# Jiahao-Ma/VFA

Hardware: AMD Instinct MI355X
Metric: voxels aggregated/sec (7 views->BEV grid) (higher is better)
Workload: dtype f32; 1 GPU; multiviewc_200x200x1; cameras_per_rank=7, cameras_total=7, channels=256, rccl_ranks=1, parallelism=single GPU

## Files before the change

include/vfa_hip.h:

```cpp
#ifndef VFA_HIP_H
#define VFA_HIP_H

#include <stddef.h>
#include <stdint.h>

#ifdef __cplusplus
extern "C" {
#endif

#define VFA_ABI_VERSION 9

#define VFA_CONV_MULTIVIEWC 0
#define VFA_CONV_MULTIVIEWX 1
#define VFA_CONV_WILDTRACK 2

#define VFA_VOX_REFERENCE 0
#define VFA_VOX_LAYER_MAJOR 1

#define VFA_VOX_KERNEL_DIRECT 0x100
#define VFA_VOX_KERNEL_TAP_CACHE 0x200

#define VFA_ERR_BAD_ARGUMENT 10001
#define VFA_ERR_UNSUPPORTED 10002

int vfa_abi_version(void);

#define VFA_FLAG_TERMS_MASK 0xf
#define VFA_FLAG_RESERVED_CUS(n) (((n) & 0xff) << 8)
#define VFA_FLAG_DEBUG(mask) (((mask) & 0xfff) << 16)
#define VFA_FLAG_DUMP_VOX (1 << 30)
#define VFA_FLAG_ROWS_ONLY (1 << 28)
#define VFA_FLAG_SKIP_ROWS (1 << 29)
#define VFA_BWD_ACCUMULATE 1

int vfa_integral_image_f32(const float *feature, float *integral, int n_views, int C, int Hf, int Wf,
                           void *stream);

int vfa_affine_relu_integral_image_f32(const float *x, const float *scale, const float *shift, float *integral, int n_views, int C,
                                       int Hf, int Wf, void *stream);

size_t vfa_feature_stats_count(int n_views, int C, int Hf);
int vfa_integral_images_f32(const float *const *features, const float *const *scales, const float *const *shifts,
                            float *const *integrals, unsigned *const *absmax, int n_views, int C, int n_maps, const int *feat_hw,
                            void *stream);
int vfa_integral_absmax_f32(const float *integral, unsigned *absmax, int n_views, int C, int Hf, int Wf, void *stream);

int vfa_integral_images_hwc_f32(const float *const *features_hwc, const float *const *scales, const float *const *shifts,
                                float *const *integrals, unsigned *const *absmax, int n_views, int C, int n_maps, const int *feat_hw,
                                void *stream);

size_t vfa_lateral_conv_workspace_bytes(int n_views, int Hf, int Wf);
int vfa_lateral_conv_f32(const float *feat, const float *weight, const float *bias, const float *gamma, const float *beta, float eps,
                         float *out_hwc, float *scale, float *shift, void *workspace, size_t workspace_bytes, int n_views, int K,
                         int Hf, int Wf, void *stream);
int vfa_lateral_convs_f32(int n_maps, const float *const *feats, const float *const *weights, const float *const *biases,
                          const float *const *gammas, const float *const *betas, const float *eps, float *const *outs_hwc,
                          float *const *scales, float *const *shifts, void *const *workspaces, const size_t *workspace_bytes, int n_views,
                          const int *Ks, const int *feat_hw, void *stream);

int vfa_lateral_convs_train_f32(int n_maps, const float *const *feats, const float *const *weights, const float *const *biases,
                                const float *const *gammas, const float *const *betas, const float *eps, float *const *outs_hwc,
                                float *const *scales, float *const *shifts, double *const *means, double *const *rstds,
                                void *const *workspaces, const size_t *workspace_bytes, int n_views, const int *Ks, const int *feat_hw,
                                void *stream);
size_t vfa_lateral_backward_workspace_bytes(int n_views, int K, int Hf, int Wf);
int vfa_lateral_scan_backward_f32(int n_maps, const float *const *grad_integrals, const float *const *ys_hwc, const float *const *scales,
                                  const float *const *shifts, const double *const *means, const double *const *rstds,
                                  const float *const *gammas, float *const *dzs_hwc, float *const *grad_biases, float *const *grad_gammas,
                                  float *const *grad_betas, void *const *workspaces, const size_t *workspace_bytes, int n_views,
                                  const int *Ks, const int *feat_hw, void *stream);
int vfa_lateral_conv_backward_f32(int n_maps, const float *const *dzs_hwc, const float *const *ys_hwc, const double *const *means,
                                  const float *const *feats, const float *const *weights, float *const *grad_feats,
                                  float *const *grad_weights, void *const *workspaces, const size_t *workspace_bytes, int n_views,
                                  const int *Ks, const int *feat_hw, void *stream);

int vfa_box_params_f32(const float *calibs, const float *grid, const float *z_layers, const float *corner_off,
                       int n_views, int n_cells, int nl, int conv_kind, float img_w, float img_h, int Hf, int Wf,
                       float cmin, float cmax, float *box, float *area, uint8_t *visible, void *stream);

int vfa_gather_f32(const float *integral, const float *box, const float *area, const uint8_t *visible, float *vox,
                   int n_views, int C, int Hf, int Wf, int nl, int n_cells, int cell_begin, int cell_count,
                   int vox_layout, void *stream);

int vfa_project_gather_f32(const float *integral, const float *calibs, const float *grid, const float *z_layers,
                           const float *corner_off, float *vox, int n_views, int C, int Hf, int Wf, int nl,
                           int n_cells, int cell_begin, int cell_count, int conv_kind, float img_w, float img_h,
                           float cmin, float cmax, int vox_layout, void *stream);

int vfa_project_collapse_f32(const float *integral, const float *calibs, const float *grid, const float *z_layers,
                             const float *corner_off, const float *weight_t, float *lin, int n_views, int C, int Hf, int Wf,
                             int nl, int n_cells, int c_out, int conv_kind, float img_w, float img_h, float cmin, float cmax,
                             void *stream);

size_t vfa_gather_workspace_bytes(int n_views, int nl, int cell_count);
int vfa_project_gather_ws_f32(const float *integral, const float *calibs, const float *grid, const float *z_layers,
                              const float *corner_off, float *vox, void *workspace, size_t workspace_bytes, int n_views,
                              int C, int Hf, int Wf, int nl, int n_cells, int cell_begin, int cell_count, int conv_kind,
                              float img_w, float img_h, float cmin, float cmax, int vox_layout, void *stream);

int vfa_project_gather_backward_f32(const float *grad_vox, const float *calibs, const float *grid, const float *z_layers,
                                    const float *corner_off, float *grad_integral, int n_views, int C, int Hf, int Wf,
                                    int nl, int n_cells, int cell_begin, int cell_count, int conv_kind, float img_w,
                                    float img_h, float cmin, float cmax, int flags, void *stream);
int vfa_project_gather_backward_grid_f32(const float *grad_vox, const float *calibs, const float *grid, const float *z_layers,
                                    const float *corner_off, float *grad_integral, int n_views, int C, int Hf, int Wf,
                                    int nl, int n_cells, int cell_begin, int cell_count, int grid_w, int conv_kind, float img_w,
                                    float img_h, float cmin, float cmax, int flags, void *stream);

size_t vfa_gather_backward_det_workspace_bytes(int n_views, int nl, int cell_count, int C, int Hf, int Wf);
int vfa_project_gather_backward_det_f32(const float *grad_vox, const float *calibs, const float *grid, const float *z_layers,
                                        const float *corner_off, float *grad_integral, int n_views, int C, int Hf, int Wf, int nl,
                                        int n_cells, int cell_begin, int cell_count, int grid_w, int conv_kind, float img_w,
                                        float img_h, float cmin, float cmax, int flags, void *workspace, size_t workspace_bytes,
                                        void *stream);

size_t vfa_gather_backward_geometry_workspace_bytes(int n_views, int cell_count);
int vfa_project_gather_backward_geometry_f32(const float *grad_vox, const float *integral, const float *calibs, const float *grid,
                                             const float *z_layers, const float *corner_off, float *grad_calibs, float *grad_grid,
                                             int n_views, int C, int Hf, int Wf, int nl, int n_cells, int cell_begin, int cell_count,
                                             int conv_kind, float img_w, float img_h, float cmin, float cmax, int flags, void *workspace,
                                             size_t workspace_bytes, void *stream);

int vfa_column_sum_f32(const float *x, float *out, long long rows, int N, int accumulate, void *stream);

int vfa_integral_image_backward_f32(float *grad_integral, float *grad_feature, int n_views, int C, int Hf, int Wf,
                                    void *stream);

int vfa_relu_mask_backward_f32(const float *grad, const float *lin, const float *bias, float *grad_lin, float *grad_bias,
                               int n_views, size_t M, int N, void *stream);

int vfa_bias_relu_accumulate_f32(const float *lin, const float *bias, float *out, int n_views, size_t M, int N,
                                 int accumulate, void *stream);

int vfa_scale_view_sum_f32(const float *lin8, const float *lin16, const float *lin32, const float *bias8,
                           const float *bias16, const float *bias32, float *ortho, int n_views, size_t M, int N,
                           int accumulate, void *stream);

int vfa_scale_view_max_f32(const float *lin8, const float *lin16, const float *lin32, const float *bias8, const float *bias16,
                           const float *bias32, float *ortho, uint8_t *argmax, int n_views, size_t M, int N, void *stream);

int vfa_scale_view_max_backward_f32(const float *grad, const float *lin8, const float *lin16, const float *lin32, const float *bias8,
                                    const float *bias16, const float *bias32, const uint8_t *argmax, float *grad_lin8,
                                    float *grad_lin16, float *grad_lin32, float *grad_bias8, float *grad_bias16, float *grad_bias32,
                                    int n_views, size_t M, int N, void *stream);

int vfa_collapse_relu_sum_f32(const float *vox, const float *weight, const float *bias, float *out, int n_views, size_t M,
                              int K, int N, int accumulate, int flags, void *stream);

size_t vfa_collapse_gemm_workspace_bytes(int K, int N);
int vfa_collapse_gemm_f32(const float *vox, const float *weight, float *lin, void *workspace, size_t workspace_bytes, size_t M,
                          int K, int N, int flags, void *stream);

int vfa_collapse_gemm_relu_backward_f32(const float *vox, const float *weight, const float *bias, const float *grad_out,
                                        float *grad_lin, float *grad_bias, void *workspace, size_t workspace_bytes, int n_views,
                                        size_t cells, int K, int N, int flags, void *stream);
int vfa_collapse_gemm_relu_backward_f16_f32(const float *vox, const float *weight, const float *bias, const float *grad_out,
                                            float *grad_lin, float *grad_bias, void *workspace, size_t workspace_bytes, int n_views,
                                            size_t cells, int K, int N, const unsigned *feat_absmax, int absmax_count,
                                            const unsigned char *row_shift, const unsigned char *tile_any, int flags, void *stream);
size_t vfa_sliver_shifts_scratch_bytes(int L, int W);
int vfa_sliver_shifts_u8(const float *calibs, const float *grid, const float *z_layers, int n_layers, const float *corner_off, int n_views,
                         int L, int W, int conv_kind, float img_w, float img_h, float cmin, float cmax, int Hf, int Wf, int per_item,
                         unsigned char *shift, void *scratch, size_t scratch_bytes, void *stream);

size_t vfa_frame_workspace_bytes(int n_views, int L, int W, int n_scales);
int vfa_frame_workspace_layout(int n_views, int L, int W, int n_scales, size_t *offsets, int *tiles);
int vfa_frame_records_f32(const float *calibs, const float *grid, const float *z_layers, const float *corner_off, int n_views, int L,
                          int W, int conv_kind, float img_w, float img_h, float cmin, float cmax, int n_scales,
                          const int *feat_hw, const float *const *weights, int flags, void *workspace, size_t workspace_bytes,
                          void *stream);
int vfa_frame_boxes_f32(const float *calibs, const float *grid, const float *z_layers, const float *corner_off, int n_views, int L,
                        int W, int conv_kind, float img_w, float img_h, float cmin, float cmax, int n_scales,
                        const int *feat_hw, void *workspace, size_t workspace_bytes, void *stream);
int vfa_frame_cuts_f32(int n_views, int L, int W, int n_scales, const float *const *weights, int flags, void *workspace,
                       size_t workspace_bytes, void *stream);
int vfa_pool_windows_f32(const float *integral, const void *workspace, size_t workspace_bytes, float *vox, int n_views, int L, int W,
                         int n_scales, int scale, int Hf, int Wf, void *stream);
int vfa_pool_collapse_relu_sum_f32(const float *const *integrals, const unsigned *const *feat_absmax, const float *const *biases,
                                   const void *workspace, size_t workspace_bytes, float *out, int n_views, int L, int W, int n_scales,
                                   const int *feat_hw, int accumulate, int flags, void *stream);

size_t vfa_pipe_workspace_bytes(int n_views, int L, int W, int n_layers, int n_scales);
int vfa_pipe_workspace_layout(int n_views, int L, int W, int n_layers, int n_scales, size_t *offsets, int *tiles);
int vfa_pipe_boxes_f32(const float *calibs, const float *grid, const float *z_layers, int n_layers, const float *corner_off, int n_views,
                       int L, int W, int conv_kind, float img_w, float img_h, float cmin, float cmax, int n_scales, const int *feat_hw,
                       int flags, void *workspace, size_t workspace_bytes, void *stream);
int vfa_pipe_cuts_f32(int n_views, int L, int W, int n_layers, int n_scales, const float *const *weights, int flags, void *workspace,
                      size_t workspace_bytes, void *stream);
int vfa_pipe_records_f32(const float *calibs, const float *grid, const float *z_layers, int n_layers, const float *corner_off,
                         int n_views, int L, int W, int conv_kind, float img_w, float img_h, float cmin, float cmax, int n_scales,
                         const int *feat_hw, const float *const *weights, int flags, void *workspace, size_t workspace_bytes, void *stream);
int vfa_pipe_collapse_relu_sum_f32(const float *const *integrals, const unsigned *const *feat_absmax, const float *const *biases,
                                   void *workspace, size_t workspace_bytes, float *out, int n_views, int L, int W, int n_layers,
                                   int n_scales, const int *feat_hw, int accumulate, int flags, void *stream);
int vfa_pipe_balance_f32(int n_views, int L, int W, int n_layers, int n_scales, int reserved_cus, int mode, void *workspace,
                         size_t workspace_bytes, void *stream);

size_t vfa_pipe_batch_workspace_bytes(int n_frames, int n_views, int L, int W, int n_layers, int n_scales);
int vfa_pipe_batch_workspace_layout(int n_frames, int n_views, int L, int W, int n_layers, int n_scales, size_t *offsets, int *tiles);
int vfa_pipe_batch_records_f32(const float *calibs, const float *grid, const float *z_layers, int n_layers, const float *corner_off,
                               int n_views, int L, int W, int conv_kind, float img_w, float img_h, float cmin, float cmax, int n_scales,
                               const int *feat_hw, const float *const *weights, int n_frames, int flags, void *workspace,
                               size_t workspace_bytes, void *stream);
int vfa_pipe_batch_collapse_relu_sum_f32(const float *const *integrals, const unsigned *const *feat_absmax, const float *const *biases,
                                         void *workspace, size_t workspace_bytes, float *out, int n_frames, int n_views, int L, int W,
                                         int n_layers, int n_scales, const int *feat_hw, int accumulate, int flags, void *stream);
int vfa_pipe_batch_balance_f32(int n_frames, int n_views, int L, int W, int n_layers, int n_scales, int reserved_cus, int mode,
                               void *workspace, size_t workspace_bytes, void *stream);

size_t vfa_grad_weight_workspace_bytes(long long rows, int K);
int vfa_grad_weight_f32(const float *g_lin, const float *vox, float *g_w, long long rows, int K, int accumulate, void *workspace,
                        size_t workspace_bytes, void *stream);
size_t vfa_grad_input_workspace_bytes(int K);
int vfa_grad_input_f32(const float *g_lin, const float *w, float *g_vox, long long rows, int K, void *workspace, size_t workspace_bytes,
                       void *stream);

int vfa_sort_vertices_f32(const float *vertices, const uint8_t *mask, const int *num_valid, int *idx, int b, int n, int m, void *stream);
int vfa_bev_nms_f32(const float *heatmap, float *conf, int L, int W, void *stream);
int vfa_bev_nms_batch_f32(const float *heatmap, float *conf, int B, int L, int W, void *stream);

int vfa_iou3d_f32(const float *box1, const float *box2, float *iou3d, float *iou_bev, long long count, void *stream);
int vfa_iou3d_frames_f32(const float *det, const int *det_begin, const float *gt, const int *gt_begin, int n_frames, int n_det, int n_gt,
                         const long long *pair_begin, long long n_pairs, float *iou, int *best_idx, float *best_iou, void *stream);

#define VFA_CLEAR_MOD_MAX_SIDE 512
#define VFA_CLEAR_MOD_TOO_LARGE 1
#define VFA_CLEAR_MOD_BAD_OFFSETS 2
#define VFA_CLEAR_MOD_SOLVER_FLAG 3
int vfa_clear_mod_frames_f64(const double *det_xy, const int *det_begin, const double *gt_xy, const int *gt_begin, int n_frames, int n_det,
                             int n_gt, double td, const long long *pair_begin, long long n_pairs, double *dist, int *gt_match,
                             double *gt_dist, long long *frame_counts, double *frame_cost, int *frame_status, void *stream);

#define VFA_BEV_DECODE_MAX_TOPK 1024
size_t vfa_bev_decode_workspace_bytes(int B, int L, int W, int topk);
int vfa_bev_decode_f32(const float *heatmap, const float *loc_offset, const long long *loc_stride, const float *dim_offset,
                       const long long *dim_stride, const float *rotation, const long long *rot_stride, int B, int L, int W, int n_rot,
                       int topk, float cls_thresh, float grid0, float grid1, float world0, float world1, const float *dimension_mean,
                       int yx_first, void *workspace, size_t workspace_bytes, int *count, float *conf, float *location, int *cell,
                       float *dimension, float *rotation_out, void *stream);

#ifdef __cplusplus
}
#endif
#endif
```

vfa_amd/_lib.py:

```python
import ctypes
import os

_HERE = os.path.dirname(os.path.abspath(__file__))
LIB_PATH = os.environ.get("VFA_AMD_LIB") or os.path.join(_HERE, "csrc", "libvfa_hip.so")
ABI_VERSION = 9

CONV_KIND = {"MultiviewC": 0, "MultiviewX": 1, "Wildtrack": 2}
VOX_REFERENCE, VOX_LAYER_MAJOR = 0, 1
VOX_KERNEL_DIRECT, VOX_KERNEL_TAP_CACHE = 0x100, 0x200
BWD_ACCUMULATE = 1


FLAG_ROWS_ONLY, FLAG_SKIP_ROWS = 1 << 28, 1 << 29
FLAG_DUMP_VOX = 1 << 30


def collapse_flags(terms=0, reserved_cus=0):
    return (int(terms) & 0xf) | ((int(reserved_cus) & 0xff) << 8)


_c_int, _c_float, _c_size_t, _vp, _c_longlong = ctypes.c_int, ctypes.c_float, ctypes.c_size_t, ctypes.c_void_p, ctypes.c_longlong
_c_double = ctypes.c_double

SIGNATURES = {
    "vfa_abi_version": [],
    "vfa_integral_image_f32": [_vp, _vp, _c_int, _c_int, _c_int, _c_int, _vp],
    "vfa_affine_relu_integral_image_f32": [_vp, _vp, _vp, _vp, _c_int, _c_int, _c_int, _c_int, _vp],
    "vfa_box_params_f32": [_vp, _vp, _vp, _vp, _c_int, _c_int, _c_int, _c_int, _c_float, _c_float, _c_int, _c_int,
                           _c_float, _c_float, _vp, _vp, _vp, _vp],
    "vfa_gather_f32": [_vp, _vp, _vp, _vp, _vp, _c_int, _c_int, _c_int, _c_int, _c_int, _c_int, _c_int, _c_int, _c_int,
                       _vp],
    "vfa_project_gather_f32": [_vp, _vp, _vp, _vp, _vp, _vp, _c_int, _c_int, _c_int, _c_int, _c_int, _c_int, _c_int,
                               _c_int, _c_int, _c_float, _c_float, _c_float, _c_float, _c_int, _vp],
    "vfa_project_collapse_f32": [_vp, _vp, _vp, _vp, _vp, _vp, _vp, _c_int, _c_int, _c_int, _c_int, _c_int, _c_int, _c_int,
                                 _c_int, _c_float, _c_float, _c_float, _c_float, _vp],
    "vfa_gather_workspace_bytes": [_c_int, _c_int, _c_int],
    "vfa_project_gather_ws_f32": [_vp, _vp, _vp, _vp, _vp, _vp, _vp, _c_size_t, _c_int, _c_int, _c_int, _c_int, _c_int,
                                  _c_int, _c_int, _c_int, _c_int, _c_float, _c_float, _c_float, _c_float, _c_int, _vp],
    "vfa_project_gather_backward_f32": [_vp, _vp, _vp, _vp, _vp, _vp, _c_int, _c_int, _c_int, _c_int, _c_int, _c_int,
                                        _c_int, _c_int, _c_int, _c_float, _c_float, _c_float, _c_float, _c_int, _vp],
    "vfa_project_gather_backward_grid_f32": [_vp, _vp, _vp, _vp, _vp, _vp, _c_int, _c_int, _c_int, _c_int, _c_int, _c_int,
                                             _c_int, _c_int, _c_int, _c_int, _c_float, _c_float, _c_float, _c_float, _c_int, _vp],
    "vfa_gather_backward_det_workspace_bytes": [_c_int, _c_int, _c_int, _c_int, _c_int, _c_int],
    "vfa_project_gather_backward_det_f32": [_vp, _vp, _vp, _vp, _vp, _vp, _c_int, _c_int, _c_int, _c_int, _c_int, _c_int,
                                            _c_int, _c_int, _c_int, _c_int, _c_float, _c_float, _c_float, _c_float, _c_int, _vp,
                                            _c_size_t, _vp],
    "vfa_gather_backward_geometry_workspace_bytes": [_c_int, _c_int],
    "vfa_project_gather_backward_geometry_f32": [_vp, _vp, _vp, _vp, _vp, _vp, _vp, _vp, _c_int, _c_int, _c_int, _c_int, _c_int, _c_int,
                                                 _c_int, _c_int, _c_int, _c_float, _c_float, _c_float, _c_float, _c_int, _vp, _c_size_t,
                                                 _vp],
    "vfa_column_sum_f32": [_vp, _vp, _c_longlong, _c_int, _c_int, _vp],
    "vfa_integral_image_backward_f32": [_vp, _vp, _c_int, _c_int, _c_int, _c_int, _vp],
    "vfa_relu_mask_backward_f32": [_vp, _vp, _vp, _vp, _vp, _c_int, _c_size_t, _c_int, _vp],
    "vfa_bias_relu_accumulate_f32": [_vp, _vp, _vp, _c_int, _c_size_t, _c_int, _c_int, _vp],
    "vfa_scale_view_sum_f32": [_vp, _vp, _vp, _vp, _vp, _vp, _vp, _c_int, _c_size_t, _c_int, _c_int, _vp],
    "vfa_scale_view_max_f32": [_vp, _vp, _vp, _vp, _vp, _vp, _vp, _vp, _c_int, _c_size_t, _c_int, _vp],
    "vfa_scale_view_max_backward_f32": [_vp, _vp, _vp, _vp, _vp, _vp, _vp, _vp, _vp, _vp, _vp, _vp, _vp, _vp, _c_int, _c_size_t, _c_int,
                                        _vp],
    "vfa_collapse_gemm_workspace_bytes": [_c_int, _c_int],
    "vfa_collapse_gemm_f32": [_vp, _vp, _vp, _vp, _c_size_t, _c_size_t, _c_int, _c_int, _c_int, _vp],
    "vfa_collapse_gemm_relu_backward_f32": [_vp, _vp, _vp, _vp, _vp, _vp, _vp, _c_size_t, _c_int, _c_size_t, _c_int, _c_int, _c_int, _vp],
    "vfa_collapse_gemm_relu_backward_f16_f32": [_vp, _vp, _vp, _vp, _vp, _vp, _vp, _c_size_t, _c_int, _c_size_t, _c_int, _c_int, _vp, _c_int, _vp,
                                                _vp, _c_int, _vp],
    "vfa_sliver_shifts_scratch_bytes": [_c_int, _c_int],
    "vfa_sliver_shifts_u8": [_vp, _vp, _vp, _c_int, _vp, _c_int, _c_int, _c_int, _c_int, _c_float, _c_float, _c_float, _c_float, _c_int, _c_int,
                             _c_int, _vp, _vp, _c_size_t, _vp],
    "vfa_collapse_relu_sum_f32": [_vp, _vp, _vp, _vp, _c_int, _c_size_t, _c_int, _c_int, _c_int, _c_int, _vp],
    "vfa_feature_stats_count": [_c_int, _c_int, _c_int],
    "vfa_integral_images_f32": [_vp, _vp, _vp, _vp, _vp, _c_int, _c_int, _c_int, _vp, _vp],
    "vfa_integral_images_hwc_f32": [_vp, _vp, _vp, _vp, _vp, _c_int, _c_int, _c_int, _vp, _vp],
    "vfa_integral_absmax_f32": [_vp, _vp, _c_int, _c_int, _c_int, _c_int, _vp],
    "vfa_lateral_conv_workspace_bytes": [_c_int, _c_int, _c_int],
    "vfa_lateral_conv_f32": [_vp, _vp, _vp, _vp, _vp, _c_float, _vp, _vp, _vp, _vp, _c_size_t, _c_int, _c_int, _c_int, _c_int, _vp],
    "vfa_grad_weight_workspace_bytes": [_c_longlong, _c_int],
    "vfa_grad_weight_f32": [_vp, _vp, _vp, _c_longlong, _c_int, _c_int, _vp, _c_size_t, _vp],
    "vfa_grad_input_workspace_bytes": [_c_int],
    "vfa_grad_input_f32": [_vp, _vp, _vp, _c_longlong, _c_int, _vp, _c_size_t, _vp],
    "vfa_lateral_convs_f32": [_c_int, _vp, _vp, _vp, _vp, _vp, _vp, _vp, _vp, _vp, _vp, _vp, _c_int, _vp, _vp, _vp],
    "vfa_lateral_convs_train_f32": [_c_int, _vp, _vp, _vp, _vp, _vp, _vp, _vp, _vp, _vp, _vp, _vp, _vp, _vp, _c_int, _vp, _vp, _vp],
    "vfa_lateral_backward_workspace_bytes": [_c_int, _c_int, _c_int, _c_int],
    "vfa_lateral_scan_backward_f32": [_c_int, _vp, _vp, _vp, _vp, _vp, _vp, _vp, _vp, _vp, _vp, _vp, _vp, _vp, _c_int, _vp, _vp, _vp],
    "vfa_lateral_conv_backward_f32": [_c_int, _vp, _vp, _vp, _vp, _vp, _vp, _vp, _vp, _vp, _c_int, _vp, _vp, _vp],
    "vfa_sort_vertices_f32": [_vp, _vp, _vp, _vp, _c_int, _c_int, _c_int, _vp],
    "vfa_bev_nms_f32": [_vp, _vp, _c_int, _c_int, _vp],
    "vfa_frame_workspace_bytes": [_c_int, _c_int, _c_int, _c_int],
    "vfa_frame_workspace_layout": [_c_int, _c_int, _c_int, _c_int, _vp, _vp],
    "vfa_frame_records_f32": [_vp, _vp, _vp, _vp, _c_int, _c_int, _c_int, _c_int, _c_float, _c_float, _c_float, _c_float,
                              _c_int, _vp, _vp, _c_int, _vp, _c_size_t, _vp],
    "vfa_frame_boxes_f32": [_vp, _vp, _vp, _vp, _c_int, _c_int, _c_int, _c_int, _c_float, _c_float, _c_float, _c_float,
                            _c_int, _vp, _vp, _c_size_t, _vp],
    "vfa_frame_cuts_f32": [_c_int, _c_int, _c_int, _c_int, _vp, _c_int, _vp, _c_size_t, _vp],
    "vfa_pool_windows_f32": [_vp, _vp, _c_size_t, _vp, _c_int, _c_int, _c_int, _c_int, _c_int, _c_int, _c_int, _vp],
    "vfa_pool_collapse_relu_sum_f32": [_vp, _vp, _vp, _vp, _c_size_t, _vp, _c_int, _c_int, _c_int, _c_int, _vp, _c_int, _c_int,
                                       _vp],
    "vfa_pipe_workspace_bytes": [_c_int, _c_int, _c_int, _c_int, _c_int],
    "vfa_pipe_workspace_layout": [_c_int, _c_int, _c_int, _c_int, _c_int, _vp, _vp],
    "vfa_pipe_boxes_f32": [_vp, _vp, _vp, _c_int, _vp, _c_int, _c_int, _c_int, _c_int, _c_float, _c_float, _c_float, _c_float,
                           _c_int, _vp, _c_int, _vp, _c_size_t, _vp],
    "vfa_pipe_cuts_f32": [_c_int, _c_int, _c_int, _c_int, _c_int, _vp, _c_int, _vp, _c_size_t, _vp],
    "vfa_pipe_records_f32": [_vp, _vp, _vp, _c_int, _vp, _c_int, _c_int, _c_int, _c_int, _c_float, _c_float, _c_float, _c_float,
                             _c_int, _vp, _vp, _c_int, _vp, _c_size_t, _vp],
    "vfa_pipe_collapse_relu_sum_f32": [_vp, _vp, _vp, _vp, _c_size_t, _vp, _c_int, _c_int, _c_int, _c_int, _c_int, _vp, _c_int, _c_int,
                                       _vp],
    "vfa_pipe_balance_f32": [_c_int, _c_int, _c_int, _c_int, _c_int, _c_int, _c_int, _vp, _c_size_t, _vp],
    "vfa_pipe_batch_workspace_bytes": [_c_int, _c_int, _c_int, _c_int, _c_int, _c_int],
    "vfa_pipe_batch_workspace_layout": [_c_int, _c_int, _c_int, _c_int, _c_int, _c_int, _vp, _vp],
    "vfa_pipe_batch_records_f32": [_vp, _vp, _vp, _c_int, _vp, _c_int, _c_int, _c_int, _c_int, _c_float, _c_float, _c_float, _c_float,
                                   _c_int, _vp, _vp, _c_int, _c_int, _vp, _c_size_t, _vp],
    "vfa_pipe_batch_collapse_relu_sum_f32": [_vp, _vp, _vp, _vp, _c_size_t, _vp, _c_int, _c_int, _c_int, _c_int, _c_int, _c_int, _vp,
                                             _c_int, _c_int, _vp],
    "vfa_pipe_batch_balance_f32": [_c_int, _c_int, _c_int, _c_int, _c_int, _c_int, _c_int, _c_int, _vp, _c_size_t, _vp],
    "vfa_bev_nms_batch_f32": [_vp, _vp, _c_int, _c_int, _c_int, _vp],
    "vfa_iou3d_f32": [_vp, _vp, _vp, _vp, _c_longlong, _vp],
    "vfa_iou3d_frames_f32": [_vp, _vp, _vp, _vp, _c_int, _c_int, _c_int, _vp, _c_longlong, _vp, _vp, _vp, _vp],
    "vfa_clear_mod_frames_f64": [_vp, _vp, _vp, _vp, _c_int, _c_int, _c_int, _c_double, _vp, _c_longlong, _vp, _vp, _vp, _vp, _vp, _vp, _vp],
    "vfa_bev_decode_workspace_bytes": [_c_int, _c_int, _c_int, _c_int],
    "vfa_bev_decode_f32": [_vp, _vp, _vp, _vp, _vp, _vp, _vp, _c_int, _c_int, _c_int, _c_int, _c_int, _c_float, _c_float, _c_float,
                           _c_float, _c_float, _vp, _c_int, _vp, _c_size_t, _vp, _vp, _vp, _vp, _vp, _vp, _vp],
}

_lib = None


class VFAHipError(RuntimeError):
    pass


def lib():
    global _lib
    if _lib is None:
        if not os.path.exists(LIB_PATH):
            raise VFAHipError(
                f"{LIB_PATH} is missing: build it with `python -m vfa_amd.build` (hipcc --offload-arch=gfx950). "
                "vfa_amd has no CPU or PyTorch fallback.")
        handle = ctypes.CDLL(LIB_PATH)
        for name, argtypes in SIGNATURES.items():
            fn = getattr(handle, name)
            fn.argtypes = argtypes
            fn.restype = ctypes.c_size_t if name.endswith(("_bytes", "_count")) else ctypes.c_int
        got = handle.vfa_abi_version()
        if got != ABI_VERSION:
            raise VFAHipError(f"libvfa_hip.so has ABI version {got}, the Python side expects {ABI_VERSION}; rebuild")
        _lib = handle
    return _lib


def call(name, *args):
    status = getattr(lib(), name)(*args)
    if status != 0:
        raise VFAHipError(f"{name} failed with status {status}"
                          + (" (bad argument)" if status == 10001 else " (hipError_t)"))


def ptr(t):
    return None if t is None else ctypes.c_void_p(t.data_ptr())


def ptr_array(tensors):
    return (ctypes.c_void_p * len(tensors))(*[None if t is None else t.data_ptr() for t in tensors])


def int_array(values):
    return (ctypes.c_int * len(values))(*[int(v) for v in values])


def current_device_index():
    import torch
    return torch._C._cuda_getDevice()


def current_stream_handle():
    import torch
    try:
        return ctypes.c_void_p(torch._C._cuda_getCurrentRawStream(torch._C._cuda_getDevice()))
    except AttributeError:
        return ctypes.c_void_p(torch.cuda.current_stream().cuda_stream)


def current_stream(dev):
    import torch
    return torch.cuda.current_stream(dev.index if dev.index is not None else current_device_index())


def require_device(*tensors):
    for t in tensors:
        if t is not None and not t.is_cuda:
            raise VFAHipError("vfa_amd runs on an AMD GPU (MI355X, gfx950) only; got a CPU tensor and there is no "
                              "CPU fallback")
```

vfa_amd/csrc/vfa_fused.hip:

```cpp
#include <hip/hip_runtime.h>
#include <stdint.h>
#include <type_traits>

#include "vfa_geom.h"
#include "vfa_split.h"
#include "vfa_tile.h"

#ifndef VFA_TICKET_ORDER
#define VFA_TICKET_ORDER __ATOMIC_RELAXED
#endif

namespace {
using namespace vfa_dev;

constexpr int kRecBytes = 96;
constexpr int kMaxSlots = 123;
constexpr unsigned kItemCost = 704, kRowItemCost = 522;
constexpr int kRecSlots = 3;
constexpr int kThreads = 512;
constexpr int kRowBytes = 2 * kC;
constexpr int kPlane = kTileBoxes * kRowBytes;
constexpr int kSteps = kC / 16;

constexpr int kCont = 1 << 8;
constexpr int kTileRows = 4;
constexpr int kTileShiftAt = 8;

typedef int i32x8 __attribute__((ext_vector_type(8)));

struct RecordArgs {
    BoxGeom g;
    int n_views, L, W, tiles_w, n_tiles, n_scales;
    ScaleDims dims[kMaxScales];
    unsigned *live[kMaxScales];
    unsigned *direct[kMaxScales];
    unsigned *overflow[kMaxScales];
    unsigned *row_counter;
    unsigned rows_cap;
    unsigned *row_list;
    unsigned char *hdrs[kMaxScales];
    unsigned char *recs[kMaxScales];
    unsigned short *item_w;
    int views_pad;
};

__global__ __launch_bounds__(kWave) void frame_records_kernel(RecordArgs a)
{
    __shared__ uint4 stage[2][kTileBoxes * 6];
    const TileLane ln = tile_lane(a.n_views, a.n_tiles, a.tiles_w, a.L, a.W);
    const int lane = threadIdx.x, half = ln.half, b = ln.b, view = ln.view, tile = ln.tile;
    const bool pair_ok = ln.pair_ok, valid = ln.valid;

    float l, t, r, bt;
    cube_box(a.g, a.g.calibs + (size_t)view * 12, ln.cell, 0, l, t, r, bt);
#pragma unroll 1
    for (int s = 0; s < a.n_scales; ++s) {
        const int Hf = a.dims[s].Hf, Wf = a.dims[s].Wf;
        const float area = box_area(l, t, r, bt, Hf, Wf);
        const bool vis = valid && box_visible(area, Hf, Wf);
        const float masked = valid ? area * 0.0f : 0.0f;
        const bool live_box = vis || (valid && masked != masked);
        const BoxTaps tp = box_taps(l, t, r, bt, Hf, Wf);
        const int dx = tp.xr.i0 - tp.xl.i0, dy = tp.yb.i0 - tp.yt.i0;
        const int dxc = dx == 0 ? 0 : (dx == 1 ? 1 : 2), dyc = dy == 0 ? 0 : (dy == 1 ? 1 : 2);
        const TileWindow tw = tile_window(tp, vis, live_box, area, Hf, Wf, half);
        const Window &win = tw.w;
        const bool any_live = tw.any_live;
        const int shift = tw.shift, n_slots = win.n_slots;
        const bool direct = n_slots > kMaxSlots;
        unsigned rows[4], cols[4];
        tap_parts(win, tp, direct, rows, cols);
        const int tag = (vis ? 1 : 0) | (dxc << 1) | (dyc << 3);
        const unsigned kx = (unsigned)(tp.xs[0] + 1) | ((unsigned)(tp.xs[2] + 1) << 16), ky = (unsigned)(tp.ys[0] + 1) | ((unsigned)(tp.ys[2] + 1) << 16);
        const int tag_p = __shfl_up(tag, 1);
        const unsigned kx_p = __shfl_up(kx, 1), ky_p = __shfl_up(ky, 1);
        const bool cont = vis && (b & 3) != 0 && tag_p == tag && kx_p == kx && ky_p == ky;

        float w[16];
        {
            float q[4];
            bilinear_weights(q, tp.xl, tp.yt); w[0] = q[0]; w[1] = q[1]; w[2] = q[2]; w[3] = q[3];
            bilinear_weights(q, tp.xr, tp.yb); w[4] = q[0]; w[5] = q[1]; w[6] = q[2]; w[7] = q[3];
            bilinear_weights(q, tp.xr, tp.yt); w[8] = q[0]; w[9] = q[1]; w[10] = q[2]; w[11] = q[3];
            bilinear_weights(q, tp.xl, tp.yb); w[12] = q[0]; w[13] = q[1]; w[14] = q[2]; w[15] = q[3];
        }
        if (pair_ok) {
            uint4 *st = stage[half] + b * 6;
            st[0] = make_uint4(__float_as_uint(w[0]), __float_as_uint(w[1]), __float_as_uint(w[2]), __float_as_uint(w[3]));
            st[1] = make_uint4(__float_as_uint(w[4]), __float_as_uint(w[5]), __float_as_uint(w[6]), __float_as_uint(w[7]));
            st[2] = make_uint4(__float_as_uint(w[8]), __float_as_uint(w[9]), __float_as_uint(w[10]), __float_as_uint(w[11]));
            st[3] = make_uint4(__float_as_uint(w[12]), __float_as_uint(w[13]), __float_as_uint(w[14]), __float_as_uint(w[15]));
            const float rcp = 1.0f / area;
            st[4] = make_uint4(__float_as_uint(rcp), (unsigned)tag | (cont ? (unsigned)kCont : 0u), rows[0] | (rows[1] << 16),
                               rows[2] | (rows[3] << 16));
            st[5] = make_uint4(cols[0] | (cols[1] << 16), cols[2] | (cols[3] << 16), __float_as_uint(masked), __float_as_uint(area));
        }
        __syncthreads();
        if (pair_ok) {
            uint4 *rec = reinterpret_cast<uint4 *>(a.recs[s] + ((size_t)view * a.n_tiles + tile) * kTileBoxes * kRecBytes);
#pragma unroll
            for (int k = 0; k < 6; ++k) rec[k * 32 + b] = stage[half][k * 32 + b];
            if (b == 0) {
                uint4 *hdr = reinterpret_cast<uint4 *>(a.hdrs[s] + ((size_t)view * a.n_tiles + tile) * kHdrBytes);
                unsigned hflags = (any_live ? kTileLive : 0) | (direct ? kTileDirect : 0) | ((unsigned)shift << kTileShiftAt), word2 = (unsigned)win.cwid;
                if (any_live) atomicOr(a.live[s] + tile, 1u << view);
                if (any_live && direct) {
                    atomicOr(a.direct[s] + tile, 1u << view);
                    const unsigned slot = atomicAdd(a.row_counter, 1u);
                    if (slot < a.rows_cap) {
                        hflags |= kTileRows; word2 = slot;
                        a.row_list[slot] = ((unsigned)s << 30) | ((unsigned)view << 25) | (unsigned)tile;
                    }
                    else atomicOr(a.overflow[s] + tile, 1u << view);
                }
                const bool main_item = any_live && !(direct && !(hflags & kTileRows));
                a.item_w[((size_t)tile * kMaxScales + s) * a.views_pad + view] =
                    (unsigned short)(!main_item ? 0u : (direct ? kRowItemCost : kItemCost + (unsigned)n_slots));
                hdr[0] = tile_header0(hflags, win, word2);
                hdr[1] = tile_header1(win);
            }
        }
        __syncthreads();
        if (blockIdx.x == 0 && lane < 6)
            reinterpret_cast<uint4 *>(a.recs[s] + (size_t)a.n_views * a.n_tiles * kTileBoxes * kRecBytes)[lane] = make_uint4(0u, 0u, 0u, 0u);
    }
}

struct ShiftArgs {
    BoxGeom g;
    int n_views, L, W, tiles_w, n_tiles, nl, Hf, Wf, per_item;
    unsigned char *out;
    unsigned *tile_max;
};
__global__ __launch_bounds__(kWave) void sliver_shift_kernel(ShiftArgs a)
{
    const TileLane ln = tile_lane(a.n_views, a.n_tiles, a.tiles_w, a.L, a.W);
    const float *P = a.g.calibs + (size_t)ln.view * 12;
    int shift = 0;
    for (int layer = 0; layer < a.nl; ++layer) {
        float l, t, r, bt;
        cube_box(a.g, P, ln.cell, layer, l, t, r, bt);
        const float area = box_area(l, t, r, bt, a.Hf, a.Wf);
        if (ln.valid && box_visible(area, a.Hf, a.Wf)) shift = max(shift, sliver_shift(area, a.Hf, a.Wf));
    }
#pragma unroll
    for (int m = 1; m < 32; m <<= 1) shift = max(shift, __shfl_xor(shift, m, 32));
    if (a.per_item) {
        if (ln.valid) a.out[(size_t)ln.view * a.L * a.W + ln.cell] = (unsigned char)shift;
    } else if (ln.pair_ok && ln.b == 0 && shift > 0) {
        atomicMax(a.tile_max + ln.tile, (unsigned)shift);
    }
}
__global__ __launch_bounds__(256) void sliver_expand_kernel(const unsigned *tile_max, unsigned char *out, int L, int W, int tiles_w)
{
    const int cell = blockIdx.x * 256 + threadIdx.x;
    if (cell >= L * W) return;
    const int cl = cell / W, cw = cell - cl * W;
    out[cell] = (unsigned char)tile_max[(cl / kTileL) * tiles_w + cw / kTileW];
}

constexpr int kWmaxParts = 32;
struct SplitArgs { const float *w[kMaxScales]; uint4 *out[kMaxScales]; unsigned *wmax; int *wexp; int f16; };
constexpr int kSplitBlocks = 8 * kSteps * 64 / 1024;
__device__ __forceinline__ void split_block(const SplitArgs &sa, int b, unsigned long long *part)
{
    const int scale = b / kSplitBlocks, j = b - scale * kSplitBlocks, tid = threadIdx.x;
    const float *__restrict__ w = sa.w[scale];
    uint4 *__restrict__ out = sa.out[scale];
    int ew = 0;
    if (sa.f16) {
        unsigned m = 0u;
        for (int i = tid; i < kC * kC; i += 1024) m = max(m, __float_as_uint(w[i]) & 0x7fffffffu);
        m = wave_max_u32(m);
        if ((tid & 63) == 0) part[tid >> 6] = m;
        __syncthreads();
        unsigned mm = 0u;
        for (int i = 0; i < 16; ++i) mm = max(mm, (unsigned)part[i]);
        ew = split_exponent(mm, kExpW);
    }
    const int idx = j * 1024 + tid;
    const int lane = idx & 63, st = (idx >> 6) & 15, wave = idx >> 10;
    const float *src = w + (size_t)(wave * 32 + (lane & 31)) * kC + 16 * st + 8 * (lane >> 5);
    if (idx == 0 && scale == 0) sa.wexp[kMaxScales] = sa.f16 ? 2 : 3;
    uint4 uh, ul;
    if (sa.f16) {
        fp16_saturate_mode(true);
        if (idx == 0) sa.wexp[scale] = ew;
        const float sc = pow2f(ew);
        uint2 h0, l0, h1, l1;
        split_f16x4(src[0] * sc, src[1] * sc, src[2] * sc, src[3] * sc, h0, l0);
        split_f16x4(src[4] * sc, src[5] * sc, src[6] * sc, src[7] * sc, h1, l1);
        uh = make_uint4(h0.x, h0.y, h1.x, h1.y);
        ul = make_uint4(l0.x, l0.y, l1.x, l1.y);
    } else {
        union { __bf16 b[8]; uint4 u; } hi, lo;
#pragma unroll
        for (int k = 0; k < 8; ++k) {
            const float x = src[k];
            hi.b[k] = (__bf16)x;
            lo.b[k] = (__bf16)(x - (float)hi.b[k]);
        }
        uh = hi.u; ul = lo.u;
    }
    out[((size_t)(wave * kSteps + st) * 2 + 0) * 64 + lane] = uh;
    out[((size_t)(wave * kSteps + st) * 2 + 1) * 64 + lane] = ul;
}

struct ChunkArgs {
    const unsigned *live[kMaxScales], *overflow[kMaxScales];
    const unsigned short *item_w;
    int n_scales, n_tiles, n_views, views_pad;
    int *chunk_start, *chunk_rank;
    SplitArgs split;
    int n_split_blocks;
};
template <int G> struct TileItemsT { unsigned m[kMaxScales]; uint4 q[kMaxScales][G]; };
template <int G>
__global__ __launch_bounds__(1024) void tile_chunks_kernel(ChunkArgs a)
{
    using TileItems = TileItemsT<G>;
    constexpr bool kCache = G == 1;
    __shared__ unsigned long long part[1024];
    if (blockIdx.x > 0) {
        split_block(a.split, (int)blockIdx.x - 1, part);
        return;
    }
    const int tid = threadIdx.x, n_tiles = a.n_tiles;
    const unsigned view_mask = a.n_views >= 32 ? 0xffffffffu : ((1u << a.n_views) - 1u);
    const int per = (n_tiles + 1023) / 1024, t0 = min(n_tiles, tid * per), t1 = min(n_tiles, t0 + per);
    constexpr unsigned kScale = 294, kTile = 330, kEmpty = 32;
    struct RawTile { unsigned lv[kMaxScales], ov[kMaxScales]; uint4 q[kMaxScales][G]; };
    auto load_raw = [&](int t) {
        RawTile rt;
#pragma unroll
        for (int s = 0; s < kMaxScales; ++s) {
            const bool on = s < a.n_scales;
            const unsigned *lp = on ? a.live[s] : a.live[0], *op = on ? a.overflow[s] : a.overflow[0];
            rt.lv[s] = lp[t]; rt.ov[s] = op[t];
#pragma unroll
            for (int g = 0; g < G; ++g) {
                const int gg = g * 8 < a.n_views ? g : 0;
                rt.q[s][g] = *reinterpret_cast<const uint4 *>(a.item_w + ((size_t)t * kMaxScales + (on ? s : 0)) * a.views_pad + 8 * gg);
            }
        }
        return rt;
    };
    auto finish_tile = [&](const RawTile &rt) {
        TileItems ti;
#pragma unroll
        for (int s = 0; s < kMaxScales; ++s) {
            const bool on = s < a.n_scales;
            ti.m[s] = on ? rt.lv[s] & ~rt.ov[s] & view_mask : 0u;
#pragma unroll
            for (int g = 0; g < G; ++g) ti.q[s][g] = (!on || g * 8 >= a.n_views) ? make_uint4(0u, 0u, 0u, 0u) : rt.q[s][g];
        }
        return ti;
    };
    auto load_tile = [&](int t) { return finish_tile(load_raw(t)); };
    auto walk = [&](const TileItems &ti, auto &&visit) -> unsigned {
        unsigned w = 0;
        int k = 0;
#pragma unroll
        for (int s = 0; s < kMaxScales; ++s) {
            bool first = true;
#pragma unroll
            for (int g = 0; g < G; ++g) {
                unsigned mg = (ti.m[s] >> (8 * g)) & 0xffu;
                const uint4 q = ti.q[s][g];
                const unsigned long long lo = (unsigned long long)q.x | ((unsigned long long)q.y << 32), hi = (unsigned long long)q.z | ((unsigned long long)q.w << 32);
                while (mg) {
                    const int v = __builtin_ctz(mg);
                    mg &= mg - 1u;
                    unsigned wi = (unsigned)(((v < 4 ? lo : hi) >> (16 * (v & 3))) & 0xffffull);
                    if (first) wi += kScale;
                    if (k == 0) wi += kTile;
                    first = false;
                    visit(k, w, w + wi);
                    w += wi;
                    ++k;
                }
            }
        }
        return k == 0 ? kEmpty : w;
    };
    TileItems c0 = {}, c1 = {};
    if (kCache && n_tiles > 0) {
        const RawTile r0 = load_raw(min(t0, n_tiles - 1)), r1 = load_raw(min(t0 + 1, n_tiles - 1));
        __builtin_amdgcn_sched_barrier(0);
        c0 = finish_tile(r0);
        c1 = finish_tile(r1);
    }
    auto tile_of = [&](int t) { return (kCache && t == t0) ? c0 : (kCache && t == t0 + 1) ? c1 : load_tile(t); };
    unsigned long long local = 0;
    for (int t = t0; t < t1; ++t) local += walk(tile_of(t), [](int, unsigned, unsigned) {});
    part[tid] = local;
    for (int c = tid; c <= kChunks; c += 1024) { a.chunk_start[c] = n_tiles; a.chunk_rank[c] = 0; }
    __syncthreads();
    for (int d = 1; d < 1024; d <<= 1) {
        const unsigned long long v = tid >= d ? part[tid - d] : 0ull;
        __syncthreads();
        part[tid] += v;
        __syncthreads();
    }
    const unsigned long long total = part[1023];
    unsigned long long before = part[tid] - local;
    auto pos_of = [&](long long cc) { return (total * (unsigned long long)cc + kChunks - 1) / kChunks; };
    for (int t = t0; t < t1; ++t) {
        const unsigned long long tb = before;
        long long c = tb > 0 ? (long long)((tb - 1) * kChunks / total) : 0;
        while (c < kChunks && pos_of(c) < tb) ++c;
        const TileItems ti = tile_of(t);
        int n_items = 0;
        walk(ti, [&](int kk, unsigned, unsigned) { n_items = kk + 1; });
        const unsigned w = walk(ti, [&](int kk, unsigned w0, unsigned w1) {
            while (c < kChunks) {
                const unsigned long long pc = pos_of(c);
                if (pc >= tb + w1) break;
                const int k = ((unsigned)(pc - tb) - w0) * 2 < (w1 - w0) ? kk : kk + 1;
                if (k >= n_items) { a.chunk_start[c] = t + 1 < n_tiles ? t + 1 : n_tiles; a.chunk_rank[c] = 0; }
                else { a.chunk_start[c] = t; a.chunk_rank[c] = k; }
                ++c;
            }
        });
        if (n_items == 0)
            for (; c < kChunks && pos_of(c) < tb + w; ++c) { a.chunk_start[c] = t; a.chunk_rank[c] = 0; }
        before += w;
    }
}

struct FusedScale {
    const float *integral;
    const float *bias;
    const uint4 *wfrag;
    const unsigned *live, *direct, *overflow;
    const unsigned char *hdrs, *recs;
    int Hf, Wf;
    const unsigned *amax;
    int amax_n;
};
struct FusedArgs {
    FusedScale sc[kMaxScales];
    int n_scales, n_views, L, W, tiles_w, n_tiles;
    float *out;
    const int *chunk_start, *chunk_rank;
    float *partial;
    unsigned *tickets;
    const float *rows;
    const unsigned *row_counter;
    int rows_cap;
    int accumulate;
    const int *wexp;
    int debug;
    unsigned long long *diag;
};
constexpr int kDbgNoFills = 1, kDbgNoPool = 2, kDbgNoMfma = 4, kDbgOneW = 8, kDbgNoRecords = 16, kDbgNoExtra = 32, kDbgStamps = 128;
constexpr int kDbgDumpVox = 0x1000;

struct LRec { uint4 v[6]; };

template <bool F16>
__device__ __forceinline__ void store_quad_at(unsigned char *planes, int off, float4 v)
{
    uint2 hu, lu;
    if constexpr (F16) {
        split_f16x4(v.x, v.y, v.z, v.w, hu, lu);
    } else {
        const float x[4] = {v.x, v.y, v.z, v.w};
        union { __bf16 b[4]; uint2 u; } hi, lo;
#pragma unroll
        for (int j = 0; j < 4; ++j) {
            hi.b[j] = (__bf16)x[j];
            lo.b[j] = (__bf16)(x[j] - (float)hi.b[j]);
        }
        hu = hi.u; lu = lo.u;
    }
    *reinterpret_cast<uint2 *>(planes + off) = hu;
    *reinterpret_cast<uint2 *>(planes + kPlane + off) = lu;
}
template <bool F16>
__device__ __forceinline__ void store_quad(unsigned char *planes, int row, int c4, float4 v)
{
    store_quad_at<F16>(planes, row * kRowBytes + ((((c4 >> 1) ^ (row & 15)) << 4) | ((c4 & 1) << 3)), v);
}

struct Item { int tile, scale, view; unsigned rest; bool valid; int rank; };

template <int TERMS, bool DIAG, bool DIRECT>
__global__ __launch_bounds__(kThreads) void pool_collapse_kernel(FusedArgs a)
{
    __shared__ float4 s_taps[(kMaxSlots + kRecSlots) * 64];
    __shared__ __align__(16) unsigned char s_planes[2 * kPlane];
    __shared__ uint4 s_hdr[2][16];
    const int tid = threadIdx.x, wave = uniform_i(tid >> 6), lane = tid & 63, r = lane & 31, h = lane >> 5;
    constexpr bool F16 = TERMS == 2;

    if (DIRECT && uniform_i((int)*a.row_counter) <= a.rows_cap) return;
    const int nblk = gridDim.x;
    if (uniform_i(a.wexp[kMaxScales]) != (F16 ? 2 : 3)) {
        if (!DIRECT)
            for (size_t i = (size_t)blockIdx.x * kThreads + tid; i < (size_t)a.L * a.W * kC; i += (size_t)nblk * kThreads)
                a.out[i] = __uint_as_float(0x7fc00000u);
        return;
    }
    const int lb = (int)xcd_contiguous(blockIdx.x, (nblk + 7) / 8);
    if (lb >= nblk) return;
    const int t_step = DIRECT ? nblk : 1;
    auto range_of = [&](int wg, int &tb, int &kb, int &te, int &ke) {
        const int c0 = (int)((long long)kChunks * wg / nblk), c1 = (int)((long long)kChunks * (wg + 1) / nblk);
        tb = uniform_i(a.chunk_start[c0]); kb = uniform_i(a.chunk_rank[c0]);
        te = uniform_i(a.chunk_start[c1]); ke = uniform_i(a.chunk_rank[c1]);
    };
    int t_begin = lb, k_begin = 0, t_end = a.n_tiles, k_end = 0;
    if (!DIRECT) range_of(lb, t_begin, k_begin, t_end, k_end);
    if (t_begin > t_end || (t_begin == t_end && k_begin >= k_end)) return;
    const int t_lim = (!DIRECT && k_end > 0) ? t_end + 1 : t_end;
    __shared__ unsigned s_ticket;
    auto share_of = [&](int tile, int &first, int &last, int &parts) {
        first = lb; last = lb; parts = 1;
        for (int j = lb - 1; j >= 0; --j) {
            int tb, kb, te, ke;
            range_of(j, tb, kb, te, ke);
            if (te < tile || (te == tile && ke == 0)) break;
            if (tb > te || (tb == te && kb >= ke)) continue;
            first = j; ++parts;
        }
        for (int j = lb + 1; j < nblk; ++j) {
            int tb, kb, te, ke;
            range_of(j, tb, kb, te, ke);
            if (tb > tile) break;
            if (tb > te || (tb == te && kb >= ke)) continue;
            last = j; ++parts;
        }
    };
    int sh_b_first = lb, sh_b_last = lb, sh_b_parts = 1, sh_e_first = lb, sh_e_last = lb, sh_e_parts = 1;
    if (!DIRECT && k_begin > 0) share_of(t_begin, sh_b_first, sh_b_last, sh_b_parts);
    if (!DIRECT && k_end > 0) share_of(t_end, sh_e_first, sh_e_last, sh_e_parts);
    const unsigned view_mask = a.n_views >= 32 ? 0xffffffffu : ((1u << a.n_views) - 1u);

    float f_a[kMaxScales] = {1.0f, 1.0f, 1.0f}, f_a_inv[kMaxScales] = {1.0f, 1.0f, 1.0f}, f_fwd[kMaxScales] = {1.0f, 1.0f, 1.0f}, f_inv[kMaxScales] = {1.0f, 1.0f, 1.0f};
    if constexpr (F16) {
        __shared__ unsigned s_amax[kMaxScales];
        if (tid < kMaxScales) s_amax[tid] = 0u;
        __syncthreads();
#pragma unroll
        for (int s2 = 0; s2 < kMaxScales; ++s2) {
            if (s2 < a.n_scales) {
                unsigned m = 0u;
                for (int i = tid; i < a.sc[s2].amax_n; i += kThreads) m = max(m, a.sc[s2].amax[i]);
                m = wave_max_u32(m);
                if (lane == 0) atomicMax(&s_amax[s2], m);
            }
        }
        __syncthreads();
#pragma unroll
        for (int s2 = 0; s2 < kMaxScales; ++s2) {
            if (s2 < a.n_scales) {
                const int ea = split_exponent((unsigned)uniform_i((int)s_amax[s2]), kExpA), ew = uniform_i(a.wexp[s2]);
                f_a[s2] = pow2f(ea); f_a_inv[s2] = pow2f(-ea); f_fwd[s2] = pow2f(ea + ew); f_inv[s2] = pow2f(-(ea + ew));
            }
        }
    }
    auto pick = [&](const float (&t)[kMaxScales], int scale) { return scale == 0 ? t[0] : (scale == 1 ? t[1] : t[2]); };

    auto mask_at = [&](const unsigned *p, int tile) {
        return *reinterpret_cast<const __attribute__((address_space(4))) unsigned *>((size_t)(p + tile));
    };
    auto live_all = [&](int tile, int scale) { return mask_at(a.sc[scale].live, tile) & view_mask; };
    auto live_of = [&](int tile, int scale) {
        const unsigned dm = mask_at(a.sc[scale].overflow, tile) & view_mask;
        return DIRECT ? dm : (mask_at(a.sc[scale].live, tile) & view_mask & ~dm);
    };
    auto seek = [&](int tile, int scale, unsigned rest, int rank) {
        Item it;
        it.valid = false; it.tile = tile; it.scale = scale; it.view = 0; it.rest = 0; it.rank = rank;
        while (tile < t_lim) {
            if (rest) {
                if (!DIRECT && tile == t_end && rank >= k_end) return it;
                it.view = __builtin_ctz(rest);
                it.rest = rest & (rest - 1u);
                it.tile = tile; it.scale = scale; it.rank = rank; it.valid = true;
                return it;
            }
            if (++scale == a.n_scales) { scale = 0; tile += t_step; rank = 0; }
            if (tile < t_lim) rest = live_of(tile, scale);
        }
        return it;
    };

    auto bias_of = [&](int scale) { return a.sc[scale].bias ? a.sc[scale].bias[wave * 32 + r] : 0.0f; };
    float rbias[kMaxScales];
#pragma unroll
    for (int s2 = 0; s2 < kMaxScales; ++s2) rbias[s2] = s2 < a.n_scales ? relu_t(bias_of(s2)) : 0.0f;

    auto write_tile = [&](int tile, const f32x16 &sum, bool have_sum) {
        if (DIAG && (a.debug & kDbgDumpVox)) return;
        const int tl = tile / a.tiles_w, tw = tile - tl * a.tiles_w;
        float extra = 0.0f;
        if (!DIRECT && !(DIAG && (a.debug & kDbgNoExtra))) {
#pragma unroll
            for (int s = 0; s < kMaxScales; ++s)
                if (s < a.n_scales) extra += (float)(a.n_views - __popc(live_all(tile, s))) * rbias[s];
        }
        int h2 = h, r2 = r;
        asm volatile("" : "+v"(h2), "+v"(r2));
        float *ocol = a.out + wave * 32 + r2;
#pragma unroll
        for (int i = 0; i < 16; ++i) {
            const int row = (i & 3) + 8 * (i >> 2) + 4 * h2;
            const int cl = tl * kTileL + (row >> 3), cw = tw * kTileW + (row & 7);
            if (cl < a.L && cw < a.W) {
                float *o = ocol + (size_t)(cl * a.W + cw) * kC;
                float v = (have_sum ? sum[i] : 0.0f) + extra;
                if (DIRECT || a.accumulate) v += *o;
                *o = v;
            }
        }
    };

    auto header_of = [&](const Item &it, int buf) {
        if (wave == 0) {
            const unsigned char *p = a.sc[it.scale].hdrs + ((size_t)it.view * a.n_tiles + it.tile) * kHdrBytes + lane * 4;
            __builtin_amdgcn_global_load_lds((const __attribute__((address_space(1))) void *)p,
                                             (__attribute__((address_space(3))) void *)(&s_hdr[buf][0]), 4, 0, 0);
        }
    };
    auto header_get = [&](i32x8 &hd, int buf) {
        const uint4 h0 = s_hdr[buf][0], h1 = s_hdr[buf][1];
        hd[0] = uniform_i((int)h0.x); hd[1] = uniform_i((int)h0.y); hd[2] = uniform_i((int)h0.z); hd[3] = uniform_i((int)h0.w);
        hd[4] = uniform_i((int)h1.x); hd[5] = uniform_i((int)h1.y); hd[6] = uniform_i((int)h1.z); hd[7] = uniform_i((int)h1.w);
    };
    constexpr int kFillWaves = 4;
    int f_slot = 0, f_n = 0;
    unsigned f_off = 0;
    const char *f_img = nullptr;
    auto begin_fills = [&](const Item &it, const i32x8 &hd) {
        f_slot = wave;
        f_n = 0;
        if (wave >= kFillWaves) return;
        const FusedScale &sc = a.sc[it.scale];
        const int slot = wave + kFillWaves * (lane & 31);
        if (!DIRECT && (hd[0] & kTileRows)) {
            f_n = kTileBoxes;
            f_off = (unsigned)slot * kSlotBytes;
            f_img = reinterpret_cast<const char *>(a.rows) + (size_t)hd[2] * kTileBoxes * kSlotBytes;
            return;
        }
        f_n = (DIRECT || (hd[0] & kTileDirect)) ? 0 : hd[1];
        const int cw = hd[2], inv = hd[3], x0 = hd[4], t0 = hd[5], top = hd[6], b0 = hd[7], wp = sc.Wf + 2;
        const int wr = (slot * inv) >> 16, wc = slot - wr * cw;
        const int y = wr < top ? t0 + wr : b0 + (wr - top), x = x0 + wc;
        f_off = (unsigned)((y + 1) * wp + (x + 1)) * kSlotBytes;
        f_img = reinterpret_cast<const char *>(sc.integral) + (size_t)it.view * (sc.Hf + 2) * wp * kSlotBytes;
    };
    auto fill_at = [&](int j) {
        const char *src = f_img + (size_t)(unsigned)__builtin_amdgcn_readlane((int)f_off, j) + lane * 16;
        __builtin_amdgcn_global_load_lds((const __attribute__((address_space(1))) void *)src,
                                         (__attribute__((address_space(3))) void *)(s_taps + f_slot * 64), 16, 0, 0);
        f_slot += kFillWaves;
    };
    auto one_fill = [&](int j) {
        if (f_slot < f_n) fill_at(j);
    };
    auto rest_fills = [&]() {
        while (f_slot < f_n) fill_at((f_slot - wave) / kFillWaves);
    };

    const int grp = lane >> 4, cq = lane & 15;
    LRec rec;
    auto load_record = [&](const Item &it, int it_flags, int it_slot) {
        if constexpr (DIRECT) {
            const uint4 *p = reinterpret_cast<const uint4 *>(a.sc[it.scale].recs + (((size_t)it.view * a.n_tiles + it.tile) * kTileBoxes + 4 * wave + grp) * kRecBytes);
#pragma unroll
            for (int k = 0; k < 6; ++k) rec.v[k] = p[k];
        } else if (!(it_flags & kTileRows) && wave >= 1 && wave <= kRecSlots) {
            const int k = wave - 1;
            const unsigned char *p = a.sc[it.scale].recs + ((size_t)it.view * a.n_tiles + it.tile) * kTileBoxes * kRecBytes + k * 1024 + lane * 16;
            __builtin_amdgcn_global_load_lds((const __attribute__((address_space(1))) void *)p,
                                             (__attribute__((address_space(3))) void *)(s_taps + (kMaxSlots + k) * 64), 16, 0, 0);
        }
    };
    auto dump_vox = [&](int tile, int row, int c4, float4 v) {
        const int tl = tile / a.tiles_w, tw = tile - tl * a.tiles_w;
        const int cl = tl * kTileL + (row >> 3), cw = tw * kTileW + (row & 7);
        if (cl < a.L && cw < a.W) *reinterpret_cast<float4 *>(a.out + (size_t)(cl * a.W + cw) * kC + 4 * c4) = v;
    };
    auto pool = [&](const Item &it, int it_flags, int it_word1, float s_a, float s_a_inv) {
        if (!DIRECT && (it_flags & kTileRows)) {
#pragma unroll
            for (int q = 0; q < 4; ++q) {
                float4 v = s_taps[(4 * wave + grp) * 64 + q * 16 + cq];
                if (DIAG && (a.debug & kDbgDumpVox)) dump_vox(it.tile, 4 * wave + grp, q * 16 + cq, v);
                if constexpr (F16) v = mul4(v, s_a);
                store_quad<F16>(s_planes, 4 * wave + grp, q * 16 + cq, v);
            }
            return;
        }
        const FusedScale &sc = a.sc[it.scale];
        const unsigned Wp = (unsigned)sc.Wf + 2u;
        const char *img = reinterpret_cast<const char *>(sc.integral) + (size_t)it.view * (sc.Hf + 2) * Wp * kSlotBytes;
        if constexpr (!DIRECT) {
            const uint4 *rp = reinterpret_cast<const uint4 *>(s_taps + kMaxSlots * 64) + (4 * wave + grp) * (kRecBytes / 16);
#pragma unroll
            for (int k = 0; k < 6; ++k) rec.v[k] = rp[k];
        }
        const float wt[16] = {__uint_as_float(rec.v[0].x), __uint_as_float(rec.v[0].y), __uint_as_float(rec.v[0].z), __uint_as_float(rec.v[0].w),
                              __uint_as_float(rec.v[1].x), __uint_as_float(rec.v[1].y), __uint_as_float(rec.v[1].z), __uint_as_float(rec.v[1].w),
                              __uint_as_float(rec.v[2].x), __uint_as_float(rec.v[2].y), __uint_as_float(rec.v[2].z), __uint_as_float(rec.v[2].w),
                              __uint_as_float(rec.v[3].x), __uint_as_float(rec.v[3].y), __uint_as_float(rec.v[3].z), __uint_as_float(rec.v[3].w)};
        const float rcp = __uint_as_float(rec.v[4].x), masked = __uint_as_float(rec.v[5].z), area = __uint_as_float(rec.v[5].w);
        const bool vis = (rec.v[4].y & (unsigned)kVis) != 0u;
        unsigned rw[4] = {rec.v[4].z & 0xffffu, rec.v[4].z >> 16, rec.v[4].w & 0xffffu, rec.v[4].w >> 16};
        unsigned cl[4] = {rec.v[5].x & 0xffffu, rec.v[5].x >> 16, rec.v[5].y & 0xffffu, rec.v[5].y >> 16};
#pragma unroll
        for (int k = 0; k < 4; ++k) {
            rw[k] = (vis ? (DIRECT ? rw[k] * Wp : rw[k]) : 0u) * 64u + (unsigned)cq;
            cl[k] = (vis ? cl[k] : 0u) * 64u;
        }
        const int row = 4 * wave + grp;
        auto pair = [&](int q, int ra, int ca, int rb2, int cb, const float *wa, const float *wb, float4 &sa, float4 &sb) {
            float4 t[2][4];
#pragma unroll
            for (int k = 0; k < 4; ++k) {
                const unsigned oa = rw[ra + (k >> 1)] + cl[ca + (k & 1)] + (unsigned)(q * 16);
                const unsigned ob = rw[rb2 + (k >> 1)] + cl[cb + (k & 1)] + (unsigned)(q * 16);
                if constexpr (DIRECT) {
                    t[0][k] = *reinterpret_cast<const float4 *>(img + (size_t)oa * 16);
                    t[1][k] = *reinterpret_cast<const float4 *>(img + (size_t)ob * 16);
                } else {
                    t[0][k] = s_taps[oa];
                    t[1][k] = s_taps[ob];
                }
            }
            sa = sample4(t[0][0], t[0][1], t[0][2], t[0][3], wa[0], wa[1], wa[2], wa[3]);
            sb = sample4(t[1][0], t[1][1], t[1][2], t[1][3], wb[0], wb[1], wb[2], wb[3]);
        };
        const float rs = (vis ? rcp : masked) * s_a, as = area * s_a_inv;
        const int plane0 = row * kRowBytes + (((((cq >> 1) ^ (row & 15)) << 4)) | ((cq & 1) << 3));
        auto finish = [&](int q, float4 lt, float4 rb, float4 rt, float4 lb) {
            float4 v = make_float4(lt.x + rb.x, lt.y + rb.y, lt.z + rb.z, lt.w + rb.w);
            v = make_float4(v.x - rt.x, v.y - rt.y, v.z - rt.z, v.w - rt.w);
            v = make_float4(v.x - lb.x, v.y - lb.y, v.z - lb.z, v.w - lb.w);
            v = make_float4(box_quotient_scaled(v.x, as, rs), box_quotient_scaled(v.y, as, rs), box_quotient_scaled(v.z, as, rs),
                            box_quotient_scaled(v.w, as, rs));
            if (DIAG && (a.debug & kDbgDumpVox))
                dump_vox(it.tile, row, q * 16 + cq, make_float4(v.x * s_a_inv, v.y * s_a_inv, v.z * s_a_inv, v.w * s_a_inv));
            store_quad_at<F16>(s_planes, plane0 ^ (q << 7), v);
        };
        if constexpr (DIRECT) {
#pragma unroll 1
            for (int q = 0; q < 4; ++q) {
                float4 lt, rb, rt, lb;
                pair(q, 0, 0, 2, 2, wt + 0, wt + 4, lt, rb);
                __builtin_amdgcn_sched_barrier(0);
                pair(q, 0, 2, 2, 0, wt + 8, wt + 12, rt, lb);
                finish(q, lt, rb, rt, lb);
            }
        } else {
            unsigned tb[4][4];
#pragma unroll
            for (int i = 0; i < 4; ++i)
#pragma unroll
                for (int j = 0; j < 4; ++j) tb[i][j] = rw[i] + cl[j];
#pragma unroll
            for (int q = 0; q < 4; ++q) {
                float4 lt, rb, rt, lb;
                {
                    const float4 t0 = s_taps[tb[0][0] + q * 16], t1 = s_taps[tb[0][1] + q * 16], t2 = s_taps[tb[1][0] + q * 16], t3 = s_taps[tb[1][1] + q * 16];
                    const float4 u0 = s_taps[tb[2][2] + q * 16], u1 = s_taps[tb[2][3] + q * 16], u2 = s_taps[tb[3][2] + q * 16], u3 = s_taps[tb[3][3] + q * 16];
                    lt = sample4(t0, t1, t2, t3, wt[0], wt[1], wt[2], wt[3]);
                    rb = sample4(u0, u1, u2, u3, wt[4], wt[5], wt[6], wt[7]);
                }
                __builtin_amdgcn_sched_barrier(0);
                {
                    const float4 t0 = s_taps[tb[0][2] + q * 16], t1 = s_taps[tb[0][3] + q * 16], t2 = s_taps[tb[1][2] + q * 16], t3 = s_taps[tb[1][3] + q * 16];
                    const float4 u0 = s_taps[tb[2][0] + q * 16], u1 = s_taps[tb[2][1] + q * 16], u2 = s_taps[tb[3][0] + q * 16], u3 = s_taps[tb[3][1] + q * 16];
                    rt = sample4(t0, t1, t2, t3, wt[8], wt[9], wt[10], wt[11]);
                    lb = sample4(u0, u1, u2, u3, wt[12], wt[13], wt[14], wt[15]);
                }
                __builtin_amdgcn_sched_barrier(0);
                finish(q, lt, rb, rt, lb);
            }
        }
    };

    Frag w[kSteps];
    auto load_weights = [&](int scale) {
        const uint4 *src = a.sc[scale].wfrag + (size_t)wave * kSteps * 2 * 64 + lane;
#pragma unroll
        for (int s = 0; s < kSteps; ++s) {
            const uint4 uh = src[(s * 2 + 0) * 64], ul = src[(s * 2 + 1) * 64];
            w[s].hi = *reinterpret_cast<const bf16x8 *>(&uh);
            w[s].lo = *reinterpret_cast<const bf16x8 *>(&ul);
        }
    };

    const int key = r & 15;
    const int frag_base = r * kRowBytes + ((h ^ (key & 1)) << 4);

    Item cur;
    if (DIRECT || k_begin == 0) {
        cur = seek(t_begin, 0, live_of(t_begin, 0), 0);
    } else {
        int sc0 = 0, left = k_begin;
        unsigned rest0 = live_of(t_begin, 0);
        while (left > 0 && (rest0 || sc0 + 1 < a.n_scales)) {
            if (rest0) { rest0 &= rest0 - 1u; --left; }
            else rest0 = live_of(t_begin, ++sc0);
        }
        cur = seek(t_begin, sc0, rest0, k_begin);
    }
    {
        f32x16 none = {};
        if (!DIRECT)
            for (int t2 = t_begin; t2 < (cur.valid ? cur.tile : t_end); ++t2) write_tile(t2, none, false);
    }
    if (!cur.valid) return;
    const int dbg = DIAG ? a.debug : 0;
    unsigned long long stamp[8] = {0, 0, 0, 0, 0, 0, 0, 0}, t_prev = 0;
    auto tick = [&](int k) {
        if (DIAG && (dbg & kDbgStamps)) {
            const unsigned long long now = __builtin_amdgcn_s_memtime();
            stamp[k] += now - t_prev;
            t_prev = now;
        }
    };
    i32x8 nh;
    int hbuf = 0;
    header_of(cur, 1);
    __builtin_amdgcn_s_waitcnt(0x0f70);
    __syncthreads();
    header_get(nh, 1);
    int cur_flags = nh[0], cur_word1 = nh[2], nxt_flags = 0, nxt_word1 = 0;
    load_record(cur, cur_flags, cur_word1);
    if (!(dbg & kDbgNoFills)) {
        begin_fills(cur, nh);
        rest_fills();
    }
    Item nxt = seek(cur.tile, cur.scale, cur.rest, cur.rank + 1);
    if (nxt.valid) header_of(nxt, hbuf);
    int w_scale = -1;
    float bc = 0.0f, sa_cur = 1.0f, sa_inv_cur = 1.0f, inv_cur = 1.0f;
    f32x16 sum;
#pragma unroll
    for (int i = 0; i < 16; ++i) sum[i] = 0.0f;
    int pend_tile = -1, pend_next = 0;
    auto flush = [&]() {
        if (pend_tile < 0) return;
        if (!DIRECT) {
            const bool at_begin = pend_tile == t_begin && k_begin > 0, at_end = pend_tile == t_end && k_end > 0;
            if (!(at_begin || at_end)) {
                write_tile(pend_tile, sum, true);
            } else {
                const int which = at_begin ? 0 : 1;
                float *pp = a.partial + (((size_t)lb * 2 + which) * 8 + wave) * 16 * 64 + lane;
#pragma unroll
                for (int i = 0; i < 16; ++i) __hip_atomic_store(pp + i * 64, sum[i], __ATOMIC_RELAXED, __HIP_MEMORY_SCOPE_AGENT);
                asm volatile("s_waitcnt vmcnt(0)" ::: "memory");
                __syncthreads();
                if (tid == 0) s_ticket = __hip_atomic_fetch_add(a.tickets + pend_tile, 1u, VFA_TICKET_ORDER, __HIP_MEMORY_SCOPE_AGENT);
                __syncthreads();
                const int first = at_begin ? sh_b_first : sh_e_first, last = at_begin ? sh_b_last : sh_e_last;
                const int parts = at_begin ? sh_b_parts : sh_e_parts;
                if (uniform_i((int)s_ticket) == parts - 1) {
                    if (tid == 0) __hip_atomic_store(a.tickets + pend_tile, 0u, __ATOMIC_RELAXED, __HIP_MEMORY_SCOPE_AGENT);
                    f32x16 tot;
#pragma unroll
                    for (int i = 0; i < 16; ++i) tot[i] = 0.0f;
                    for (int j = first; j <= last; ++j) {
                        if (j == lb) {
#pragma unroll
                            for (int i = 0; i < 16; ++i) tot[i] += sum[i];
                            continue;
                        }
                        int tb, kb, te, ke;
                        range_of(j, tb, kb, te, ke);
                        if (tb > te || (tb == te && kb >= ke)) continue;
                        const int wj = (pend_tile == tb && kb > 0) ? 0 : 1;
                        const float *qq = a.partial + (((size_t)j * 2 + wj) * 8 + wave) * 16 * 64 + lane;
#pragma unroll
                        for (int i = 0; i < 16; ++i) tot[i] += __hip_atomic_load(qq + i * 64, __ATOMIC_RELAXED, __HIP_MEMORY_SCOPE_AGENT);
                    }
                    write_tile(pend_tile, tot, true);
                }
            }
        } else {
            write_tile(pend_tile, sum, true);
        }
#pragma unroll
        for (int i = 0; i < 16; ++i) sum[i] = 0.0f;
        if (!DIRECT)
            for (int t2 = pend_tile + 1; t2 < pend_next; ++t2) write_tile(t2, sum, false);
        pend_tile = -1;
    };
    if (DIAG) t_prev = __builtin_amdgcn_s_memtime();

    while (cur.valid) {
        Item nn;
        nn.valid = false;
        if (nxt.valid) nn = seek(nxt.tile, nxt.scale, nxt.rest, nxt.rank + 1);
        tick(0);
        __builtin_amdgcn_s_waitcnt(0x0f70);
        tick(1);
        __syncthreads();
        if (nxt.valid) header_get(nh, hbuf);
        tick(2);
        flush();
        if (cur.scale != w_scale && !((dbg & kDbgOneW) && w_scale >= 0)) {
            load_weights(cur.scale);
            bc = bias_of(cur.scale);
            if constexpr (F16) { bc *= pick(f_fwd, cur.scale); sa_cur = pick(f_a, cur.scale); sa_inv_cur = pick(f_a_inv, cur.scale); inv_cur = pick(f_inv, cur.scale); }
            w_scale = cur.scale;
        }
        const int shift = F16 ? (cur_flags >> kTileShiftAt) & 0xff : 0;
        const float up = pow2f(shift), down = pow2f(-shift);
        if constexpr (F16) fp16_saturate_mode(true);
        if (!(dbg & kDbgNoPool)) pool(cur, cur_flags, cur_word1, sa_cur * down, sa_inv_cur * up);
        if constexpr (F16) fp16_saturate_mode(false);
        tick(3);
        __builtin_amdgcn_s_waitcnt(0x0f70);
        __syncthreads();
        tick(4);
        f_n = 0;
        if (nxt.valid) {
            nxt_flags = nh[0]; nxt_word1 = nh[2];
            if (!(dbg & kDbgNoFills)) begin_fills(nxt, nh);
            if (!(dbg & kDbgNoRecords)) load_record(nxt, nxt_flags, nxt_word1);
        }
        hbuf ^= 1;
        if (nn.valid) header_of(nn, hbuf);
        tick(5);

        f32x16 acc;
#pragma unroll
        for (int i = 0; i < 16; ++i) acc[i] = bc * down;
        if (!(dbg & kDbgNoMfma)) {
            int key2 = key, fb = frag_base;
            asm volatile("" : "+v"(key2), "+v"(fb));
            const unsigned pa = (unsigned)(size_t)(__attribute__((address_space(3))) unsigned char *)s_planes + (unsigned)fb;
            auto frags = [&](int k, bf16x8 &hh, bf16x8 &ll) {
                const unsigned addr = pa + (unsigned)((k ^ (key2 >> 1)) << 5);
                asm volatile("ds_read_b128 %0, %2\n\tds_read_b128 %1, %2 offset:%3" : "=&v"(hh), "=&v"(ll) : "v"(addr), "n"(kPlane) : "memory");
            };
            bf16x8 fh[3], fl[3];
            frags(0, fh[0], fl[0]);
            frags(1, fh[1], fl[1]);
#pragma unroll
            for (int k = 0; k < kSteps; ++k) {
                one_fill(k);
                if (k + 2 < kSteps) {
                    frags(k + 2, fh[(k + 2) % 3], fl[(k + 2) % 3]);
                    asm volatile("s_waitcnt lgkmcnt(4)" : "+v"(fh[k % 3]), "+v"(fl[k % 3]));
                } else if (k + 1 < kSteps) {
                    asm volatile("s_waitcnt lgkmcnt(2)" : "+v"(fh[k % 3]), "+v"(fl[k % 3]));
                } else {
                    asm volatile("s_waitcnt lgkmcnt(0)" : "+v"(fh[k % 3]), "+v"(fl[k % 3]));
                }
                __builtin_amdgcn_sched_barrier(0);
                if constexpr (F16) {
                    const f16x8 ah = __builtin_bit_cast(f16x8, fh[k % 3]), al = __builtin_bit_cast(f16x8, fl[k % 3]);
                    const f16x8 wh = __builtin_bit_cast(f16x8, w[k].hi), wl = __builtin_bit_cast(f16x8, w[k].lo);
                    acc = __builtin_amdgcn_mfma_f32_32x32x16_f16(ah, wl, acc, 0, 0, 0);
                    acc = __builtin_amdgcn_mfma_f32_32x32x16_f16(ah, wh, acc, 0, 0, 0);
                    acc = __builtin_amdgcn_mfma_f32_32x32x16_f16(al, wh, acc, 0, 0, 0);
                } else {
                    acc = __builtin_amdgcn_mfma_f32_32x32x16_bf16(fh[k % 3], w[k].lo, acc, 0, 0, 0);
                    acc = __builtin_amdgcn_mfma_f32_32x32x16_bf16(fh[k % 3], w[k].hi, acc, 0, 0, 0);
                    acc = __builtin_amdgcn_mfma_f32_32x32x16_bf16(fl[k % 3], w[k].hi, acc, 0, 0, 0);
                    if (TERMS >= 4) acc = __builtin_amdgcn_mfma_f32_32x32x16_bf16(fl[k % 3], w[k].lo, acc, 0, 0, 0);
                }
                __builtin_amdgcn_sched_barrier(0);
            }
        }
        rest_fills();
#pragma unroll
        for (int i = 0; i < 16; ++i) {
            if constexpr (F16) sum[i] = fmaf(relu_t(acc[i]), inv_cur * up, sum[i]);
            else sum[i] = sum[i] + relu_t(acc[i]);
        }
        tick(6);

        if (!nxt.valid || nxt.tile != cur.tile) {
            pend_tile = cur.tile;
            pend_next = nxt.valid ? nxt.tile : t_end;
        }
        if (DIAG) stamp[7] += 1;
        cur = nxt;
        cur_flags = nxt_flags; cur_word1 = nxt_word1;
        nxt = nn;
    }
    flush();
    if (DIAG && (dbg & kDbgStamps) && a.diag && tid == ((dbg >> 8) & 7) * 64)
        for (int k = 0; k < 8; ++k) a.diag[(size_t)blockIdx.x * 8 + k] = stamp[k];
}

struct PoolArgs {
    const float *integral;
    const unsigned char *hdrs, *recs;
    const unsigned *direct;
    float *vox;
    int n_views, L, W, tiles_w, n_tiles, Hf, Wf;
    long long per_xcd;
};

__global__ __launch_bounds__(512, 2) void pool_windows_kernel(PoolArgs a)
{
    __shared__ float4 s_win0[(kMaxSlots + 3) / 4 * 4 * 16], s_win1[(kMaxSlots + 3) / 4 * 4 * 16];
    __shared__ __align__(16) unsigned char s_rec0[kTileBoxes * kRecBytes], s_rec1[kTileBoxes * kRecBytes];
    const int tid = threadIdx.x, wave = uniform_i(tid >> 6), lane = tid & 63, grp = lane >> 4, cq = lane & 15;
    const long long n_units = (long long)a.n_views * a.n_tiles * 4;
    const int nblk = gridDim.x;
    const int lb = (int)xcd_contiguous(blockIdx.x, (nblk + 7) / 8);
    if (lb >= nblk) return;
    const long long u_begin = n_units * lb / nblk, u_end = n_units * (lb + 1) / nblk;
    if (u_begin >= u_end) return;
    const int Wp = a.Wf + 2;
    const size_t img_stride = (size_t)(a.Hf + 2) * Wp * kSlotBytes;

    auto header_of = [&](long long u, i32x8 &hd) {
        const unsigned char *p = a.hdrs + (size_t)(u >> 2) * kHdrBytes;
        hd = *reinterpret_cast<const __attribute__((address_space(4))) i32x8 *>((size_t)p);
    };
    auto header_wait = [&](i32x8 &) {};
    struct Pos { int item, q, view, tl, tw; };
    auto pos_of = [&](long long u) {
        Pos p;
        p.item = (int)(u >> 2); p.q = (int)(u & 3);
        p.view = p.item / a.n_tiles;
        const int tile = p.item - p.view * a.n_tiles;
        p.tl = tile / a.tiles_w; p.tw = tile - p.tl * a.tiles_w;
        return p;
    };
    auto advance = [&](Pos &p) {
        if (++p.q == 4) {
            p.q = 0; ++p.item;
            if (++p.tw == a.tiles_w) {
                p.tw = 0;
                if (++p.tl * a.tiles_w >= a.n_tiles) { p.tl = 0; ++p.view; }
            }
        }
    };
    auto fetch = [&](auto buf_tag, const Pos &ps, const i32x8 &hd) {
        constexpr int B = decltype(buf_tag)::value;
        const int item = ps.item, q = ps.q, view = ps.view;
        const int flags = hd[0], n_slots = hd[1], cwid = hd[2], inv = hd[3], x0 = hd[4], t0 = hd[5], top_rows = hd[6], b0 = hd[7];
        if (wave < 3) {
            const unsigned char *src = a.recs + (size_t)item * kTileBoxes * kRecBytes + wave * 1024 + lane * 16;
            __builtin_amdgcn_global_load_lds((const __attribute__((address_space(1))) void *)src,
                                             (__attribute__((address_space(3))) void *)((B ? s_rec1 : s_rec0) + wave * 1024), 16, 0, 0);
        }
        if ((flags & kTileLive) && !(flags & kTileDirect)) {
            const char *img = reinterpret_cast<const char *>(a.integral) + view * img_stride + q * 256 + cq * 16;
            for (int s = 4 * wave; s < n_slots; s += 32) {
                const int sl = min(s + grp, n_slots - 1);
                const int wr = (sl * inv) >> 16, wc = sl - wr * cwid;
                const int y = wr < top_rows ? t0 + wr : b0 + (wr - top_rows), x = x0 + wc;
                const char *src = img + ((size_t)(y + 1) * Wp + (x + 1)) * kSlotBytes;
                __builtin_amdgcn_global_load_lds((const __attribute__((address_space(1))) void *)src,
                                                 (__attribute__((address_space(3))) void *)((B ? s_win1 : s_win0) + s * 16), 16, 0, 0);
            }
        }
    };
    float4 keep = make_float4(0.f, 0.f, 0.f, 0.f);
    float *keep_at = nullptr;
    auto flush = [&]() {
        if (keep_at) {
            typedef float nt4 __attribute__((ext_vector_type(4)));
            const nt4 x = {keep.x, keep.y, keep.z, keep.w};
            __builtin_nontemporal_store(x, reinterpret_cast<nt4 *>(keep_at));
        }
    };
    auto pool = [&](auto buf_tag, const Pos &ps, int flags) {
        constexpr int B = decltype(buf_tag)::value;
        const int q = ps.q, view = ps.view, tl = ps.tl, tw = ps.tw;
        if (flags & kTileDirect) {
            keep_at = nullptr;
            return;
        }
        const int b = 4 * wave + grp;
        const int cl = tl * kTileL + (b >> 3), cw = tw * kTileW + (b & 7);
        uint4 r[6];
        {
            const unsigned ra = (unsigned)(size_t)(__attribute__((address_space(3))) unsigned char *)(B ? s_rec1 : s_rec0) + (unsigned)(b * kRecBytes);
            asm volatile("ds_read_b128 %0, %6\n\tds_read_b128 %1, %6 offset:16\n\tds_read_b128 %2, %6 offset:32\n\t"
                         "ds_read_b128 %3, %6 offset:48\n\tds_read_b128 %4, %6 offset:64\n\tds_read_b128 %5, %6 offset:80\n\t"
                         "s_waitcnt lgkmcnt(0)"
                         : "=&v"(r[0]), "=&v"(r[1]), "=&v"(r[2]), "=&v"(r[3]), "=&v"(r[4]), "=&v"(r[5]) : "v"(ra) : "memory");
        }
        const float wt[16] = {__uint_as_float(r[0].x), __uint_as_float(r[0].y), __uint_as_float(r[0].z), __uint_as_float(r[0].w),
                              __uint_as_float(r[1].x), __uint_as_float(r[1].y), __uint_as_float(r[1].z), __uint_as_float(r[1].w),
                              __uint_as_float(r[2].x), __uint_as_float(r[2].y), __uint_as_float(r[2].z), __uint_as_float(r[2].w),
                              __uint_as_float(r[3].x), __uint_as_float(r[3].y), __uint_as_float(r[3].z), __uint_as_float(r[3].w)};
        const float rcp = __uint_as_float(r[4].x), masked = __uint_as_float(r[5].z), area = __uint_as_float(r[5].w);
        const bool vis = (r[4].y & (unsigned)kVis) != 0u;
        unsigned rws[4] = {r[4].z & 0xffffu, r[4].z >> 16, r[4].w & 0xffffu, r[4].w >> 16};
        unsigned cls[4] = {r[5].x & 0xffffu, r[5].x >> 16, r[5].y & 0xffffu, r[5].y >> 16};
#pragma unroll
        for (int k = 0; k < 4; ++k) {
            rws[k] = vis ? rws[k] : 0u;
            cls[k] = vis ? cls[k] : 0u;
        }
        typedef float nf4 __attribute__((ext_vector_type(4)));
        nf4 t[4][4];
        {
            const unsigned wa = (unsigned)(size_t)(__attribute__((address_space(3))) float4 *)(B ? s_win1 : s_win0) + (unsigned)(cq * 16);
            unsigned ad[4][4];
#pragma unroll
            for (int i = 0; i < 4; ++i)
#pragma unroll
                for (int j = 0; j < 4; ++j) ad[i][j] = wa + (rws[i] + cls[j]) * 256u;
#pragma unroll
            for (int i = 0; i < 4; i += 2)
                asm volatile("ds_read_b128 %0, %8\n\tds_read_b128 %1, %9\n\tds_read_b128 %2, %10\n\tds_read_b128 %3, %11\n\t"
                             "ds_read_b128 %4, %12\n\tds_read_b128 %5, %13\n\tds_read_b128 %6, %14\n\tds_read_b128 %7, %15"
                             : "=&v"(t[i][0]), "=&v"(t[i][1]), "=&v"(t[i][2]), "=&v"(t[i][3]), "=&v"(t[i + 1][0]), "=&v"(t[i + 1][1]),
                               "=&v"(t[i + 1][2]), "=&v"(t[i + 1][3])
                             : "v"(ad[i][0]), "v"(ad[i][1]), "v"(ad[i][2]), "v"(ad[i][3]), "v"(ad[i + 1][0]), "v"(ad[i + 1][1]),
                               "v"(ad[i + 1][2]), "v"(ad[i + 1][3])
                             : "memory");
            asm volatile("s_waitcnt lgkmcnt(0)"
                         : "+v"(t[0][0]), "+v"(t[0][1]), "+v"(t[0][2]), "+v"(t[0][3]), "+v"(t[1][0]), "+v"(t[1][1]), "+v"(t[1][2]), "+v"(t[1][3]),
                           "+v"(t[2][0]), "+v"(t[2][1]), "+v"(t[2][2]), "+v"(t[2][3]), "+v"(t[3][0]), "+v"(t[3][1]), "+v"(t[3][2]), "+v"(t[3][3])
                         :: "memory");
        }
        auto f4 = [](const nf4 &v) { return make_float4(v.x, v.y, v.z, v.w); };
        const float4 lt = sample4(f4(t[0][0]), f4(t[0][1]), f4(t[1][0]), f4(t[1][1]), wt[0], wt[1], wt[2], wt[3]);
        const float4 rb = sample4(f4(t[2][2]), f4(t[2][3]), f4(t[3][2]), f4(t[3][3]), wt[4], wt[5], wt[6], wt[7]);
        const float4 rt = sample4(f4(t[0][2]), f4(t[0][3]), f4(t[1][2]), f4(t[1][3]), wt[8], wt[9], wt[10], wt[11]);
        const float4 lb2 = sample4(f4(t[2][0]), f4(t[2][1]), f4(t[3][0]), f4(t[3][1]), wt[12], wt[13], wt[14], wt[15]);
        float4 res = make_float4(box_mean(lt.x, rb.x, rt.x, lb2.x, area, rcp), box_mean(lt.y, rb.y, rt.y, lb2.y, area, rcp),
                                 box_mean(lt.z, rb.z, rt.z, lb2.z, area, rcp), box_mean(lt.w, rb.w, rt.w, lb2.w, area, rcp));
        if (!vis) res = make_float4(masked, masked, masked, masked);
        const bool inside = cl < a.L && cw < a.W;
        keep = res;
        keep_at = inside ? a.vox + ((size_t)view * a.L * a.W + (size_t)cl * a.W + cw) * kC + q * 64 + cq * 4 : nullptr;
    };

    i32x8 hc, hn;
    header_of(u_begin, hc);
    header_wait(hc);
    Pos pc = pos_of(u_begin), pn = pc;
    fetch(std::integral_constant<int, 0>{}, pc, hc);
    advance(pn);
    if (u_begin + 1 < u_end) header_of(u_begin + 1, hn);
    for (long long u = u_begin; u < u_end; u += 2) {
        asm volatile("s_waitcnt vmcnt(0)" ::: "memory");
        __builtin_amdgcn_s_barrier();
        asm volatile("" ::: "memory");
        flush();
        if (u + 1 < u_end) {
            header_wait(hn);
            fetch(std::integral_constant<int, 1>{}, pn, hn);
        }
        pool(std::integral_constant<int, 0>{}, pc, hc[0]);
        if (u + 1 >= u_end) break;
        hc = hn;
        pc = pn;
        advance(pn);
        if (u + 2 < u_end) header_of(u + 2, hn);
        asm volatile("s_waitcnt vmcnt(0)" ::: "memory");
        __builtin_amdgcn_s_barrier();
        asm volatile("" ::: "memory");
        flush();
        if (u + 2 < u_end) {
            header_wait(hn);
            fetch(std::integral_constant<int, 0>{}, pn, hn);
        }
        pool(std::integral_constant<int, 1>{}, pc, hc[0]);
        hc = hn;
        pc = pn;
        advance(pn);
        if (u + 3 < u_end) header_of(u + 3, hn);
    }
    flush();
}

__global__ __launch_bounds__(512) void pool_direct_kernel(PoolArgs a)
{
    const int tid = threadIdx.x, wave = uniform_i(tid >> 6), lane = tid & 63, grp = lane >> 4, cq = lane & 15;
    const int tile = blockIdx.x >> 2, q = blockIdx.x & 3;
    unsigned mask = (unsigned)uniform_i((int)a.direct[tile]);
    if (a.n_views < 32) mask &= (1u << a.n_views) - 1u;
    const int tl = tile / a.tiles_w, tw = tile - tl * a.tiles_w;
    const int b = 4 * wave + grp;
    const int cl = tl * kTileL + (b >> 3), cw = tw * kTileW + (b & 7);
    const int Wp = a.Wf + 2;
    while (mask) {
        const int view = __builtin_ctz(mask);
        mask &= mask - 1u;
        const int item = view * a.n_tiles + tile;
        const uint4 *rp = reinterpret_cast<const uint4 *>(a.recs + ((size_t)item * kTileBoxes + b) * kRecBytes);
        uint4 r[6];
#pragma unroll
        for (int k = 0; k < 6; ++k) r[k] = rp[k];
        const float wt[16] = {__uint_as_float(r[0].x), __uint_as_float(r[0].y), __uint_as_float(r[0].z), __uint_as_float(r[0].w),
                              __uint_as_float(r[1].x), __uint_as_float(r[1].y), __uint_as_float(r[1].z), __uint_as_float(r[1].w),
                              __uint_as_float(r[2].x), __uint_as_float(r[2].y), __uint_as_float(r[2].z), __uint_as_float(r[2].w),
                              __uint_as_float(r[3].x), __uint_as_float(r[3].y), __uint_as_float(r[3].z), __uint_as_float(r[3].w)};
        const float rcp = __uint_as_float(r[4].x), masked = __uint_as_float(r[5].z), area = __uint_as_float(r[5].w);
        const bool vis = (r[4].y & (unsigned)kVis) != 0u;
        const unsigned rws[4] = {vis ? r[4].z & 0xffffu : 0u, vis ? r[4].z >> 16 : 0u, vis ? r[4].w & 0xffffu : 0u, vis ? r[4].w >> 16 : 0u};
        const unsigned cls[4] = {vis ? r[5].x & 0xffffu : 0u, vis ? r[5].x >> 16 : 0u, vis ? r[5].y & 0xffffu : 0u, vis ? r[5].y >> 16 : 0u};
        const char *img = reinterpret_cast<const char *>(a.integral) + (size_t)view * (a.Hf + 2) * Wp * kSlotBytes + q * 256 + cq * 16;
        float4 t[4][4];
#pragma unroll
        for (int i = 0; i < 4; ++i)
#pragma unroll
            for (int j = 0; j < 4; ++j) t[i][j] = *reinterpret_cast<const float4 *>(img + (size_t)(rws[i] * Wp + cls[j]) * kSlotBytes);
        __builtin_amdgcn_sched_barrier(0);
        const float4 lt = sample4(t[0][0], t[0][1], t[1][0], t[1][1], wt[0], wt[1], wt[2], wt[3]);
        const float4 rb = sample4(t[2][2], t[2][3], t[3][2], t[3][3], wt[4], wt[5], wt[6], wt[7]);
        const float4 rt = sample4(t[0][2], t[0][3], t[1][2], t[1][3], wt[8], wt[9], wt[10], wt[11]);
        const float4 lb2 = sample4(t[2][0], t[2][1], t[3][0], t[3][1], wt[12], wt[13], wt[14], wt[15]);
        float4 res = make_float4(box_mean(lt.x, rb.x, rt.x, lb2.x, area, rcp), box_mean(lt.y, rb.y, rt.y, lb2.y, area, rcp),
                                 box_mean(lt.z, rb.z, rt.z, lb2.z, area, rcp), box_mean(lt.w, rb.w, rt.w, lb2.w, area, rcp));
        if (!vis) res = make_float4(masked, masked, masked, masked);
        if (cl < a.L && cw < a.W) {
            typedef float nt4 __attribute__((ext_vector_type(4)));
            const nt4 x = {res.x, res.y, res.z, res.w};
            __builtin_nontemporal_store(x, reinterpret_cast<nt4 *>(a.vox + ((size_t)view * a.L * a.W + (size_t)cl * a.W + cw) * kC + q * 64 + cq * 4));
        }
    }
}

struct RowsArgs {
    const float *integral[kMaxScales];
    const unsigned char *recs[kMaxScales];
    int Hf[kMaxScales], Wf[kMaxScales];
    const unsigned *row_list;
    const unsigned *row_counter;
    float *rows;
    int n_tiles, rows_cap;
};
__global__ __launch_bounds__(512) void pool_rows_kernel(RowsArgs a)
{
    const int tid = threadIdx.x, wave = uniform_i(tid >> 6), lane = tid & 63, grp = lane >> 4, cq = lane & 15;
    const int count = min(uniform_i((int)*a.row_counter), a.rows_cap);
    const int b = 4 * wave + grp;
    for (int u = blockIdx.x; u < 4 * count; u += gridDim.x) {
        const int slot = u >> 2, q = u & 3;
        const unsigned e = (unsigned)uniform_i((int)a.row_list[slot]);
        const int s = (int)(e >> 30), view = (int)((e >> 25) & 31u), tile = (int)(e & 0x1ffffffu);
        const int Wp = a.Wf[s] + 2;
        const int item = view * a.n_tiles + tile;
        const uint4 *rp = reinterpret_cast<const uint4 *>(a.recs[s] + ((size_t)item * kTileBoxes + b) * kRecBytes);
        uint4 r[6];
#pragma unroll
        for (int k = 0; k < 6; ++k) r[k] = rp[k];
        const float wt[16] = {__uint_as_float(r[0].x), __uint_as_float(r[0].y), __uint_as_float(r[0].z), __uint_as_float(r[0].w),
                              __uint_as_float(r[1].x), __uint_as_float(r[1].y), __uint_as_float(r[1].z), __uint_as_float(r[1].w),
                              __uint_as_float(r[2].x), __uint_as_float(r[2].y), __uint_as_float(r[2].z), __uint_as_float(r[2].w),
                              __uint_as_float(r[3].x), __uint_as_float(r[3].y), __uint_as_float(r[3].z), __uint_as_float(r[3].w)};
        const float rcp = __uint_as_float(r[4].x), masked = __uint_as_float(r[5].z), area = __uint_as_float(r[5].w);
        const bool vis = (r[4].y & (unsigned)kVis) != 0u;
        const unsigned rws[4] = {vis ? r[4].z & 0xffffu : 0u, vis ? r[4].z >> 16 : 0u, vis ? r[4].w & 0xffffu : 0u, vis ? r[4].w >> 16 : 0u};
        const unsigned cls[4] = {vis ? r[5].x & 0xffffu : 0u, vis ? r[5].x >> 16 : 0u, vis ? r[5].y & 0xffffu : 0u, vis ? r[5].y >> 16 : 0u};
        const char *img = reinterpret_cast<const char *>(a.integral[s]) + (size_t)view * (a.Hf[s] + 2) * Wp * kSlotBytes + q * 256 + cq * 16;
        float4 t[4][4];
#pragma unroll
        for (int i = 0; i < 4; ++i)
#pragma unroll
            for (int j = 0; j < 4; ++j) t[i][j] = *reinterpret_cast<const float4 *>(img + (size_t)(rws[i] * Wp + cls[j]) * kSlotBytes);
        __builtin_amdgcn_sched_barrier(0);
        const float4 lt = sample4(t[0][0], t[0][1], t[1][0], t[1][1], wt[0], wt[1], wt[2], wt[3]);
        const float4 rb = sample4(t[2][2], t[2][3], t[3][2], t[3][3], wt[4], wt[5], wt[6], wt[7]);
        const float4 rt = sample4(t[0][2], t[0][3], t[1][2], t[1][3], wt[8], wt[9], wt[10], wt[11]);
        const float4 lb2 = sample4(t[2][0], t[2][1], t[3][0], t[3][1], wt[12], wt[13], wt[14], wt[15]);
        float4 res = make_float4(box_mean(lt.x, rb.x, rt.x, lb2.x, area, rcp), box_mean(lt.y, rb.y, rt.y, lb2.y, area, rcp),
                                 box_mean(lt.z, rb.z, rt.z, lb2.z, area, rcp), box_mean(lt.w, rb.w, rt.w, lb2.w, area, rcp));
        if (!vis) res = make_float4(masked, masked, masked, masked);
        reinterpret_cast<float4 *>(a.rows)[((size_t)slot * kTileBoxes + b) * (kC / 4) + q * 16 + cq] = res;
    }
}


struct WorkspaceLayout {
    size_t live[kMaxScales], direct[kMaxScales], overflow[kMaxScales], counter, hdrs[kMaxScales], recs[kMaxScales], wfrag[kMaxScales],
        masks_bytes, chunks, ranks, diag, rows, row_list, partial, tickets, item_w, wmax, wexp, amax, total;
    int tiles_l, tiles_w, n_tiles, rows_cap, views_pad;
};
inline WorkspaceLayout layout_of(int n_views, int L, int W, int n_scales)
{
    WorkspaceLayout w;
    w.tiles_l = (L + kTileL - 1) / kTileL;
    w.tiles_w = (W + kTileW - 1) / kTileW;
    w.n_tiles = w.tiles_l * w.tiles_w;
    size_t off = 0;
    for (int s = 0; s < kMaxScales; ++s) {
        const bool on = s < n_scales;
        w.live[s] = off;  off = align_up(off + (on ? (size_t)w.n_tiles * 4 : 0), 256);
        w.direct[s] = off; off = align_up(off + (on ? (size_t)w.n_tiles * 4 : 0), 256);
        w.overflow[s] = off; off = align_up(off + (on ? (size_t)w.n_tiles * 4 : 0), 256);
    }
    w.counter = off; off += 256;
    w.tickets = off; off = align_up(off + (size_t)w.n_tiles * sizeof(unsigned), 256);
    w.masks_bytes = off;
    for (int s = 0; s < kMaxScales; ++s) {
        const bool on = s < n_scales;
        w.hdrs[s] = off;  off = align_up(off + (on ? (size_t)n_views * w.n_tiles * kHdrBytes : 0), 256);
        w.recs[s] = off;  off = align_up(off + (on ? ((size_t)n_views * w.n_tiles * kTileBoxes + 1) * kRecBytes : 0), 256);
        w.wfrag[s] = off; off = align_up(off + (on ? (size_t)8 * kSteps * 2 * 64 * 16 : 0), 256);
    }
    w.chunks = off;
    off = align_up(off + (kChunks + 1) * sizeof(int), 256);
    w.ranks = off;
    off = align_up(off + (kChunks + 1) * sizeof(int), 256);
    w.partial = off;
    off = align_up(off + (size_t)kMaxBlocks * 2 * 8 * 16 * 64 * sizeof(float), 256);
    w.diag = off;
    off = align_up(off + 512 * 8 * sizeof(unsigned long long), 256);
    const size_t items = (size_t)n_views * w.n_tiles * n_scales;
    size_t cap = items / 4 + 64;
    if (cap > 8192) cap = 8192;
    if (items * (size_t)(kTileBoxes * kC * sizeof(float)) <= ((size_t)1 << 30)) cap = items;
    if (cap > items) cap = items;
    w.rows_cap = (int)cap;
    w.row_list = off;
    off = align_up(off + cap * sizeof(unsigned), 256);
    w.wmax = off; off = align_up(off + (size_t)kMaxScales * kWmaxParts * sizeof(unsigned), 256);
    w.wexp = off; off = align_up(off + (kMaxScales + 1) * sizeof(int), 256);
    w.amax = off; off = align_up(off + (size_t)kMaxScales * kFallbackStats * sizeof(unsigned), 256);
    w.views_pad = (n_views + 7) / 8 * 8;
    w.item_w = off;
    off = align_up(off + (size_t)w.n_tiles * kMaxScales * w.views_pad * sizeof(unsigned short) + 16, 256);
    w.rows = off;
    off = align_up(off + cap * kTileBoxes * kC * sizeof(float), 256);
    w.total = off;
    return w;
}

inline int rows_cap_of(const WorkspaceLayout &lay, size_t bytes)
{
    if (bytes <= lay.rows) return 0;
    const size_t fit = (bytes - lay.rows) / ((size_t)kTileBoxes * kC * sizeof(float));
    return fit < (size_t)lay.rows_cap ? (int)fit : lay.rows_cap;
}

}

extern "C" {

size_t vfa_frame_workspace_bytes(int n_views, int L, int W, int n_scales)
{
    if (n_views < 0 || L < 0 || W < 0 || n_scales < 1 || n_scales > kMaxScales) return 0;
    return layout_of(n_views, L, W, n_scales).total;
}

int vfa_frame_workspace_layout(int n_views, int L, int W, int n_scales, size_t *offsets, int *tiles)
{
    if (n_views < 0 || L < 0 || W < 0 || n_scales < 1 || n_scales > kMaxScales || !offsets || !tiles) return VFA_ERR_BAD_ARGUMENT;
    const WorkspaceLayout lay = layout_of(n_views, L, W, n_scales);
    for (int k = 0; k < kMaxScales; ++k) {
        offsets[5 * k + 0] = lay.live[k];
        offsets[5 * k + 1] = lay.direct[k];
        offsets[5 * k + 2] = lay.hdrs[k];
        offsets[5 * k + 3] = lay.recs[k];
        offsets[5 * k + 4] = lay.wfrag[k];
    }
    offsets[15] = lay.diag;
    offsets[16] = lay.total;
    for (int k = 0; k < kMaxScales; ++k) offsets[17 + k] = lay.overflow[k];
    offsets[20] = lay.counter;
    offsets[21] = lay.rows;
    offsets[22] = (size_t)lay.rows_cap;
    offsets[23] = lay.chunks;
    offsets[24] = lay.ranks;
    tiles[0] = lay.tiles_l;
    tiles[1] = lay.tiles_w;
    tiles[2] = kMaxSlots;
    tiles[3] = kChunks;
    return 0;
}

int vfa_frame_boxes_f32(const float *calibs, const float *grid, const float *z_layers, const float *corner_off, int n_views, int L,
                        int W, int conv_kind, float img_w, float img_h, float cmin, float cmax, int n_scales,
                        const int *feat_hw, void *workspace, size_t workspace_bytes, void *stream)
{
    if (n_views < 0 || L < 0 || W < 0 || n_scales < 1 || n_scales > kMaxScales || conv_kind < 0 || conv_kind > 2 || !feat_hw)
        return VFA_ERR_BAD_ARGUMENT;
    if (n_views > 32) return VFA_ERR_UNSUPPORTED;
    const WorkspaceLayout lay = layout_of(n_views, L, W, n_scales);
    if (lay.n_tiles == 0 || n_views == 0) return 0;
    if ((long long)n_views * lay.n_tiles >= (1ll << 31) - 2 || lay.n_tiles >= (1 << 25)) return VFA_ERR_UNSUPPORTED;
    if (!workspace || workspace_bytes < lay.rows) return VFA_ERR_BAD_ARGUMENT;
    hipStream_t s = (hipStream_t)stream;
    unsigned char *ws = reinterpret_cast<unsigned char *>(workspace);
    RecordArgs a;
    a.g = BoxGeom{calibs, grid, z_layers, corner_off, conv_kind, img_w, img_h, cmin, cmax};
    a.n_views = n_views; a.L = L; a.W = W; a.tiles_w = lay.tiles_w; a.n_tiles = lay.n_tiles; a.n_scales = n_scales;
    for (int k = 0; k < kMaxScales; ++k) {
        a.dims[k].Hf = k < n_scales ? feat_hw[2 * k] : 1;
        a.dims[k].Wf = k < n_scales ? feat_hw[2 * k + 1] : 1;
        if (a.dims[k].Hf <= 0 || a.dims[k].Wf <= 0 || a.dims[k].Hf > 65533 || a.dims[k].Wf > 65533) return VFA_ERR_BAD_ARGUMENT;
        a.live[k] = reinterpret_cast<unsigned *>(ws + lay.live[k]);
        a.direct[k] = reinterpret_cast<unsigned *>(ws + lay.direct[k]);
        a.overflow[k] = reinterpret_cast<unsigned *>(ws + lay.overflow[k]);
        a.hdrs[k] = ws + lay.hdrs[k];
        a.recs[k] = ws + lay.recs[k];
    }
    a.row_counter = reinterpret_cast<unsigned *>(ws + lay.counter);
    a.rows_cap = (unsigned)rows_cap_of(lay, workspace_bytes);
    a.row_list = reinterpret_cast<unsigned *>(ws + lay.row_list);
    a.item_w = reinterpret_cast<unsigned short *>(ws + lay.item_w);
    a.views_pad = lay.views_pad;
    const hipError_t e = zero_fill(ws, lay.masks_bytes, s);
    if (e != hipSuccess) return (int)e;
    const long long pairs = (long long)n_views * lay.n_tiles;
    hipLaunchKernelGGL(frame_records_kernel, dim3((unsigned)((pairs + 1) / 2)), dim3(kWave), 0, s, a);
    return (int)hipGetLastError();
}

int vfa_frame_cuts_f32(int n_views, int L, int W, int n_scales, const float *const *weights, int flags, void *workspace,
                       size_t workspace_bytes, void *stream)
{
    const int terms = flags & VFA_FLAG_TERMS_MASK;
    if ((flags & ~VFA_FLAG_TERMS_MASK) || (terms != 0 && terms != 2 && terms != 3 && terms != 4)) return VFA_ERR_BAD_ARGUMENT;
    if (n_views < 0 || L < 0 || W < 0 || n_scales < 1 || n_scales > kMaxScales) return VFA_ERR_BAD_ARGUMENT;
    if (n_views > 32) return VFA_ERR_UNSUPPORTED;
    const WorkspaceLayout lay = layout_of(n_views, L, W, n_scales);
    if (lay.n_tiles == 0 || n_views == 0) return 0;
    if (!workspace || workspace_bytes < lay.rows) return VFA_ERR_BAD_ARGUMENT;
    hipStream_t s = (hipStream_t)stream;
    unsigned char *ws = reinterpret_cast<unsigned char *>(workspace);
    ChunkArgs ca;
    for (int k = 0; k < kMaxScales; ++k) {
        const int q = k < n_scales ? k : 0;
        ca.live[k] = reinterpret_cast<const unsigned *>(ws + lay.live[q]);
        ca.overflow[k] = reinterpret_cast<const unsigned *>(ws + lay.overflow[q]);
    }
    ca.n_scales = n_scales; ca.n_tiles = lay.n_tiles; ca.n_views = n_views; ca.views_pad = lay.views_pad;
    ca.item_w = reinterpret_cast<const unsigned short *>(ws + lay.item_w);
    ca.chunk_start = reinterpret_cast<int *>(ws + lay.chunks);
    ca.chunk_rank = reinterpret_cast<int *>(ws + lay.ranks);
    ca.split = SplitArgs{};
    ca.n_split_blocks = 0;
    if (weights) {
        SplitArgs &sa = ca.split;
        for (int k = 0; k < kMaxScales; ++k) {
            sa.w[k] = weights[k < n_scales ? k : 0];
            sa.out[k] = reinterpret_cast<uint4 *>(ws + lay.wfrag[k < n_scales ? k : 0]);
            if (!sa.w[k]) return VFA_ERR_BAD_ARGUMENT;
        }
        sa.wmax = reinterpret_cast<unsigned *>(ws + lay.wmax);
        sa.wexp = reinterpret_cast<int *>(ws + lay.wexp);
        sa.f16 = (terms == 0 || terms == 2) ? 1 : 0;
        ca.n_split_blocks = n_scales * kSplitBlocks;
    }
    if (n_views <= 8) hipLaunchKernelGGL(tile_chunks_kernel<1>, dim3(1 + ca.n_split_blocks), dim3(1024), 0, s, ca);
    else hipLaunchKernelGGL(tile_chunks_kernel<4>, dim3(1 + ca.n_split_blocks), dim3(1024), 0, s, ca);
    return (int)hipGetLastError();
}

int vfa_frame_records_f32(const float *calibs, const float *grid, const float *z_layers, const float *corner_off, int n_views, int L,
                          int W, int conv_kind, float img_w, float img_h, float cmin, float cmax, int n_scales,
                          const int *feat_hw, const float *const *weights, int flags, void *workspace, size_t workspace_bytes, void *stream)
{
    const int st = vfa_frame_boxes_f32(calibs, grid, z_layers, corner_off, n_views, L, W, conv_kind, img_w, img_h, cmin, cmax, n_scales, feat_hw,
                                       workspace, workspace_bytes, stream);
    if (st) return st;
    return vfa_frame_cuts_f32(n_views, L, W, n_scales, weights, flags, workspace, workspace_bytes, stream);
}

int vfa_pool_windows_f32(const float *integral, const void *workspace, size_t workspace_bytes, float *vox, int n_views, int L, int W,
                         int n_scales, int scale, int Hf, int Wf, void *stream)
{
    if (n_views < 0 || L < 0 || W < 0 || n_scales < 1 || n_scales > kMaxScales || scale < 0 || scale >= n_scales || Hf <= 0 || Wf <= 0)
        return VFA_ERR_BAD_ARGUMENT;
    if (n_views > 32) return VFA_ERR_UNSUPPORTED;
    const WorkspaceLayout lay = layout_of(n_views, L, W, n_scales);
    if (lay.n_tiles == 0 || n_views == 0) return 0;
    if (!workspace || workspace_bytes < lay.rows || !integral || !vox) return VFA_ERR_BAD_ARGUMENT;
    const unsigned char *ws = reinterpret_cast<const unsigned char *>(workspace);
    PoolArgs a;
    a.integral = integral; a.hdrs = ws + lay.hdrs[scale]; a.recs = ws + lay.recs[scale]; a.vox = vox;
    a.direct = reinterpret_cast<const unsigned *>(ws + lay.direct[scale]);
    a.n_views = n_views; a.L = L; a.W = W; a.tiles_w = lay.tiles_w; a.n_tiles = lay.n_tiles; a.Hf = Hf; a.Wf = Wf;
    const long long units = (long long)n_views * lay.n_tiles * 4;
    if (units >= (1ll << 31) - 8) return VFA_ERR_UNSUPPORTED;
    a.per_xcd = 0;
    int n_cu = 256;
    {
        int dev = 0, cus = 0;
        if (hipGetDevice(&dev) == hipSuccess && hipDeviceGetAttribute(&cus, hipDeviceAttributeMultiprocessorCount, dev) == hipSuccess &&
            cus > 0)
            n_cu = cus;
    }
    long long nblk = 2ll * n_cu;
    if (nblk > units) nblk = units;
    nblk = (nblk + 7) / 8 * 8;
    hipLaunchKernelGGL(pool_windows_kernel, dim3((unsigned)nblk), dim3(512), 0, (hipStream_t)stream, a);
    int st = (int)hipGetLastError();
    if (st) return st;
    if ((long long)lay.n_tiles * 4 >= (1ll << 31)) return VFA_ERR_UNSUPPORTED;
    hipLaunchKernelGGL(pool_direct_kernel, dim3((unsigned)(lay.n_tiles * 4)), dim3(512), 0, (hipStream_t)stream, a);
    return (int)hipGetLastError();
}

int vfa_pool_collapse_relu_sum_f32(const float *const *integrals, const unsigned *const *feat_absmax, const float *const *biases,
                                   const void *workspace, size_t workspace_bytes, float *out, int n_views, int L, int W, int n_scales,
                                   const int *feat_hw, int accumulate, int flags, void *stream)
{
    const int terms = flags & VFA_FLAG_TERMS_MASK, reserved_cus = (flags >> 8) & 0xff;
    const int debug = ((flags >> 16) & 0xfff) | ((flags & VFA_FLAG_DUMP_VOX) ? kDbgDumpVox : 0);
    if (debug && terms != 0 && terms != 2) return VFA_ERR_BAD_ARGUMENT;
    if (flags & ~(VFA_FLAG_TERMS_MASK | 0xfffff00 | VFA_FLAG_ROWS_ONLY | VFA_FLAG_SKIP_ROWS | VFA_FLAG_DUMP_VOX)) return VFA_ERR_BAD_ARGUMENT;
    if ((flags & VFA_FLAG_ROWS_ONLY) && (flags & VFA_FLAG_SKIP_ROWS)) return VFA_ERR_BAD_ARGUMENT;
    if (n_views < 0 || L < 0 || W < 0 || n_scales < 1 || n_scales > kMaxScales || !feat_hw || !integrals ||
        (terms != 0 && terms != 2 && terms != 3 && terms != 4))
        return VFA_ERR_BAD_ARGUMENT;
    const bool f16 = terms == 0 || terms == 2;
    if (n_views > 32) return VFA_ERR_UNSUPPORTED;
    const WorkspaceLayout lay = layout_of(n_views, L, W, n_scales);
    if (lay.n_tiles == 0) return 0;
    hipStream_t s = (hipStream_t)stream;
    if (n_views == 0) {
        if (!accumulate) return (int)zero_fill(out, (size_t)L * W * kC * sizeof(float), s);
        return 0;
    }
    if (!workspace || workspace_bytes < lay.rows) return VFA_ERR_BAD_ARGUMENT;
    const unsigned char *ws = reinterpret_cast<const unsigned char *>(workspace);
    const int rows_cap = rows_cap_of(lay, workspace_bytes);
    FusedArgs a;
    for (int k = 0; k < kMaxScales; ++k) {
        const int q = k < n_scales ? k : 0;
        a.sc[k].integral = integrals[q];
        a.sc[k].bias = biases ? biases[q] : nullptr;
        a.sc[k].wfrag = reinterpret_cast<const uint4 *>(ws + lay.wfrag[q]);
        a.sc[k].live = reinterpret_cast<const unsigned *>(ws + lay.live[q]);
        a.sc[k].direct = reinterpret_cast<const unsigned *>(ws + lay.direct[q]);
        a.sc[k].overflow = reinterpret_cast<const unsigned *>(ws + lay.overflow[q]);
        a.sc[k].hdrs = ws + lay.hdrs[q];
        a.sc[k].recs = ws + lay.recs[q];
        a.sc[k].Hf = feat_hw[2 * q];
        a.sc[k].Wf = feat_hw[2 * q + 1];
        if (!a.sc[k].integral) return VFA_ERR_BAD_ARGUMENT;
        a.sc[k].amax = nullptr; a.sc[k].amax_n = 0;
    }
    if (f16 && !(flags & VFA_FLAG_ROWS_ONLY)) {
        for (int k = 0; k < n_scales; ++k) {
            if (feat_absmax && feat_absmax[k]) {
                a.sc[k].amax = feat_absmax[k];
                a.sc[k].amax_n = (int)feature_stats_count(n_views, kC, a.sc[k].Hf);
            } else {
                unsigned *dst = reinterpret_cast<unsigned *>(const_cast<unsigned char *>(ws) + lay.amax) + (size_t)k * kFallbackStats;
                const int st = integral_absmax_folded(a.sc[k].integral, dst, n_views, kC, a.sc[k].Hf, a.sc[k].Wf, kFallbackStats, &a.sc[k].amax_n, stream);
                if (st) return st;
                a.sc[k].amax = dst;
            }
        }
    }
    a.wexp = reinterpret_cast<const int *>(ws + lay.wexp);
    a.n_scales = n_scales; a.n_views = n_views; a.L = L; a.W = W; a.tiles_w = lay.tiles_w; a.n_tiles = lay.n_tiles;
    a.out = out; a.accumulate = accumulate;
    a.chunk_start = reinterpret_cast<const int *>(ws + lay.chunks);
    a.chunk_rank = reinterpret_cast<const int *>(ws + lay.ranks);
    a.partial = reinterpret_cast<float *>(const_cast<unsigned char *>(ws) + lay.partial);
    a.tickets = reinterpret_cast<unsigned *>(const_cast<unsigned char *>(ws) + lay.tickets);
    a.debug = debug;
    a.diag = reinterpret_cast<unsigned long long *>(const_cast<unsigned char *>(ws) + lay.diag);
    if (debug & kDbgDumpVox) {
        if (n_views != 1 || n_scales != 1 || accumulate || !out) return VFA_ERR_BAD_ARGUMENT;
        const hipError_t e = hipMemsetAsync(out, 0, (size_t)L * W * kC * sizeof(float), s);
        if (e != hipSuccess) return (int)e;
    }
    int n_cu = 256;
    {
        int dev = 0, cus = 0;
        if (hipGetDevice(&dev) == hipSuccess && hipDeviceGetAttribute(&cus, hipDeviceAttributeMultiprocessorCount, dev) == hipSuccess &&
            cus > 0)
            n_cu = cus;
    }
    if (reserved_cus > 0 && n_cu - reserved_cus >= 8) n_cu -= reserved_cus;
    int nblk = lay.n_tiles < n_cu ? lay.n_tiles : n_cu;
    nblk = (nblk + 7) / 8 * 8;
    if (nblk > kMaxBlocks) nblk = kMaxBlocks;
    a.rows = reinterpret_cast<const float *>(ws + lay.rows);
    a.row_counter = reinterpret_cast<const unsigned *>(ws + lay.counter);
    a.rows_cap = rows_cap;
    if (!(debug & 64) && !(flags & VFA_FLAG_SKIP_ROWS)) {
        RowsArgs ra;
        for (int k = 0; k < kMaxScales; ++k) {
            ra.integral[k] = a.sc[k].integral; ra.recs[k] = a.sc[k].recs;
            ra.Hf[k] = a.sc[k].Hf; ra.Wf[k] = a.sc[k].Wf;
        }
        ra.row_list = reinterpret_cast<const unsigned *>(ws + lay.row_list);
        ra.row_counter = a.row_counter;
        ra.rows = reinterpret_cast<float *>(const_cast<unsigned char *>(ws) + lay.rows);
        ra.n_tiles = lay.n_tiles; ra.rows_cap = rows_cap;
        hipLaunchKernelGGL(pool_rows_kernel, dim3(4096), dim3(512), 0, s, ra);
        const int st0 = (int)hipGetLastError();
        if (st0 || (flags & VFA_FLAG_ROWS_ONLY)) return st0;
    }
    if (debug & 64) {
        hipLaunchKernelGGL((pool_collapse_kernel<2, false, true>), dim3(nblk), dim3(kThreads), 0, s, a);
        return (int)hipGetLastError();
    }
    if (debug)
        hipLaunchKernelGGL((pool_collapse_kernel<2, true, false>), dim3(nblk), dim3(kThreads), 0, s, a);
    else if (terms == 4)
        hipLaunchKernelGGL((pool_collapse_kernel<4, false, false>), dim3(nblk), dim3(kThreads), 0, s, a);
    else if (terms == 3)
        hipLaunchKernelGGL((pool_collapse_kernel<3, false, false>), dim3(nblk), dim3(kThreads), 0, s, a);
    else
        hipLaunchKernelGGL((pool_collapse_kernel<2, false, false>), dim3(nblk), dim3(kThreads), 0, s, a);
    int st = (int)hipGetLastError();
    if (st || debug) return st;
    if ((size_t)rows_cap >= (size_t)n_views * lay.n_tiles * n_scales) return st;
    if (terms == 4)
        hipLaunchKernelGGL((pool_collapse_kernel<4, false, true>), dim3(nblk), dim3(kThreads), 0, s, a);
    else if (terms == 3)
        hipLaunchKernelGGL((pool_collapse_kernel<3, false, true>), dim3(nblk), dim3(kThreads), 0, s, a);
    else
        hipLaunchKernelGGL((pool_collapse_kernel<2, false, true>), dim3(nblk), dim3(kThreads), 0, s, a);
    return (int)hipGetLastError();
}

size_t vfa_sliver_shifts_scratch_bytes(int L, int W)
{
    if (L <= 0 || W <= 0) return 0;
    return ((size_t)((L + kTileL - 1) / kTileL) * ((W + kTileW - 1) / kTileW) * sizeof(unsigned) + 15) / 16 * 16;
}

int vfa_sliver_shifts_u8(const float *calibs, const float *grid, const float *z_layers, int n_layers, const float *corner_off, int n_views,
                         int L, int W, int conv_kind, float img_w, float img_h, float cmin, float cmax, int Hf, int Wf, int per_item,
                         unsigned char *shift, void *scratch, size_t scratch_bytes, void *stream)
{
    if (n_views < 0 || L < 0 || W < 0 || n_layers < 1 || Hf <= 0 || Wf <= 0 || conv_kind < 0 || conv_kind > 2 || !shift) return VFA_ERR_BAD_ARGUMENT;
    if (per_item && n_layers != 1) return VFA_ERR_BAD_ARGUMENT;
    if (n_views == 0 || L == 0 || W == 0) return 0;
    hipStream_t s = (hipStream_t)stream;
    ShiftArgs a;
    a.g = BoxGeom{calibs, grid, z_layers, corner_off, conv_kind, img_w, img_h, cmin, cmax};
    a.n_views = n_views; a.L = L; a.W = W; a.tiles_w = (W + kTileW - 1) / kTileW; a.n_tiles = ((L + kTileL - 1) / kTileL) * a.tiles_w;
    a.nl = n_layers; a.Hf = Hf; a.Wf = Wf; a.per_item = per_item ? 1 : 0;
    a.out = shift; a.tile_max = reinterpret_cast<unsigned *>(scratch);
    if (!per_item) {
        if (!scratch || scratch_bytes < vfa_sliver_shifts_scratch_bytes(L, W)) return VFA_ERR_BAD_ARGUMENT;
        const hipError_t e = zero_fill(scratch, vfa_sliver_shifts_scratch_bytes(L, W), s);
        if (e != hipSuccess) return (int)e;
    }
    const long long pairs = (long long)n_views * a.n_tiles;
    hipLaunchKernelGGL(sliver_shift_kernel, dim3((unsigned)((pairs + 1) / 2)), dim3(kWave), 0, s, a);
    if (!per_item) hipLaunchKernelGGL(sliver_expand_kernel, dim3((unsigned)((L * W + 255) / 256)), dim3(256), 0, s, a.tile_max, shift, L, W, a.tiles_w);
    return (int)hipGetLastError();
}

}
```

vfa_amd/ops.py:

```python
import os
import ctypes

import torch

from . import _lib


def _f32c(t):
    return t.to(dtype=torch.float32).contiguous()


class KernelTimer:
    active = None

    def __init__(self, only=None, every=1):
        self.records = []
        self.only = None if only is None else frozenset(only)
        self.every = max(int(every), 1)
        self.seen = {}

    def __enter__(self):
        KernelTimer.active = self
        return self

# ... 397 lines not shown
        key = (dev.index, _lib.current_stream(dev).cuda_stream)
        ws = _det_ws.get(key)
        if ws is None or ws.numel() < need:
            ws = _det_ws[key] = None
            ws = _det_ws[key] = torch.empty(max(need, 256), dtype=torch.uint8, device=dev)
        _launch("vfa_project_gather_backward_det_f32", _lib.ptr(grad_vox), _lib.ptr(calibs), _lib.ptr(grid_flat),
                _lib.ptr(z_layers), _lib.ptr(corner_off), _lib.ptr(out), n, C, Hp - 2, Wp - 2, nl, n_cells, cell_begin,
                cell_count, grid_w, int(conv_kind), float(image_wh[0]), float(image_wh[1]), float(crange[0]), float(crange[1]),
                (_lib.BWD_ACCUMULATE if accumulate else 0) | _lib.collapse_flags(0, reserved_cus), _lib.ptr(ws), need,
                _lib.current_stream_handle(), tag=(n, C, Hp - 2, Wp - 2, nl, cell_count))
        return out
    _launch("vfa_project_gather_backward_grid_f32", _lib.ptr(grad_vox), _lib.ptr(calibs), _lib.ptr(grid_flat),
            _lib.ptr(z_layers), _lib.ptr(corner_off), _lib.ptr(out), n, C, Hp - 2, Wp - 2, nl, n_cells, cell_begin,
            cell_count, grid_w, int(conv_kind), float(image_wh[0]), float(image_wh[1]), float(crange[0]), float(crange[1]),
            (_lib.BWD_ACCUMULATE if accumulate else 0) | (_lib.VOX_KERNEL_DIRECT if kernel == "direct" else 0),
            _lib.current_stream_handle())
    return out


def project_gather_backward_geometry(grad_vox, integral, calibs, grid_flat, z_layers, corner_off, conv_kind, image_wh,
                                     crange=(-1, 0.95), cell_begin=0, cell_count=None, grad_calibs=None, grad_grid=None, want_calibs=True,
                                     want_grid=True, accumulate=False):
    if integral.dim() != 4:
        raise ValueError(f"integral must be (n, Hf+2, Wf+2, C), got {tuple(integral.shape)}")
    n, Hp, Wp, C = integral.shape
    if Hp < 3 or Wp < 3:
        raise ValueError(f"integral must be zero-bordered (n, Hf+2, Wf+2, C), got {tuple(integral.shape)}")
    if tuple(calibs.shape) != (n, 12):
        raise ValueError(f"calibs must be ({n}, 12), got {tuple(calibs.shape)}")
    if grid_flat.dim() != 2 or grid_flat.shape[1] != 3:
        raise ValueError(f"grid_flat must be (n_cells, 3), got {tuple(grid_flat.shape)}")
    n_cells, nl = grid_flat.shape[0], z_layers.numel()
    cell_count = n_cells - cell_begin if cell_count is None else cell_count
    if cell_begin < 0 or cell_count < 0 or cell_begin + cell_count > n_cells:
        raise ValueError(f"cell range [{cell_begin}, {cell_begin + cell_count}) outside the {n_cells} cells")
    if tuple(grad_vox.shape) != (n, cell_count, nl * C):
        raise ValueError(f"grad_vox must be ({n}, {cell_count}, {nl * C}), got {tuple(grad_vox.shape)}")
    for name, t, shape in (("grad_calibs", grad_calibs, (n, 12)), ("grad_grid", grad_grid, (cell_count, 3))):
        if t is not None and (tuple(t.shape) != shape or t.dtype != torch.float32 or not t.is_contiguous()):
            raise ValueError(f"{name} must be a contiguous fp32 {shape}, got {tuple(t.shape)} {t.dtype}")
    _lib.require_device(grad_vox, integral, calibs, grid_flat, z_layers, corner_off, grad_calibs, grad_grid)
    dev = grad_vox.device
    if accumulate and ((grad_calibs is None and want_calibs) or (grad_grid is None and want_grid)):
        raise ValueError("accumulate=True adds into the outputs: pass every wanted one (grad_calibs / grad_grid), or want_*=False")
    if grad_calibs is None and want_calibs:
        grad_calibs = torch.empty((n, 12), dtype=torch.float32, device=dev)
    if grad_grid is None and want_grid:
        grad_grid = torch.empty((cell_count, 3), dtype=torch.float32, device=dev)
    if grad_calibs is None and grad_grid is None:
        return None, None
    acc = bool(accumulate)
    grad_vox, integral, calibs, grid_flat = _f32c(grad_vox), _f32c(integral), _f32c(calibs), _f32c(grid_flat)
    need = int(_lib.lib().vfa_gather_backward_geometry_workspace_bytes(n, cell_count)) if grad_calibs is not None else 0
    ws = torch.empty(max(need, 256), dtype=torch.uint8, device=dev) if need else None
    _launch("vfa_project_gather_backward_geometry_f32", _lib.ptr(grad_vox), _lib.ptr(integral), _lib.ptr(calibs),
            _lib.ptr(grid_flat), _lib.ptr(z_layers), _lib.ptr(corner_off), _lib.ptr(grad_calibs), _lib.ptr(grad_grid), n, C, Hp - 2,
            Wp - 2, nl, n_cells, cell_begin, cell_count, int(conv_kind), float(image_wh[0]), float(image_wh[1]), float(crange[0]),
            float(crange[1]), _lib.BWD_ACCUMULATE if acc else 0, _lib.ptr(ws), need, _lib.current_stream_handle(),
            tag=(n, C, Hp - 2, Wp - 2, nl, cell_count))
    return grad_calibs, grad_grid


def integral_image_backward(grad_integral):
    _lib.require_device(grad_integral)
    grad_integral = _f32c(grad_integral)
    n, Hp, Wp, C = grad_integral.shape
    grad_feature = torch.empty((n, C, Hp - 2, Wp - 2), dtype=torch.float32, device=grad_integral.device)
    _launch("vfa_integral_image_backward_f32", _lib.ptr(grad_integral), _lib.ptr(grad_feature), n, C, Hp - 2, Wp - 2,
            _lib.current_stream_handle())
    return grad_feature


def relu_mask_backward(grad, lin, bias, deterministic=None):
    _lib.require_device(grad, lin, bias)
    n, M, N = lin.shape
    grad = _f32c(grad)
    det = deterministic_mode(deterministic)
    if N % 4 != 0 or 1024 % N != 0:
        pre = lin if bias is None else lin + bias
        g = grad.unsqueeze(0) * (pre > 0)
        if bias is None:
            return g, None
        return g, (column_sum(g.reshape(n * M, N)) if det else g.sum(dim=(0, 1)))
    glin = torch.empty_like(lin)
    gbias = None if (bias is None or det) else torch.empty_like(bias)
    _launch("vfa_relu_mask_backward_f32", _lib.ptr(grad), _lib.ptr(lin), _lib.ptr(bias), _lib.ptr(glin), _lib.ptr(gbias),
            n, M, N, _lib.current_stream_handle())
    if det and bias is not None:
        gbias = column_sum(glin.view(n * M, N))
    return glin, gbias


COLUMN_SUM_WIDTH = 16384


def column_sum(x, out=None, accumulate=False):
    _lib.require_device(x, out)
    x = _f32c(x)
    rows, N = x.shape
    if out is None:
        out = torch.empty(N, dtype=torch.float32, device=x.device)
        accumulate = False
    assert tuple(out.shape) == (N,) and out.is_contiguous() and out.dtype == torch.float32
    B = COLUMN_SUM_WIDTH // N if N % 4 == 0 else 1
    if B >= 2 and rows >= 4 * B:
        head = rows // B * B
        part = torch.empty((B + rows - head, N), dtype=torch.float32, device=x.device)
        _launch("vfa_column_sum_f32", _lib.ptr(x), _lib.ptr(part), head // B, B * N, 0, _lib.current_stream_handle(), tag=(rows, N))
        part[B:] = x[head:]
        x, rows = part, part.shape[0]
    _launch("vfa_column_sum_f32", _lib.ptr(x), _lib.ptr(out), rows, N, 1 if accumulate else 0, _lib.current_stream_handle(),
            tag=(rows, N))
    return out


_grad_w_ws = {}


def grad_weight(g_lin, vox, out=None, accumulate=False):
    _lib.require_device(g_lin, vox, out)
    g_lin, vox = _f32c(g_lin), _f32c(vox)
    rows, K = vox.shape
    assert tuple(g_lin.shape) == (rows, 256) and K % 256 == 0
    dev = vox.device
    if out is None:
        out = torch.empty((256, K), dtype=torch.float32, device=dev)
        accumulate = False
    assert tuple(out.shape) == (256, K) and out.is_contiguous() and out.dtype == torch.float32
    need = _lib.lib().vfa_grad_weight_workspace_bytes(rows, K)
    key = (dev.index, _lib.current_stream(dev).cuda_stream)
    ws = _grad_w_ws.get(key)
    if ws is None or ws.numel() < need:
        ws = _grad_w_ws[key] = torch.empty(max(need, 8), dtype=torch.uint8, device=dev)
    _launch("vfa_grad_weight_f32", _lib.ptr(g_lin), _lib.ptr(vox), _lib.ptr(out), rows, K, 1 if accumulate else 0, _lib.ptr(ws),
            ws.numel(), _lib.current_stream_handle(), tag=(rows, K))
    return out


def grad_input(g_lin, w, out=None):
    _lib.require_device(g_lin, w, out)
    g_lin, w = _f32c(g_lin), _f32c(w)
    rows, K = g_lin.shape[0], w.shape[1]
    assert g_lin.shape[1] == 256 and w.shape[0] == 256 and K % 256 == 0
    dev = g_lin.device
    if out is None:
        out = torch.empty((rows, K), dtype=torch.float32, device=dev)
    assert tuple(out.shape) == (rows, K) and out.is_contiguous() and out.dtype == torch.float32
    need = _lib.lib().vfa_grad_input_workspace_bytes(K)
    key = (dev.index, _lib.current_stream(dev).cuda_stream, "x")
    ws = _grad_w_ws.get(key)
    if ws is None or ws.numel() < need:
        ws = _grad_w_ws[key] = torch.empty(max(need, 8), dtype=torch.uint8, device=dev)
    _launch("vfa_grad_input_f32", _lib.ptr(g_lin), _lib.ptr(w), _lib.ptr(out), rows, K, _lib.ptr(ws), ws.numel(),
            _lib.current_stream_handle(), tag=(rows, K))
    return out


def bias_relu_accumulate(lin, bias, out=None, accumulate=False):
    _lib.require_device(lin, bias, out)
    n, M, N = lin.shape
    if out is None:
        out = torch.empty((M, N), dtype=torch.float32, device=lin.device)
        accumulate = False
    _launch("vfa_bias_relu_accumulate_f32", _lib.ptr(lin), _lib.ptr(bias), _lib.ptr(out), n, M, N,
              1 if accumulate else 0, _lib.current_stream_handle())
    return out


def scale_view_sum(lin8, lin16, lin32, b8, b16, b32, out=None, accumulate=False):
    _lib.require_device(lin8, lin16, lin32, b8, b16, b32, out)
    n, M, N = lin8.shape
    if out is None:
        out = torch.empty((M, N), dtype=torch.float32, device=lin8.device)
        accumulate = False
    _launch("vfa_scale_view_sum_f32", _lib.ptr(lin8), _lib.ptr(lin16), _lib.ptr(lin32), _lib.ptr(b8), _lib.ptr(b16),
              _lib.ptr(b32), _lib.ptr(out), n, M, N, 1 if accumulate else 0, _lib.current_stream_handle())
    return out


MAX_VIEWS = 256


def scale_view_max(lin8, lin16, lin32, b8, b16, b32, out=None, want_argmax=True):
    _lib.require_device(lin8, lin16, lin32, b8, b16, b32, out)
    n, M, N = lin8.shape
    if tuple(lin16.shape) != (n, M, N) or tuple(lin32.shape) != (n, M, N):
        raise ValueError(f"scale_view_max: lin shapes differ: {tuple(lin8.shape)}, {tuple(lin16.shape)}, {tuple(lin32.shape)}")
    if n > MAX_VIEWS:
        raise ValueError(f"scale_view_max: {n} views, at most {MAX_VIEWS}")
    lin8, lin16, lin32 = _f32c(lin8), _f32c(lin16), _f32c(lin32)
    b8, b16, b32 = (None if b is None else _f32c(b) for b in (b8, b16, b32))
    if out is None:
        out = torch.empty((M, N), dtype=torch.float32, device=lin8.device)
    argmax = torch.empty((M, N), dtype=torch.uint8, device=lin8.device) if want_argmax else None
    _launch("vfa_scale_view_max_f32", _lib.ptr(lin8), _lib.ptr(lin16), _lib.ptr(lin32), _lib.ptr(b8), _lib.ptr(b16), _lib.ptr(b32),
            _lib.ptr(out), _lib.ptr(argmax), n, M, N, _lib.current_stream_handle(), tag=(n, M, N))
    return out, argmax


def scale_view_max_backward(grad, lin8, lin16, lin32, b8, b16, b32, argmax, want_bias=(True, True, True)):
    _lib.require_device(grad, lin8, lin16, lin32, b8, b16, b32, argmax)
    n, M, N = lin8.shape
    if tuple(argmax.shape) != (M, N) or argmax.dtype != torch.uint8:
        raise ValueError(f"scale_view_max_backward: argmax must be uint8 ({M}, {N}), got {tuple(argmax.shape)} {argmax.dtype}")
    grad, lin8, lin16, lin32, argmax = _f32c(grad), _f32c(lin8), _f32c(lin16), _f32c(lin32), argmax.contiguous()
    b8, b16, b32 = (None if b is None else _f32c(b) for b in (b8, b16, b32))
    glins = [torch.empty((n, M, N), dtype=torch.float32, device=lin8.device) for _ in range(3)]
    _launch("vfa_scale_view_max_backward_f32", _lib.ptr(grad), _lib.ptr(lin8), _lib.ptr(lin16), _lib.ptr(lin32), _lib.ptr(b8),
            _lib.ptr(b16), _lib.ptr(b32), _lib.ptr(argmax), *(_lib.ptr(g) for g in glins), None, None, None, n, M, N,
            _lib.current_stream_handle(), tag=(n, M, N))
    gbias = []
    for g, b, want in zip(glins, (b8, b16, b32), want_bias):
        gbias.append(column_sum(g.view(n * M, N)) if (b is not None and want) else None)
    return (*glins, *gbias)


def collapse_relu_sum(vox, weight, bias, out=None, accumulate=False, terms=0, reserved_cus=0):
    _lib.require_device(vox, weight, bias, out)
    vox, weight = _f32c(vox), _f32c(weight)
    bias = None if bias is None else _f32c(bias)
    n, M, K = vox.shape
    N = weight.shape[0]
    assert weight.shape == (N, K), (tuple(weight.shape), K)
    if out is None:
        out = torch.empty((M, N), dtype=torch.float32, device=vox.device)
        accumulate = False
    _launch("vfa_collapse_relu_sum_f32", _lib.ptr(vox), _lib.ptr(weight), _lib.ptr(bias),
            _lib.ptr(out), n, M, K, N, 1 if accumulate else 0, _lib.collapse_flags(terms, reserved_cus),
            _lib.current_stream_handle())
    return out


_gemm_ws = {}


def collapse_gemm(vox2d, weight, out=None, terms=0, reserved_cus=0):
    _lib.require_device(vox2d, weight, out)
    vox2d, weight = _f32c(vox2d), _f32c(weight)
    M, K = vox2d.shape
    N = weight.shape[0]
    assert weight.shape == (N, K), (tuple(weight.shape), K)
    if out is None:
        out = torch.empty((M, N), dtype=torch.float32, device=vox2d.device)
    need = _lib.lib().vfa_collapse_gemm_workspace_bytes(K, N)
    key = (vox2d.device.index, _lib.current_stream(vox2d.device).cuda_stream)
    ws = _gemm_ws.get(key)
    if ws is None or ws.numel() < need:
        ws = _gemm_ws[key] = torch.empty(max(need, 1), dtype=torch.uint8, device=vox2d.device)
    _launch("vfa_collapse_gemm_f32", _lib.ptr(vox2d), _lib.ptr(weight), _lib.ptr(out), _lib.ptr(ws), ws.numel(), M, K, N,
            _lib.collapse_flags(terms, reserved_cus), _lib.current_stream_handle(), tag=(M, K, N))
    return out


def collapse_gemm_relu_backward(vox, weight, bias, grad_out, terms=0, reserved_cus=0, absmax=None, shift=None, deterministic=None):
    _lib.require_device(vox, weight, bias, grad_out)
    det = deterministic_mode(deterministic)
    vox, weight, grad_out = _f32c(vox), _f32c(weight), _f32c(grad_out)
    n, cells, K = vox.shape
    assert tuple(weight.shape) == (256, K) and tuple(grad_out.shape) == (cells, 256)
    bias = None if bias is None else _f32c(bias)
    dev = vox.device
    glin = torch.empty((n, cells, 256), dtype=torch.float32, device=dev)
    gbias = None if det else torch.zeros(256, dtype=torch.float32, device=dev)
    need = _lib.lib().vfa_collapse_gemm_workspace_bytes(K, 256)
    key = (dev.index, _lib.current_stream(dev).cuda_stream)
    ws = _gemm_ws.get(key)
    if ws is None or ws.numel() < need:
        ws = _gemm_ws[key] = torch.empty(max(need, 1), dtype=torch.uint8, device=dev)
    if absmax is not None:
        _lib.require_device(absmax, shift)
        assert absmax.dtype == torch.int32 and absmax.is_contiguous()
        rows = tiles = None
        if shift is not None:
            assert shift.dtype == torch.uint8 and shift.shape[-1] == cells and shift.numel() in (cells, n * cells)
            rows = shift.reshape(-1, cells).expand(n, cells).contiguous().view(-1)
            pad = (-rows.numel()) % 128
            tiles = (torch.nn.functional.pad(rows, (0, pad)) if pad else rows).view(-1, 128).amax(dim=1).contiguous()
        _launch("vfa_collapse_gemm_relu_backward_f16_f32", _lib.ptr(vox), _lib.ptr(weight), _lib.ptr(bias) if bias is not None else None,
                _lib.ptr(grad_out), _lib.ptr(glin), _lib.ptr(gbias), _lib.ptr(ws), ws.numel(), n, cells, K, 256, _lib.ptr(absmax),
                absmax.numel(), _lib.ptr(rows) if rows is not None else None, _lib.ptr(tiles) if tiles is not None else None,
                _lib.collapse_flags(0, reserved_cus), _lib.current_stream_handle(), tag=(n, cells, K, "f16"))
    else:
        _launch("vfa_collapse_gemm_relu_backward_f32", _lib.ptr(vox), _lib.ptr(weight), _lib.ptr(bias) if bias is not None else None,
                _lib.ptr(grad_out), _lib.ptr(glin), _lib.ptr(gbias), _lib.ptr(ws), ws.numel(), n, cells, K, 256,
                _lib.collapse_flags(terms, reserved_cus), _lib.current_stream_handle(), tag=(n, cells, K))
    if det:
        gbias = column_sum(glin.view(n * cells, 256))
    return glin, gbias


def sliver_shifts(calibs, grid, z_layers, corner_off, conv_kind, image_wh, feat_hw, per_item, crange=(-1, 0.95)):
    calibs, grid, z_layers, corner_off = _geometry(calibs, grid, z_layers, corner_off)
    n, (L, W) = calibs.shape[0], grid.shape[:2]
    out = torch.empty((n if per_item else 1, L * W), dtype=torch.uint8, device=calibs.device)
    need = _lib.lib().vfa_sliver_shifts_scratch_bytes(L, W)
    scratch = torch.empty(max(need, 16), dtype=torch.uint8, device=calibs.device)
    _launch("vfa_sliver_shifts_u8", _lib.ptr(calibs), _lib.ptr(grid), _lib.ptr(z_layers), z_layers.numel(), _lib.ptr(corner_off), n, L, W,
            int(conv_kind), float(image_wh[0]), float(image_wh[1]), float(crange[0]), float(crange[1]), int(feat_hw[0]), int(feat_hw[1]),
            1 if per_item else 0, _lib.ptr(out), _lib.ptr(scratch), scratch.numel(), _lib.current_stream_handle(), tag=(n, L, W))
    return out


def frame_records(calibs, grid, z_layers, corner_off, conv_kind, image_wh, feat_hws, weights=None, crange=(-1, 0.95),
                  workspace=None, row_slots=None, cuts=True, terms=0):
    calibs, grid, z_layers, corner_off = _geometry(calibs, grid, z_layers, corner_off)
    n, (L, W) = calibs.shape[0], grid.shape[:2]
    if z_layers.numel() != 1:
        raise _lib.VFAHipError("frame_records / pool_collapse cover single-layer grids (nl = 1) only")
    ns = len(feat_hws)
    need = _lib.lib().vfa_frame_workspace_bytes(n, L, W, ns)
    if row_slots is not None:
        lay = frame_workspace_layout(n, L, W, ns)
        need = lay["rows"] + min(int(row_slots), lay["rows_cap"]) * 32 * 256 * 4
        workspace = None
    if workspace is None or workspace.numel() < need:
        workspace = torch.empty(max(need, 1), dtype=torch.uint8, device=calibs.device)
    hw = _lib.int_array([v for f in feat_hws for v in f])
    wts = _weight_ptrs(weights, ns, (256, 256))
    if not cuts:
        _launch("vfa_frame_boxes_f32", _lib.ptr(calibs), _lib.ptr(grid), _lib.ptr(z_layers), _lib.ptr(corner_off), n, L, W,
                int(conv_kind), float(image_wh[0]), float(image_wh[1]), float(crange[0]), float(crange[1]), ns, hw,
                _lib.ptr(workspace), workspace.numel(), _lib.current_stream_handle(), tag=(n, L, W, ns))
        return workspace
    _launch("vfa_frame_records_f32", _lib.ptr(calibs), _lib.ptr(grid), _lib.ptr(z_layers), _lib.ptr(corner_off), n, L, W,
            int(conv_kind), float(image_wh[0]), float(image_wh[1]), float(crange[0]), float(crange[1]), ns, hw, wts, int(terms) & 0xf,
            _lib.ptr(workspace), workspace.numel(), _lib.current_stream_handle(), tag=(n, L, W, ns))
    return workspace


def frame_cuts(workspace, n_views, grid_lw, n_scales, weights=None, terms=0):
    _lib.require_device(workspace)
    wts = _weight_ptrs(weights, n_scales, (256, 256))
    _launch("vfa_frame_cuts_f32", int(n_views), int(grid_lw[0]), int(grid_lw[1]), int(n_scales), wts, int(terms) & 0xf, _lib.ptr(workspace),
            workspace.numel(), _lib.current_stream_handle(), tag=(int(n_views), int(grid_lw[0]), int(grid_lw[1]), int(n_scales)))
    return workspace


def pool_collapse(integrals, biases, workspace, grid_lw, out=None, accumulate=False, terms=0, reserved_cus=0, debug=0, stage="all",
                  absmax=None, dump_vox=False):
    _lib.require_device(*integrals, workspace, out)
    stage_flag = {"all": 0, "rows": _lib.FLAG_ROWS_ONLY, "main": _lib.FLAG_SKIP_ROWS}[stage]
    ns = len(integrals)
    n = integrals[0].shape[0]
    L, W = grid_lw
    assert all(i.shape[0] == n and i.shape[3] == 256 and i.is_contiguous() and i.dtype == torch.float32 for i in integrals)
    if out is None and stage != "rows":
        out = torch.empty((L * W, 256), dtype=torch.float32, device=integrals[0].device)
        accumulate = False
    assert out is None or (out.dtype == torch.float32 and out.is_contiguous() and tuple(out.shape) == (L * W, 256)), \
        "out must be a contiguous fp32 (L*W, 256) tensor"
    biases = [None if b is None else _f32c(b) for b in (biases if biases is not None else [None] * ns)]
    hw = _lib.int_array([v for i in integrals for v in (i.shape[1] - 2, i.shape[2] - 2)])
    absmax, absmax_ptrs = _absmax_of(integrals, absmax)
    _launch("vfa_pool_collapse_relu_sum_f32", _lib.ptr_array(list(integrals)), absmax_ptrs, _lib.ptr_array(biases), _lib.ptr(workspace),
            workspace.numel(), _lib.ptr(out) if out is not None else None, n, L, W, ns, hw, 1 if accumulate else 0,
            _lib.collapse_flags(terms, reserved_cus) | ((int(debug) & 0xfff) << 16) | stage_flag | (_lib.FLAG_DUMP_VOX if dump_vox else 0),
            _lib.current_stream_handle(), tag=(n, L, W, tuple((i.shape[1] - 2, i.shape[2] - 2) for i in integrals), stage))
    return out


def pool_windows(integral, workspace, grid_lw, n_scales, scale, out=None):
    _lib.require_device(integral, workspace, out)
    n, Hp, Wp, C = integral.shape
    assert C == 256 and integral.is_contiguous() and integral.dtype == torch.float32
    L, W = grid_lw
    vox = out if out is not None else torch.empty((n, L * W, 256), dtype=torch.float32, device=integral.device)
    _launch("vfa_pool_windows_f32", _lib.ptr(integral), _lib.ptr(workspace), workspace.numel(), _lib.ptr(vox), n, L, W,
            int(n_scales), int(scale), Hp - 2, Wp - 2, _lib.current_stream_handle(), tag=(n, C, Hp - 2, Wp - 2, 1, L * W))
    return vox


def frame_workspace_layout(n_views, L, W, n_scales):
    import ctypes
    off = (ctypes.c_size_t * 25)()
    tiles = (ctypes.c_int * 4)()
    _lib.call("vfa_frame_workspace_layout", int(n_views), int(L), int(W), int(n_scales), off, tiles)
    names = ("live", "direct", "hdrs", "recs", "wfrag")
    out = {nm: [int(off[5 * k + i]) for k in range(n_scales)] for i, nm in enumerate(names)}
    out["overflow"] = [int(off[17 + k]) for k in range(n_scales)]
    out.update(diag=int(off[15]), total=int(off[16]), counter=int(off[20]), rows=int(off[21]), rows_cap=int(off[22]),
               chunks=int(off[23]), ranks=int(off[24]),
               tiles_l=int(tiles[0]), tiles_w=int(tiles[1]), max_slots=int(tiles[2]), n_chunks=int(tiles[3]))
    return out


def pipe_workspace_bytes(n_views, L, W, n_layers, n_scales):
    return int(_lib.lib().vfa_pipe_workspace_bytes(int(n_views), int(L), int(W), int(n_layers), int(n_scales)))


def pipe_records(calibs, grid, z_layers, corner_off, conv_kind, image_wh, feat_hws, weights=None, crange=(-1, 0.95), workspace=None,
                 cuts=True, terms=0):
    calibs, grid, z_layers, corner_off = _geometry(calibs, grid, z_layers, corner_off)
    n, (L, W) = calibs.shape[0], grid.shape[:2]
    nl, ns = z_layers.numel(), len(feat_hws)
    need = pipe_workspace_bytes(n, L, W, nl, ns)
    if workspace is None or workspace.numel() < need:
        workspace = torch.empty(max(need, 1), dtype=torch.uint8, device=calibs.device)
        if need > 0:
            bal = pipe_workspace_layout(n, L, W, nl, ns)["balance"]
            workspace[bal:bal + BALANCE_STATE_BYTES].zero_()
    hw = _lib.int_array([v for f in feat_hws for v in f])
    args = (_lib.ptr(calibs), _lib.ptr(grid), _lib.ptr(z_layers), nl, _lib.ptr(corner_off), n, L, W, int(conv_kind),
            float(image_wh[0]), float(image_wh[1]), float(crange[0]), float(crange[1]), ns, hw)
    if not cuts:
        _launch("vfa_pipe_boxes_f32", *args, int(terms) & 0xf, _lib.ptr(workspace), workspace.numel(), _lib.current_stream_handle(),
                tag=(n, L, W, nl, ns))
        return workspace
    wts = _weight_ptrs(weights, ns, (256, 256 * nl))
    _launch("vfa_pipe_records_f32", *args, wts, int(terms) & 0xf, _lib.ptr(workspace), workspace.numel(), _lib.current_stream_handle(),
            tag=(n, L, W, nl, ns))
    return workspace


def pipe_cuts(workspace, n_views, grid_lw, n_layers, n_scales, weights=None, terms=0):
    _lib.require_device(workspace)
    wts = _weight_ptrs(weights, n_scales, (256, 256 * n_layers))
    _launch("vfa_pipe_cuts_f32", int(n_views), int(grid_lw[0]), int(grid_lw[1]), int(n_layers), int(n_scales), wts, int(terms) & 0xf, _lib.ptr(workspace),
            workspace.numel(), _lib.current_stream_handle(), tag=(int(n_views), int(grid_lw[0]), int(grid_lw[1]), int(n_layers), int(n_scales)))
    return workspace


def pipe_collapse(integrals, biases, workspace, grid_lw, n_layers, out=None, accumulate=False, terms=0, reserved_cus=0, debug=0,
                  absmax=None, dump_vox=False):
    _lib.require_device(*integrals, workspace, out)
    ns = len(integrals)
    n = integrals[0].shape[0]
    L, W = grid_lw
    assert all(i.shape[0] == n and i.shape[3] == 256 and i.is_contiguous() and i.dtype == torch.float32 for i in integrals)
    if out is None:
        out = torch.empty((L * W, 256), dtype=torch.float32, device=integrals[0].device)
        accumulate = False
    assert out.dtype == torch.float32 and out.is_contiguous() and tuple(out.shape) == (L * W, 256)
    biases = [None if b is None else _f32c(b) for b in (biases if biases is not None else [None] * ns)]
    hw = _lib.int_array([v for i in integrals for v in (i.shape[1] - 2, i.shape[2] - 2)])
    absmax, absmax_ptrs = _absmax_of(integrals, absmax)
    _launch("vfa_pipe_collapse_relu_sum_f32", _lib.ptr_array(list(integrals)), absmax_ptrs, _lib.ptr_array(biases), _lib.ptr(workspace),
            workspace.numel(), _lib.ptr(out), n, L, W, int(n_layers), ns, hw, 1 if accumulate else 0,
            _lib.collapse_flags(terms, reserved_cus) | ((int(debug) & 0xfff) << 16) | (_lib.FLAG_DUMP_VOX if dump_vox else 0),
            _lib.current_stream_handle(), tag=(n, L, W, int(n_layers), tuple((i.shape[1] - 2, i.shape[2] - 2) for i in integrals)))
    return out


def pipe_balance(workspace, n_views, grid_lw, n_layers, n_scales, reserved_cus=0, reset=False):
    _lib.require_device(workspace)
    L, W = grid_lw
    _launch("vfa_pipe_balance_f32", int(n_views), int(L), int(W), int(n_layers), int(n_scales), int(reserved_cus), 0 if reset else 1,
            _lib.ptr(workspace), workspace.numel(), _lib.current_stream_handle())


BALANCE_STATE_BYTES = 8192


def pipe_workspace_layout(n_views, L, W, n_layers, n_scales):
    import ctypes
    off = (ctypes.c_size_t * 22)()
    tiles = (ctypes.c_int * 5)()
    _lib.call("vfa_pipe_workspace_layout", int(n_views), int(L), int(W), int(n_layers), int(n_scales), off, tiles)
    names = ("live", "hdrs", "recs", "wfrag")
    out = {nm: [int(off[4 * k + i]) for k in range(n_scales)] for i, nm in enumerate(names)}
    out.update(tickets=int(off[12]), globs=int(off[17]), chunks=int(off[13]), ranks=int(off[14]), diag=int(off[15]), total=int(off[16]),
               tiles_l=int(tiles[0]), tiles_w=int(tiles[1]), max_slots=int(tiles[2]), n_chunks=int(tiles[3]),
               max_slots_3piece=int(tiles[4]), balance=int(off[18]), shifts=[int(off[19 + k]) for k in range(n_scales)])
    return out


def pipe_batch_workspace_bytes(n_frames, n_views, L, W, n_layers, n_scales):
    return int(_lib.lib().vfa_pipe_batch_workspace_bytes(int(n_frames), int(n_views), int(L), int(W), int(n_layers), int(n_scales)))


def pipe_batch_workspace_layout(n_frames, n_views, L, W, n_layers, n_scales):
    off = (ctypes.c_size_t * 25)()
    tiles = (ctypes.c_int * 6)()
    _lib.call("vfa_pipe_batch_workspace_layout", int(n_frames), int(n_views), int(L), int(W), int(n_layers), int(n_scales), off, tiles)
    names = ("live", "hdrs", "recs", "wfrag")
    out = {nm: [int(off[4 * k + i]) for k in range(n_scales)] for i, nm in enumerate(names)}
    out.update(tickets=int(off[12]), globs=int(off[17]), chunks=int(off[13]), ranks=int(off[14]), diag=int(off[15]), total=int(off[16]),
               tiles_l=int(tiles[0]), tiles_w=int(tiles[1]), max_slots=int(tiles[2]), n_chunks=int(tiles[3]),
               max_slots_3piece=int(tiles[4]), balance=int(off[18]), shifts=[int(off[19 + k]) for k in range(n_scales)],
               meta=int(off[22]), frame_exp=int(off[23]), virtual_tiles=int(tiles[5]))
    return out


def pipe_batch_records(calibs, grid, z_layers, corner_off, conv_kind, image_wh, feat_hws, n_frames, weights=None, crange=(-1, 0.95),
                       workspace=None, terms=0):
    calibs, grid, z_layers, corner_off = _geometry(calibs, grid, z_layers, corner_off)
    n, (L, W) = calibs.shape[0], grid.shape[:2]
    nl, ns = z_layers.numel(), len(feat_hws)
    need = pipe_batch_workspace_bytes(n_frames, n, L, W, nl, ns)
    if workspace is None:
        workspace = torch.empty(max(need, 1), dtype=torch.uint8, device=calibs.device)
        if need > 0:
            bal = pipe_batch_workspace_layout(n_frames, n, L, W, nl, ns)["balance"]
            workspace[bal:bal + BALANCE_STATE_BYTES].zero_()
    wts = _weight_ptrs(weights, ns, (256, 256 * nl))
    hw = _lib.int_array([v for f in feat_hws for v in f])
    _launch("vfa_pipe_batch_records_f32", _lib.ptr(calibs), _lib.ptr(grid), _lib.ptr(z_layers), nl, _lib.ptr(corner_off), n, L, W,
            int(conv_kind), float(image_wh[0]), float(image_wh[1]), float(crange[0]), float(crange[1]), ns, hw, wts, int(n_frames),
            int(terms) & 0xf, _lib.ptr(workspace), workspace.numel(), _lib.current_stream_handle(), tag=(int(n_frames), n, L, W, nl, ns))
    return workspace


def pipe_batch_collapse(integrals, biases, workspace, n_frames, grid_lw, n_layers, out=None, accumulate=False, terms=0, reserved_cus=0,
                        debug=0, absmax=None, dump_vox=False):
    _lib.require_device(*integrals, workspace, out)
    ns, B = len(integrals), int(n_frames)
    L, W = grid_lw
    if B < 1 or integrals[0].shape[0] % B:
        raise ValueError(f"pipe_batch_collapse: {integrals[0].shape[0]} integral images are not {B} frames of equal camera count")
    n = integrals[0].shape[0] // B
    assert all(i.shape[0] == B * n and i.shape[3] == 256 and i.is_contiguous() and i.dtype == torch.float32 for i in integrals)
    if out is None:
        out = torch.empty((B, L * W, 256), dtype=torch.float32, device=integrals[0].device)
        accumulate = False
    assert out.dtype == torch.float32 and out.is_contiguous() and tuple(out.shape) == (B, L * W, 256)
    biases = [None if b is None else _f32c(b) for b in (biases if biases is not None else [None] * ns)]
    hw = _lib.int_array([v for i in integrals for v in (i.shape[1] - 2, i.shape[2] - 2)])
    absmax, absmax_ptrs = _absmax_of(integrals, absmax)
    _launch("vfa_pipe_batch_collapse_relu_sum_f32", _lib.ptr_array(list(integrals)), absmax_ptrs, _lib.ptr_array(biases),
            _lib.ptr(workspace), workspace.numel(), _lib.ptr(out), B, n, L, W, int(n_layers), ns, hw, 1 if accumulate else 0,
            _lib.collapse_flags(terms, reserved_cus) | ((int(debug) & 0xfff) << 16) | (_lib.FLAG_DUMP_VOX if dump_vox else 0),
            _lib.current_stream_handle(), tag=(B, n, L, W, int(n_layers), tuple((i.shape[1] - 2, i.shape[2] - 2) for i in integrals)))
    return out


def pipe_batch_balance(workspace, n_frames, n_views, grid_lw, n_layers, n_scales, reserved_cus=0, reset=False):
    _lib.require_device(workspace)
    L, W = grid_lw
    _launch("vfa_pipe_batch_balance_f32", int(n_frames), int(n_views), int(L), int(W), int(n_layers), int(n_scales), int(reserved_cus),
            0 if reset else 1, _lib.ptr(workspace), workspace.numel(), _lib.current_stream_handle())
```

vfa_amd/vfa_op.py:

```python
import os

import numpy as np
import torch
import torch.nn as nn

from . import _lib, lazy, ops
from .utils import project

EPSILON = 1e-6
MAXIMUM_AREA_RATIO = 0.3

VOX_BYTES_LIMIT = int(os.environ.get("VFA_AMD_VOX_BYTES", str(8 << 30)))
USE_FUSED = os.environ.get("VFA_AMD_FUSED", "0") == "1"
COLLAPSE_KERNEL = os.environ.get("VFA_AMD_COLLAPSE", "mfma_bf16")
COLLAPSE_TERMS = int(os.environ.get("VFA_AMD_COLLAPSE_TERMS", "2"))
FUSED_POOL = os.environ.get("VFA_AMD_FUSED_POOL", "1") == "1"
WINDOW_POOL = os.environ.get("VFA_AMD_WINDOW_POOL", "1") == "1"


def _conv_kind(args):
    name = getattr(args, "data", None)
    if name not in _lib.CONV_KIND:
        raise UnboundLocalError(f"local variable 'coord' referenced before assignment (args.data={name!r} is not one "
                                f"of {sorted(_lib.CONV_KIND)})")
    return _lib.CONV_KIND[name]


class _IntegralImage(torch.autograd.Function):

    @staticmethod
    def forward(ctx, feature):
        return ops.integral_image(feature)

    @staticmethod
    def backward(ctx, grad_integral):
        return ops.integral_image_backward(grad_integral.clone())


class _BoxPool(torch.autograd.Function):

    @staticmethod
    def forward(ctx, integral, calibs, grid_flat, z_layers, corner_off, geom, cell_begin, cell_count):
        conv_kind, img_w, img_h, cmin, cmax = geom[:5]
        vox = ops.project_gather(integral, calibs, grid_flat, z_layers, corner_off, conv_kind, (img_w, img_h),
                                 (cmin, cmax), cell_begin, cell_count, _lib.VOX_LAYER_MAJOR)
        geometry = ctx.needs_input_grad[1] or ctx.needs_input_grad[2]
        ctx.save_for_backward(calibs, grid_flat, z_layers, corner_off, *((integral,) if geometry else ()))
        ctx.meta = (geom, tuple(integral.shape), cell_begin, cell_count)
        return vox

    @staticmethod
    def backward(ctx, grad_vox):
        calibs, grid_flat, z_layers, corner_off = ctx.saved_tensors[:4]
        geom, shape, cell_begin, cell_count = ctx.meta
        conv_kind, img_w, img_h, cmin, cmax = geom[:5]
        need_cal, need_grid = ctx.needs_input_grad[1], ctx.needs_input_grad[2]
        grad_integral = g_cal = g_grid = None
        if ctx.needs_input_grad[0] or not (need_cal or need_grid):
            grad_integral = ops.project_gather_backward(grad_vox, shape, calibs, grid_flat, z_layers, corner_off, conv_kind,
                                                        (img_w, img_h), (cmin, cmax), cell_begin, cell_count,
                                                        grid_w=geom[5] if len(geom) > 5 else 0)
        if need_cal or need_grid:
            g_cal, g_cells = ops.project_gather_backward_geometry(grad_vox, ctx.saved_tensors[4], calibs, grid_flat, z_layers, corner_off,
                                                                  conv_kind, (img_w, img_h), (cmin, cmax), cell_begin, cell_count,
                                                                  want_calibs=need_cal, want_grid=need_grid)
            if need_grid:
                g_grid = torch.zeros(grid_flat.shape, dtype=torch.float32, device=grid_flat.device)
                g_grid[cell_begin:cell_begin + cell_count] = g_cells
        return grad_integral, g_cal, g_grid, None, None, None, None, None


class _CollapseGemm(torch.autograd.Function):

    @staticmethod
    def forward(ctx, vox2d, weight, reserved_cus=0):
        ctx.save_for_backward(vox2d, weight)
        return ops.collapse_gemm(vox2d, weight, terms=_unfused_terms(), reserved_cus=reserved_cus)

    @staticmethod
    def backward(ctx, grad):
        vox2d, weight = ctx.saved_tensors
        grad = grad.contiguous()
        hand = grad.shape[1] == 256 and weight.shape[0] == 256 and weight.shape[1] % 256 == 0 and grad.shape[0] > 0
        g_vox = g_w = None
        if ctx.needs_input_grad[0]:
            g_vox = ops.grad_input(grad, weight) if hand else torch.matmul(grad, weight)
        if ctx.needs_input_grad[1]:
            g_w = ops.grad_weight(grad, vox2d) if hand else torch.matmul(grad.t(), vox2d)
        return g_vox, g_w, None


SIDE_STREAM = os.environ.get("VFA_AMD_SIDE_STREAM", "1") == "1"
_side_streams = {}


def _side_stream(dev):
    key = (dev.type, dev.index if dev.index is not None else torch.cuda.current_device())
    if key not in _side_streams:
        _side_streams[key] = torch.cuda.Stream(device=dev, priority=-1)
    return _side_streams[key]


def _fused_terms():
    return 2 if COLLAPSE_TERMS in (0, 2, 6) else COLLAPSE_TERMS


def _unfused_terms(terms=None):
    terms = COLLAPSE_TERMS if terms is None else terms
    return 3 if terms in (0, 2, 6) else terms


def _one_frame_module_set(mods, n_views):
    m0 = mods[0]
    return (1 <= len(mods) <= 3 and 0 < n_views <= 32
            and all(m.channel == 256 and m.collapse.out_features == 256 and m.num_grid_layer == m0.num_grid_layer
                    and m.geometry_key == m0.geometry_key and getattr(m.args, "data", None) == getattr(m0.args, "data", None)
                    and tuple(m.args.image_size) == tuple(m0.args.image_size) for m in mods))


def fused_frame_ok(mods, n_views, mode="fused"):
    on = FUSED_POOL if mode == "fused" else (WINDOW_POOL and not FUSED_POOL)
    return bool(on and COLLAPSE_KERNEL != "library" and _one_frame_module_set(mods, n_views) and mods[0].num_grid_layer == 1)


def fused_frame(mods, features, calibs, grid, crange=(-1, 0.95), out=None, accumulate=False, reserved_cus=0, integrals=None):
    if integrals is not None:
        features = [i.permute(0, 3, 1, 2)[:, :, 1:-1, 1:-1] for i in integrals]
    _lib.require_device(calibs, grid, *features)
    m0 = mods[0]
    conv_kind = _conv_kind(m0.args)
    img_h, img_w = (float(v) for v in m0.args.image_size)
    length, width = grid.shape[-3], grid.shape[-2]
    dev = features[0].device
    z_layers, corner_off = m0._kernel_geometry(dev)
    with torch.no_grad():
        cur = _lib.current_stream(dev)
        side = _side_stream(dev) if SIDE_STREAM and integrals is None and not torch.cuda.is_current_stream_capturing() else cur
        weights = [m.layer_major_weight() for m in mods]
        ws = torch.empty(max(_lib.lib().vfa_frame_workspace_bytes(calibs.shape[0], length, width, len(mods)), 1),
                         dtype=torch.uint8, device=dev)
        side.wait_stream(cur)
        feat_hws = [tuple(f.shape[-2:]) for f in features]
        if side is cur:
            ops.frame_records(calibs, grid, z_layers, corner_off, conv_kind, (img_w, img_h), feat_hws, weights=weights,
                              crange=crange, workspace=ws, terms=_fused_terms())
            boxes_done = None
        else:
            with torch.cuda.stream(side):
                ops.frame_records(calibs, grid, z_layers, corner_off, conv_kind, (img_w, img_h), feat_hws, crange=crange,
                                  workspace=ws, cuts=False)
                boxes_done = torch.cuda.Event()
                boxes_done.record(side)
                ops.frame_cuts(ws, calibs.shape[0], (length, width), len(mods), weights=weights, terms=_fused_terms())
        if integrals is None:
            integrals = ops.integral_images(features)
        biases = [m.collapse.bias for m in mods]
        if boxes_done is None:
            return ops.pool_collapse(integrals, biases, ws, (length, width), out=out, accumulate=accumulate, terms=_fused_terms(),
                                     reserved_cus=reserved_cus)
        cur.wait_event(boxes_done)
        ops.pool_collapse(integrals, biases, ws, (length, width), terms=_fused_terms(), reserved_cus=reserved_cus, stage="rows")
        cur.wait_stream(side)
        return ops.pool_collapse(integrals, biases, ws, (length, width), out=out, accumulate=accumulate, terms=_fused_terms(),
                                 reserved_cus=reserved_cus, stage="main")


PIPE = os.environ.get("VFA_AMD_PIPE", "1") == "1"
PIPE_SINGLE_LAYER = os.environ.get("VFA_AMD_PIPE_SINGLE_LAYER", "0") == "1"
PIPE_WS_LIMIT = int(os.environ.get("VFA_AMD_PIPE_WS_BYTES", str(3 << 30)))


def pipe_frame_ok(mods, n_views, tensors=()):
    if not (PIPE and COLLAPSE_KERNEL != "library" and _one_frame_module_set(mods, n_views)):
        return False
    if mods[0].num_grid_layer == 1 and not PIPE_SINGLE_LAYER:
        return False
    if not torch.is_grad_enabled():
        return True
    params = [p for m in mods for p in (m.collapse.weight, m.collapse.bias)] + [t for t in tensors if t is not None]
    return not any(p.requires_grad for p in params)


def pipe_frame(mods, features, calibs, grid, crange=(-1, 0.95), out=None, accumulate=False, reserved_cus=0, integrals=None,
               terms=None):
    terms = COLLAPSE_TERMS if terms is None else int(terms)
    if integrals is not None:
        features = [i.permute(0, 3, 1, 2)[:, :, 1:-1, 1:-1] for i in integrals]
    _lib.require_device(calibs, grid, *features)
    m0 = mods[0]
    conv_kind = _conv_kind(m0.args)
    img_h, img_w = (float(v) for v in m0.args.image_size)
    if grid.dim() < 3:
        raise ValueError("pipe_frame needs the grid as (L, W, 3) or (1, L, W, 3): the tiles follow its rows and columns")
    grid = grid.reshape(grid.shape[-3], grid.shape[-2], 3)
    length, width = grid.shape[0], grid.shape[1]
    dev = features[0].device
    n, nl, ns = calibs.shape[0], m0.num_grid_layer, len(mods)
    z_layers, corner_off = m0._kernel_geometry(dev)
    if out is None:
        out = torch.empty((length * width, 256), dtype=torch.float32, device=dev)
        accumulate = False
    if out.dtype != torch.float32 or not out.is_contiguous() or tuple(out.shape) != (length * width, 256):
        raise ValueError("pipe_frame: out must be a contiguous fp32 (L*W, 256) tensor")
    if length * width == 0:
        return out
    feat_hws = [tuple(f.shape[-2:]) for f in features]
    rows = length
    while rows > 4 and ops.pipe_workspace_bytes(n, rows, width, nl, ns) > PIPE_WS_LIMIT:
        rows = max(4, ((rows + 1) // 2 + 3) // 4 * 4)
    with torch.no_grad():
        cur = _lib.current_stream(dev)
        side = _side_stream(dev) if SIDE_STREAM and integrals is None and not torch.cuda.is_current_stream_capturing() else cur
        weights = [m.collapse.weight for m in mods]
        biases = [m.collapse.bias for m in mods]
        band_rows = min(rows, length)
        n_bands = (length + rows - 1) // rows
        st = _pipe_state(dev, (n, length, width, band_rows, nl, ns, terms, int(reserved_cus), conv_kind, tuple(feat_hws)),
                         ops.pipe_workspace_bytes(n, band_rows, width, nl, ns), n_bands)
        ws = st["ws"]
        balancing = PIPE_BALANCE and st["frames"] == 0 and not torch.cuda.is_current_stream_capturing()
        for b, r0 in enumerate(range(0, length, rows)):
            r1 = min(length, r0 + rows)
            band = grid[r0:r1]
            if side is not cur:
                side.wait_stream(cur)
            with torch.cuda.stream(side):
                ops.pipe_records(calibs, band, z_layers, corner_off, conv_kind, (img_w, img_h), feat_hws, weights=weights,
                                 crange=crange, workspace=ws, terms=terms)
            if integrals is None:
                integrals = ops.integral_images(features)
            if side is not cur:
                cur.wait_stream(side)
            if n_bands > 1:
                bal_off = st["balance_off"] if r1 - r0 == band_rows else ops.pipe_workspace_layout(n, r1 - r0, width, nl, ns)["balance"]
                ws[bal_off:bal_off + ops.BALANCE_STATE_BYTES].copy_(st["bands"][b], non_blocking=True)
            if balancing:
                ops.pipe_balance(ws, n, (r1 - r0, width), nl, ns, reserved_cus=reserved_cus)
                if n_bands > 1:
                    st["bands"][b].copy_(ws[bal_off:bal_off + ops.BALANCE_STATE_BYTES], non_blocking=True)
            ops.pipe_collapse(integrals, biases, ws, (r1 - r0, width), nl, out=out[r0 * width:r1 * width], accumulate=accumulate,
                              terms=terms, reserved_cus=reserved_cus)
        st["frames"] += 1
        if side is not cur:
            ws.record_stream(side)
    return out


def pipe_frames_ok(mods, n_views, tensors=()):
    if not (PIPE and COLLAPSE_KERNEL != "library" and _one_frame_module_set(mods, n_views)):
        return False
    if not torch.is_grad_enabled():
        return True
    params = [p for m in mods for p in (m.collapse.weight, m.collapse.bias)] + [t for t in tensors if t is not None]
    return not any(p.requires_grad for p in params)


def pipe_frames(mods, features, calibs, grid, n_frames, crange=(-1, 0.95), out=None, accumulate=False, reserved_cus=0, integrals=None,
                terms=None):
    terms = COLLAPSE_TERMS if terms is None else int(terms)
    B = int(n_frames)
    if integrals is not None:
        features = [i.permute(0, 3, 1, 2)[:, :, 1:-1, 1:-1] for i in integrals]
    _lib.require_device(calibs, grid, *features)
    m0 = mods[0]
    conv_kind = _conv_kind(m0.args)
    img_h, img_w = (float(v) for v in m0.args.image_size)
    if grid.dim() < 3:
        raise ValueError("pipe_frames needs the grid as (L, W, 3) or (1, L, W, 3): the tiles follow its rows and columns")
    if calibs.dim() != 3:
        raise ValueError(f"pipe_frames takes one rig for the whole batch: calibs (n, 3, 4), got {tuple(calibs.shape)}")
    grid = grid.reshape(grid.shape[-3], grid.shape[-2], 3)
    length, width = grid.shape[0], grid.shape[1]
    dev = features[0].device
    n, nl, ns = calibs.shape[0], m0.num_grid_layer, len(mods)
    if B < 0 or any(f.shape[0] != B * n for f in features):
        raise ValueError(f"pipe_frames: every scale needs {B} x {n} maps (frame-major), got {[tuple(f.shape) for f in features]}")
    if out is None:
        out = torch.empty((B, length * width, 256), dtype=torch.float32, device=dev)
        accumulate = False
    if out.dtype != torch.float32 or not out.is_contiguous() or tuple(out.shape) != (B, length * width, 256):
        raise ValueError("pipe_frames: out must be a contiguous fp32 (B, L*W, 256) tensor")
    if B == 0 or length * width == 0:
        return out
    z_layers, corner_off = m0._kernel_geometry(dev)
    feat_hws = [tuple(f.shape[-2:]) for f in features]
    rows = length
    while rows > 4 and ops.pipe_batch_workspace_bytes(B, n, rows, width, nl, ns) > PIPE_WS_LIMIT:
        rows = max(4, ((rows + 1) // 2 + 3) // 4 * 4)
    with torch.no_grad():
        cur = _lib.current_stream(dev)
        side = _side_stream(dev) if SIDE_STREAM and integrals is None and not torch.cuda.is_current_stream_capturing() else cur
        weights = [m.collapse.weight for m in mods]
        biases = [m.collapse.bias for m in mods]
        band_rows = min(rows, length)
        n_bands = (length + rows - 1) // rows
        st = _pipe_state(dev, ("frames", B, n, length, width, band_rows, nl, ns, terms, int(reserved_cus), conv_kind, tuple(feat_hws)),
                         ops.pipe_batch_workspace_bytes(B, n, band_rows, width, nl, ns), n_bands,
                         layout=lambda: ops.pipe_batch_workspace_layout(B, n, band_rows, width, nl, ns))
        ws_full = st["ws"]
        balancing = PIPE_BALANCE and st["frames"] == 0 and not torch.cuda.is_current_stream_capturing()
        for b, r0 in enumerate(range(0, length, rows)):
            r1 = min(length, r0 + rows)
            band = grid[r0:r1]
            ws = ws_full if r1 - r0 == band_rows else ws_full[:ops.pipe_batch_workspace_bytes(B, n, r1 - r0, width, nl, ns)]
            if side is not cur:
                side.wait_stream(cur)
            with torch.cuda.stream(side):
                ops.pipe_batch_records(calibs, band, z_layers, corner_off, conv_kind, (img_w, img_h), feat_hws, B, weights=weights,
                                       crange=crange, workspace=ws, terms=terms)
            if integrals is None:
                integrals = ops.integral_images(features)
            if side is not cur:
                cur.wait_stream(side)
            if n_bands > 1:
                bal_off = (st["balance_off"] if r1 - r0 == band_rows
                           else ops.pipe_batch_workspace_layout(B, n, r1 - r0, width, nl, ns)["balance"])
                ws[bal_off:bal_off + ops.BALANCE_STATE_BYTES].copy_(st["bands"][b], non_blocking=True)
            if balancing:
                ops.pipe_batch_balance(ws, B, n, (r1 - r0, width), nl, ns, reserved_cus=reserved_cus)
                if n_bands > 1:
                    st["bands"][b].copy_(ws[bal_off:bal_off + ops.BALANCE_STATE_BYTES], non_blocking=True)
            if n_bands == 1:
                ops.pipe_batch_collapse(integrals, biases, ws, B, (length, width), nl, out=out, accumulate=accumulate, terms=terms,
                                        reserved_cus=reserved_cus)
            else:
                part = ops.pipe_batch_collapse(integrals, biases, ws, B, (r1 - r0, width), nl, terms=terms, reserved_cus=reserved_cus)
                if accumulate:
                    out[:, r0 * width:r1 * width] += part
                else:
                    out[:, r0 * width:r1 * width] = part
        st["frames"] += 1
        if side is not cur:
            ws_full.record_stream(side)
    return out


PIPE_BALANCE = os.environ.get("VFA_AMD_PIPE_BALANCE", "1") == "1"
PIPE_STATES_KEPT = int(os.environ.get("VFA_AMD_PIPE_STATES", "8"))
_pipe_states = {}
_pipe_pinned = []
_capture_owner = None


class owned_capture_states:

    def __init__(self):
        self.states = []

    def __enter__(self):
        global _capture_owner
        self._outer, _capture_owner = _capture_owner, self
        return self

    def __exit__(self, *exc):
        global _capture_owner
        _capture_owner = self._outer
        return False


def _pipe_state(dev, key, ws_bytes, n_bands, layout=None):
    key = (dev.index, _lib.current_stream(dev).cuda_stream) + key
    capturing = torch.cuda.is_current_stream_capturing()
    if capturing and _capture_owner is not None:
        for st in _capture_owner.states:
            if st["key"] == key:
                return st
    st = _pipe_states.pop(key, None)
    if st is None and capturing:
        for k2 in list(_pipe_states):
            if k2[0] == key[0] and k2[2:] == key[2:] and _pipe_states[k2]["frames"] > 0:
                st = _pipe_states.pop(k2)
                break
    if st is None:
        ws = torch.empty(max(ws_bytes, 1), dtype=torch.uint8, device=dev)
        lay = layout() if layout is not None else ops.pipe_workspace_layout(key[2], key[5], key[4], key[6], key[7])
        st = {"ws": ws, "frames": 0, "balance_off": lay["balance"],
              "bands": [torch.zeros(ops.BALANCE_STATE_BYTES, dtype=torch.uint8, device=dev) for _ in range(n_bands)] if n_bands > 1 else None}
        ws[lay["balance"]:lay["balance"] + ops.BALANCE_STATE_BYTES].zero_()
    if capturing:
        st["pinned"] = True
        st["key"] = key
        (_capture_owner.states if _capture_owner is not None else _pipe_pinned).append(st)
        return st
    _pipe_states[key] = st
    while len(_pipe_states) > PIPE_STATES_KEPT:
        _pipe_states.pop(next(iter(_pipe_states)))
    return st


FUSED_TRAIN = os.environ.get("VFA_AMD_FUSED_TRAIN", "1") == "1"


def _frame_kernels_cover(mods, n_views):
    return COLLAPSE_KERNEL != "library" and _one_frame_module_set(mods, n_views)


class _FusedFrameTrain(torch.autograd.Function):

    @staticmethod
    def forward(ctx, calibs, grid, crange, meta, reserved_cus, *tensors):
        mods, from_integrals = meta
        ns = len(mods)
        lats, weights, biases = tensors[:ns], tensors[ns:2 * ns], tensors[2 * ns:3 * ns]
        n = calibs.shape[0]
        with torch.no_grad():
            if from_integrals:
                integrals = ops.IntegralImages(l.detach() for l in lats)
                integrals.absmax = list(tensors[3 * ns:4 * ns])
            else:
                integrals = ops.integral_images([l.detach() for l in lats])
            piped = pipe_frame_ok(mods, n)
            frame = pipe_frame if piped else fused_frame
            out = frame(mods, None, calibs, grid, crange, reserved_cus=reserved_cus, integrals=integrals)
        f16 = (COLLAPSE_TERMS if piped else _fused_terms()) in (0, 2)
        ctx.save_for_backward(calibs, grid, *integrals, *weights, *biases, *(integrals.absmax if f16 else ()))
        ctx.meta = (mods, tuple(float(c) for c in crange), piped, f16, from_integrals)
        return out

    @staticmethod
    def backward(ctx, grad_out):
        mods, crange, piped, f16, from_integrals = ctx.meta
        ns = len(mods)
        calibs, grid = ctx.saved_tensors[:2]
        integrals = ctx.saved_tensors[2:2 + ns]
        weights = ctx.saved_tensors[2 + ns:2 + 2 * ns]
        biases = ctx.saved_tensors[2 + 2 * ns:2 + 3 * ns]
        stats = ctx.saved_tensors[2 + 3 * ns:2 + 4 * ns] if f16 else (None,) * ns
        m0 = mods[0]
        conv_kind = _conv_kind(m0.args)
        img_h, img_w = (float(v) for v in m0.args.image_size)
        n = calibs.shape[0]
        dev = grad_out.device
        grid_flat = grid.reshape(-1, 3).to(dtype=torch.float32).contiguous()
        cal = calibs.reshape(n, 12).to(dtype=torch.float32).contiguous()
        z_layers, corner_off = m0._kernel_geometry(dev)
        n_cells, nl, C = grid_flat.shape[0], m0.num_grid_layer, 256
        grad_out = grad_out.contiguous()
        g_lats, g_ws, g_bs = [], [], []
        need_cal, need_grid = ctx.needs_input_grad[0], ctx.needs_input_grad[1]
        need_geo = need_cal or need_grid
        g_cal = torch.zeros((n, 12), dtype=torch.float32, device=dev) if need_cal else None
        g_grid = torch.zeros((n_cells, 3), dtype=torch.float32, device=dev) if need_grid else None
        with torch.no_grad():
            for k, (m, integral, w, b, stat) in enumerate(zip(mods, integrals, weights, biases, stats)):
                need_lat, need_w, need_b = ctx.needs_input_grad[5 + k], ctx.needs_input_grad[5 + ns + k], ctx.needs_input_grad[5 + 2 * ns + k]
                if not (need_lat or need_w or need_b or need_geo):
                    g_lats.append(None), g_ws.append(None), g_bs.append(None)
                    continue
                w_lm = w.view(C, C, nl).permute(0, 2, 1).reshape(C, nl * C).contiguous()
                g_int = torch.zeros_like(integral) if need_lat else None
                g_w_lm = torch.zeros_like(w_lm) if need_w else None
                g_b = torch.zeros_like(b) if need_b else None
                per_cell = n * nl * C * 4 * 2
                if need_lat and ops.deterministic_mode():
                    per_cell += -(-ops.det_workspace_bytes(n, nl, 1024, C, integral.shape[1] - 2, integral.shape[2] - 2) // 1024)
                chunk = max(1, min(n_cells, VOX_BYTES_LIMIT // max(per_cell, 1)))
                shifts = None
                if stat is not None and grid.dim() >= 3:
                    shifts = ops.sliver_shifts(cal, grid, z_layers, corner_off, conv_kind, (img_w, img_h),
# ... 442 lines not shown
```

Before: 1.532 billion voxels/s.

## Let fused pool workers compute their own direct rows and parallelize chunk cutting

Adds an opt-in OWN_ROWS mode in which each pool_collapse worker computes the direct-row box means for its own assigned items, instead of running a separate rows stage. The chunk partitioner now charges extra cost for direct items. Unconditionally, the chunk-cut kernel is spread over 8 blocks using a per-tile summed weight gathered with atomics in frame_records, and tile prefix weights come from masks rather than full item walks. The OWN_ROWS path is off by default behind an env var, so the default flow keeps the side-stream rows stage while still getting the new cut kernel and the extra atomicAdd per tile.

```diff
diff --git a/include/vfa_hip.h b/include/vfa_hip.h
--- a/include/vfa_hip.h
+++ b/include/vfa_hip.h
@@ -31,6 +31,7 @@
 #define VFA_FLAG_DUMP_VOX (1 << 30)
 #define VFA_FLAG_ROWS_ONLY (1 << 28)
 #define VFA_FLAG_SKIP_ROWS (1 << 29)
+#define VFA_FLAG_OWN_ROWS (1 << 4)
 #define VFA_BWD_ACCUMULATE 1
 
 int vfa_integral_image_f32(const float *feature, float *integral, int n_views, int C, int Hf, int Wf,
diff --git a/vfa_amd/_lib.py b/vfa_amd/_lib.py
--- a/vfa_amd/_lib.py
+++ b/vfa_amd/_lib.py
@@ -12,6 +12,7 @@
 
 
 FLAG_ROWS_ONLY, FLAG_SKIP_ROWS = 1 << 28, 1 << 29
+FLAG_OWN_ROWS = 1 << 4
 FLAG_DUMP_VOX = 1 << 30
 
 
diff --git a/vfa_amd/csrc/vfa_fused.hip b/vfa_amd/csrc/vfa_fused.hip
--- a/vfa_amd/csrc/vfa_fused.hip
+++ b/vfa_amd/csrc/vfa_fused.hip
@@ -41,6 +41,7 @@
     unsigned char *hdrs[kMaxScales];
     unsigned char *recs[kMaxScales];
     unsigned short *item_w;
+    unsigned *tile_w;
     int views_pad;
 };
 
@@ -53,6 +54,7 @@
 
     float l, t, r, bt;
     cube_box(a.g, a.g.calibs + (size_t)view * 12, ln.cell, 0, l, t, r, bt);
+    unsigned cost_sum = 0;
 #pragma unroll 1
     for (int s = 0; s < a.n_scales; ++s) {
         const int Hf = a.dims[s].Hf, Wf = a.dims[s].Wf;
@@ -114,8 +116,9 @@
                     else atomicOr(a.overflow[s] + tile, 1u << view);
                 }
                 const bool main_item = any_live && !(direct && !(hflags & kTileRows));
-                a.item_w[((size_t)tile * kMaxScales + s) * a.views_pad + view] =
-                    (unsigned short)(!main_item ? 0u : (direct ? kRowItemCost : kItemCost + (unsigned)n_slots));
+                const unsigned cost = !main_item ? 0u : (direct ? kRowItemCost : kItemCost + (unsigned)n_slots);
+                a.item_w[((size_t)tile * kMaxScales + s) * a.views_pad + view] = (unsigned short)cost;
+                cost_sum += cost;
                 hdr[0] = tile_header0(hflags, win, word2);
                 hdr[1] = tile_header1(win);
             }
@@ -124,6 +127,7 @@
         if (blockIdx.x == 0 && lane < 6)
             reinterpret_cast<uint4 *>(a.recs[s] + (size_t)a.n_views * a.n_tiles * kTileBoxes * kRecBytes)[lane] = make_uint4(0u, 0u, 0u, 0u);
     }
+    if (pair_ok && b == 0 && cost_sum) atomicAdd(a.tile_w + tile, cost_sum);
 }
 
 struct ShiftArgs {
@@ -208,55 +212,77 @@
 
 struct ChunkArgs {
     const unsigned *live[kMaxScales], *overflow[kMaxScales];
+    const unsigned *direct[kMaxScales];
     const unsigned short *item_w;
+    const unsigned *tile_w;
+    unsigned own_cost;
     int n_scales, n_tiles, n_views, views_pad;
     int *chunk_start, *chunk_rank;
     SplitArgs split;
     int n_split_blocks;
 };
-template <int G> struct TileItemsT { unsigned m[kMaxScales]; uint4 q[kMaxScales][G]; };
+template <int G> struct TileItemsT { unsigned m[kMaxScales], d[kMaxScales]; uint4 q[kMaxScales][G]; };
+constexpr int kCutBlocks = 8;
+constexpr unsigned kOwnRowCost = 625;
 template <int G>
 __global__ __launch_bounds__(1024) void tile_chunks_kernel(ChunkArgs a)
 {
     using TileItems = TileItemsT<G>;
-    constexpr bool kCache = G == 1;
     __shared__ unsigned long long part[1024];
-    if (blockIdx.x > 0) {
-        split_block(a.split, (int)blockIdx.x - 1, part);
+    if (blockIdx.x >= kCutBlocks) {
+        split_block(a.split, (int)blockIdx.x - kCutBlocks, part);
         return;
     }
+    const int c_lo = kChunks * (int)blockIdx.x / kCutBlocks, c_hi = kChunks * ((int)blockIdx.x + 1) / kCutBlocks;
     const int tid = threadIdx.x, n_tiles = a.n_tiles;
     const unsigned view_mask = a.n_views >= 32 ? 0xffffffffu : ((1u << a.n_views) - 1u);
     const int per = (n_tiles + 1023) / 1024, t0 = min(n_tiles, tid * per), t1 = min(n_tiles, t0 + per);
     constexpr unsigned kScale = 294, kTile = 330, kEmpty = 32;
-    struct RawTile { unsigned lv[kMaxScales], ov[kMaxScales]; uint4 q[kMaxScales][G]; };
-    auto load_raw = [&](int t) {
-        RawTile rt;
+    struct RawMasks { unsigned lv[kMaxScales], ov[kMaxScales], dr[kMaxScales], sum; };
+    struct Masks { unsigned m[kMaxScales], d[kMaxScales], sum; };
+    auto load_masks = [&](int t) {
+        RawMasks rm;
+#pragma unroll
+        for (int s = 0; s < kMaxScales; ++s) {
+            const int q = s < a.n_scales ? s : 0;
+            rm.lv[s] = a.live[q][t]; rm.ov[s] = a.overflow[q][t]; rm.dr[s] = a.direct[q][t];
+        }
+        rm.sum = a.tile_w[t];
+        return rm;
+    };
+    auto finish_masks = [&](const RawMasks &rm) {
+        Masks mk;
+#pragma unroll
+        for (int s = 0; s < kMaxScales; ++s) {
+            mk.m[s] = s < a.n_scales ? rm.lv[s] & ~rm.ov[s] & view_mask : 0u;
+            mk.d[s] = mk.m[s] & rm.dr[s];
+        }
+        mk.sum = rm.sum;
+        return mk;
+    };
+    auto weight_of = [&](const Masks &mk) -> unsigned {
+        unsigned w = mk.sum;
+        bool any = false;
+#pragma unroll
+        for (int s = 0; s < kMaxScales; ++s)
+            if (mk.m[s]) { w += kScale + a.own_cost * (unsigned)__popc(mk.d[s]); any = true; }
+        return any ? w + kTile : kEmpty;
+    };
+    auto load_tile = [&](const Masks &mk, int t) {
+        TileItems ti;
 #pragma unroll
         for (int s = 0; s < kMaxScales; ++s) {
             const bool on = s < a.n_scales;
-            const unsigned *lp = on ? a.live[s] : a.live[0], *op = on ? a.overflow[s] : a.overflow[0];
-            rt.lv[s] = lp[t]; rt.ov[s] = op[t];
+            ti.m[s] = mk.m[s]; ti.d[s] = mk.d[s];
 #pragma unroll
             for (int g = 0; g < G; ++g) {
                 const int gg = g * 8 < a.n_views ? g : 0;
-                rt.q[s][g] = *reinterpret_cast<const uint4 *>(a.item_w + ((size_t)t * kMaxScales + (on ? s : 0)) * a.views_pad + 8 * gg);
-            }
-        }
-        return rt;
-    };
-    auto finish_tile = [&](const RawTile &rt) {
-        TileItems ti;
-#pragma unroll
-        for (int s = 0; s < kMaxScales; ++s) {
-            const bool on = s < a.n_scales;
-            ti.m[s] = on ? rt.lv[s] & ~rt.ov[s] & view_mask : 0u;
-#pragma unroll
-            for (int g = 0; g < G; ++g) ti.q[s][g] = (!on || g * 8 >= a.n_views) ? make_uint4(0u, 0u, 0u, 0u) : rt.q[s][g];
+                const uint4 q = *reinterpret_cast<const uint4 *>(a.item_w + ((size_t)t * kMaxScales + (on ? s : 0)) * a.views_pad + 8 * gg);
+                ti.q[s][g] = (!on || g * 8 >= a.n_views) ? make_uint4(0u, 0u, 0u, 0u) : q;
+            }
         }
         return ti;
     };
-    auto load_tile = [&](int t) { return finish_tile(load_raw(t)); };
     auto walk = [&](const TileItems &ti, auto &&visit) -> unsigned {
         unsigned w = 0;
         int k = 0;
@@ -272,6 +298,7 @@
                     const int v = __builtin_ctz(mg);
                     mg &= mg - 1u;
                     unsigned wi = (unsigned)(((v < 4 ? lo : hi) >> (16 * (v & 3))) & 0xffffull);
+                    if ((ti.d[s] >> (8 * g + v)) & 1u) wi += a.own_cost;
                     if (first) wi += kScale;
                     if (k == 0) wi += kTile;
                     first = false;
@@ -283,18 +310,19 @@
         }
         return k == 0 ? kEmpty : w;
     };
-    TileItems c0 = {}, c1 = {};
-    if (kCache && n_tiles > 0) {
-        const RawTile r0 = load_raw(min(t0, n_tiles - 1)), r1 = load_raw(min(t0 + 1, n_tiles - 1));
+    Masks c0 = {}, c1 = {};
+    if (n_tiles > 0) {
+        const RawMasks r0 = load_masks(min(t0, n_tiles - 1)), r1 = load_masks(min(t0 + 1, n_tiles - 1));
         __builtin_amdgcn_sched_barrier(0);
-        c0 = finish_tile(r0);
-        c1 = finish_tile(r1);
-    }
-    auto tile_of = [&](int t) { return (kCache && t == t0) ? c0 : (kCache && t == t0 + 1) ? c1 : load_tile(t); };
+        c0 = finish_masks(r0);
+        c1 = finish_masks(r1);
+    }
+    auto masks_of = [&](int t) { return t == t0 ? c0 : t == t0 + 1 ? c1 : finish_masks(load_masks(t)); };
     unsigned long long local = 0;
-    for (int t = t0; t < t1; ++t) local += walk(tile_of(t), [](int, unsigned, unsigned) {});
+    for (int t = t0; t < t1; ++t) local += weight_of(masks_of(t));
     part[tid] = local;
-    for (int c = tid; c <= kChunks; c += 1024) { a.chunk_start[c] = n_tiles; a.chunk_rank[c] = 0; }
+    for (int c = c_lo + tid; c < c_hi; c += 1024) { a.chunk_start[c] = n_tiles; a.chunk_rank[c] = 0; }
+    if (c_hi == kChunks && tid == 0) { a.chunk_start[kChunks] = n_tiles; a.chunk_rank[kChunks] = 0; }
     __syncthreads();
     for (int d = 1; d < 1024; d <<= 1) {
         const unsigned long long v = tid >= d ? part[tid - d] : 0ull;
@@ -305,26 +333,33 @@
     const unsigned long long total = part[1023];
     unsigned long long before = part[tid] - local;
     auto pos_of = [&](long long cc) { return (total * (unsigned long long)cc + kChunks - 1) / kChunks; };
+    auto put = [&](long long c, int t, int k) {
+        if (c >= c_lo && c < c_hi) { a.chunk_start[c] = t; a.chunk_rank[c] = k; }
+    };
     for (int t = t0; t < t1; ++t) {
+        const Masks mk = masks_of(t);
         const unsigned long long tb = before;
+        const unsigned w = weight_of(mk);
+        before += w;
         long long c = tb > 0 ? (long long)((tb - 1) * kChunks / total) : 0;
         while (c < kChunks && pos_of(c) < tb) ++c;
-        const TileItems ti = tile_of(t);
+        const long long mine = c > c_lo ? c : c_lo;
+        if (mine >= c_hi || pos_of(mine) >= tb + w) continue;
+        const TileItems ti = load_tile(mk, t);
         int n_items = 0;
         walk(ti, [&](int kk, unsigned, unsigned) { n_items = kk + 1; });
-        const unsigned w = walk(ti, [&](int kk, unsigned w0, unsigned w1) {
+        walk(ti, [&](int kk, unsigned w0, unsigned w1) {
             while (c < kChunks) {
                 const unsigned long long pc = pos_of(c);
                 if (pc >= tb + w1) break;
                 const int k = ((unsigned)(pc - tb) - w0) * 2 < (w1 - w0) ? kk : kk + 1;
-                if (k >= n_items) { a.chunk_start[c] = t + 1 < n_tiles ? t + 1 : n_tiles; a.chunk_rank[c] = 0; }
-                else { a.chunk_start[c] = t; a.chunk_rank[c] = k; }
+                if (k >= n_items) put(c, t + 1 < n_tiles ? t + 1 : n_tiles, 0);
+                else put(c, t, k);
                 ++c;
             }
         });
         if (n_items == 0)
-            for (; c < kChunks && pos_of(c) < tb + w; ++c) { a.chunk_start[c] = t; a.chunk_rank[c] = 0; }
-        before += w;
+            for (; c < kChunks && pos_of(c) < tb + w; ++c) put(c, t, 0);
     }
 }
 
@@ -348,6 +383,7 @@
     const float *rows;
     const unsigned *row_counter;
     int rows_cap;
+    int own_rows;
     int accumulate;
     const int *wexp;
     int debug;
@@ -381,6 +417,62 @@
 __device__ __forceinline__ void store_quad(unsigned char *planes, int row, int c4, float4 v)
 {
     store_quad_at<F16>(planes, row * kRowBytes + ((((c4 >> 1) ^ (row & 15)) << 4) | ((c4 & 1) << 3)), v);
+}
+
+struct DirectBox { float wt[16], rcp, masked, area; bool vis; unsigned rws[4], cls[4]; };
+__device__ __forceinline__ DirectBox direct_box(const uint4 *rp)
+{
+    uint4 r[6];
+#pragma unroll
+    for (int k = 0; k < 6; ++k) r[k] = rp[k];
+    DirectBox bx;
+#pragma unroll
+    for (int k = 0; k < 4; ++k) {
+        bx.wt[4 * k + 0] = __uint_as_float(r[k].x); bx.wt[4 * k + 1] = __uint_as_float(r[k].y);
+        bx.wt[4 * k + 2] = __uint_as_float(r[k].z); bx.wt[4 * k + 3] = __uint_as_float(r[k].w);
+    }
+    bx.rcp = __uint_as_float(r[4].x); bx.masked = __uint_as_float(r[5].z); bx.area = __uint_as_float(r[5].w);
+    bx.vis = (r[4].y & (unsigned)kVis) != 0u;
+    const unsigned rw[4] = {r[4].z & 0xffffu, r[4].z >> 16, r[4].w & 0xffffu, r[4].w >> 16};
+    const unsigned cl[4] = {r[5].x & 0xffffu, r[5].x >> 16, r[5].y & 0xffffu, r[5].y >> 16};
+#pragma unroll
+    for (int k = 0; k < 4; ++k) { bx.rws[k] = bx.vis ? rw[k] : 0u; bx.cls[k] = bx.vis ? cl[k] : 0u; }
+    return bx;
+}
+__device__ __forceinline__ void direct_taps(const DirectBox &bx, const char *img, int Wp, float4 (&t)[4][4])
+{
+#pragma unroll
+    for (int i = 0; i < 4; ++i)
+#pragma unroll
+        for (int j = 0; j < 4; ++j) t[i][j] = *reinterpret_cast<const float4 *>(img + (size_t)(bx.rws[i] * Wp + bx.cls[j]) * kSlotBytes);
+    __builtin_amdgcn_sched_barrier(0);
+}
+__device__ __forceinline__ float4 direct_mean(const DirectBox &bx, const float4 (&t)[4][4])
+{
+    const float *wt = bx.wt;
+    const float4 lt = sample4(t[0][0], t[0][1], t[1][0], t[1][1], wt[0], wt[1], wt[2], wt[3]);
+    const float4 rb = sample4(t[2][2], t[2][3], t[3][2], t[3][3], wt[4], wt[5], wt[6], wt[7]);
+    const float4 rt = sample4(t[0][2], t[0][3], t[1][2], t[1][3], wt[8], wt[9], wt[10], wt[11]);
+    const float4 lb2 = sample4(t[2][0], t[2][1], t[3][0], t[3][1], wt[12], wt[13], wt[14], wt[15]);
+    float4 res = make_float4(box_mean(lt.x, rb.x, rt.x, lb2.x, bx.area, bx.rcp), box_mean(lt.y, rb.y, rt.y, lb2.y, bx.area, bx.rcp),
+                             box_mean(lt.z, rb.z, rt.z, lb2.z, bx.area, bx.rcp), box_mean(lt.w, rb.w, rt.w, lb2.w, bx.area, bx.rcp));
+    if (!bx.vis) res = make_float4(bx.masked, bx.masked, bx.masked, bx.masked);
+    return res;
+}
+__device__ __forceinline__ void direct_item_rows(const unsigned char *recs, const char *img_view, int Wp, float4 *slot_rows, int b, int cq)
+{
+    const DirectBox bx = direct_box(reinterpret_cast<const uint4 *>(recs + (size_t)b * kRecBytes));
+    const char *img = img_view + cq * 16;
+    float4 *dst = slot_rows + (size_t)b * (kC / 4) + cq;
+    float4 t0[4][4], t1[4][4];
+    direct_taps(bx, img, Wp, t0);
+    direct_taps(bx, img + 256, Wp, t1);
+    dst[0] = direct_mean(bx, t0);
+    direct_taps(bx, img + 512, Wp, t0);
+    dst[16] = direct_mean(bx, t1);
+    direct_taps(bx, img + 768, Wp, t1);
+    dst[32] = direct_mean(bx, t0);
+    dst[48] = direct_mean(bx, t1);
 }
 
 struct Item { int tile, scale, view; unsigned rest; bool valid; int rank; };
@@ -715,6 +807,24 @@
             for (int t2 = t_begin; t2 < (cur.valid ? cur.tile : t_end); ++t2) write_tile(t2, none, false);
     }
     if (!cur.valid) return;
+    if constexpr (!DIRECT) {
+        if (a.own_rows) {
+            for (Item p = cur; p.valid; p = seek(p.tile, p.scale, p.rest, p.rank + 1)) {
+                if (!((mask_at(a.sc[p.scale].direct, p.tile) >> p.view) & 1u)) continue;
+                const FusedScale &sc = a.sc[p.scale];
+                const size_t item = (size_t)p.view * a.n_tiles + p.tile;
+                typedef unsigned u32x4 __attribute__((ext_vector_type(4)));
+                const u32x4 h0 = *reinterpret_cast<const __attribute__((address_space(4))) u32x4 *>((size_t)(sc.hdrs + item * kHdrBytes));
+                if (!(h0.x & (unsigned)kTileRows) || h0.z >= (unsigned)a.rows_cap) continue;
+                const int wp = sc.Wf + 2;
+                direct_item_rows(sc.recs + item * kTileBoxes * kRecBytes,
+                                 reinterpret_cast<const char *>(sc.integral) + (size_t)p.view * (sc.Hf + 2) * wp * kSlotBytes, wp,
+                                 reinterpret_cast<float4 *>(const_cast<float *>(a.rows)) + (size_t)h0.z * kTileBoxes * (kC / 4), 4 * wave + (lane >> 4), lane & 15);
+            }
+            asm volatile("s_waitcnt vmcnt(0)" ::: "memory");
+            __syncthreads();
+        }
+    }
     const int dbg = DIAG ? a.debug : 0;
     unsigned long long stamp[8] = {0, 0, 0, 0, 0, 0, 0, 0}, t_prev = 0;
     auto tick = [&](int k) {
@@ -1142,32 +1252,11 @@
         const int s = (int)(e >> 30), view = (int)((e >> 25) & 31u), tile = (int)(e & 0x1ffffffu);
         const int Wp = a.Wf[s] + 2;
         const int item = view * a.n_tiles + tile;
-        const uint4 *rp = reinterpret_cast<const uint4 *>(a.recs[s] + ((size_t)item * kTileBoxes + b) * kRecBytes);
-        uint4 r[6];
-#pragma unroll
-        for (int k = 0; k < 6; ++k) r[k] = rp[k];
-        const float wt[16] = {__uint_as_float(r[0].x), __uint_as_float(r[0].y), __uint_as_float(r[0].z), __uint_as_float(r[0].w),
-                              __uint_as_float(r[1].x), __uint_as_float(r[1].y), __uint_as_float(r[1].z), __uint_as_float(r[1].w),
-                              __uint_as_float(r[2].x), __uint_as_float(r[2].y), __uint_as_float(r[2].z), __uint_as_float(r[2].w),
-                              __uint_as_float(r[3].x), __uint_as_float(r[3].y), __uint_as_float(r[3].z), __uint_as_float(r[3].w)};
-        const float rcp = __uint_as_float(r[4].x), masked = __uint_as_float(r[5].z), area = __uint_as_float(r[5].w);
-        const bool vis = (r[4].y & (unsigned)kVis) != 0u;
-        const unsigned rws[4] = {vis ? r[4].z & 0xffffu : 0u, vis ? r[4].z >> 16 : 0u, vis ? r[4].w & 0xffffu : 0u, vis ? r[4].w >> 16 : 0u};
-        const unsigned cls[4] = {vis ? r[5].x & 0xffffu : 0u, vis ? r[5].x >> 16 : 0u, vis ? r[5].y & 0xffffu : 0u, vis ? r[5].y >> 16 : 0u};
+        const DirectBox bx = direct_box(reinterpret_cast<const uint4 *>(a.recs[s] + ((size_t)item * kTileBoxes + b) * kRecBytes));
         const char *img = reinterpret_cast<const char *>(a.integral[s]) + (size_t)view * (a.Hf[s] + 2) * Wp * kSlotBytes + q * 256 + cq * 16;
         float4 t[4][4];
-#pragma unroll
-        for (int i = 0; i < 4; ++i)
-#pragma unroll
-            for (int j = 0; j < 4; ++j) t[i][j] = *reinterpret_cast<const float4 *>(img + (size_t)(rws[i] * Wp + cls[j]) * kSlotBytes);
-        __builtin_amdgcn_sched_barrier(0);
-        const float4 lt = sample4(t[0][0], t[0][1], t[1][0], t[1][1], wt[0], wt[1], wt[2], wt[3]);
-        const float4 rb = sample4(t[2][2], t[2][3], t[3][2], t[3][3], wt[4], wt[5], wt[6], wt[7]);
-        const float4 rt = sample4(t[0][2], t[0][3], t[1][2], t[1][3], wt[8], wt[9], wt[10], wt[11]);
-        const float4 lb2 = sample4(t[2][0], t[2][1], t[3][0], t[3][1], wt[12], wt[13], wt[14], wt[15]);
-        float4 res = make_float4(box_mean(lt.x, rb.x, rt.x, lb2.x, area, rcp), box_mean(lt.y, rb.y, rt.y, lb2.y, area, rcp),
-                                 box_mean(lt.z, rb.z, rt.z, lb2.z, area, rcp), box_mean(lt.w, rb.w, rt.w, lb2.w, area, rcp));
-        if (!vis) res = make_float4(masked, masked, masked, masked);
+        direct_taps(bx, img, Wp, t);
+        const float4 res = direct_mean(bx, t);
         reinterpret_cast<float4 *>(a.rows)[((size_t)slot * kTileBoxes + b) * (kC / 4) + q * 16 + cq] = res;
     }
 }
@@ -1175,7 +1264,7 @@
 
 struct WorkspaceLayout {
     size_t live[kMaxScales], direct[kMaxScales], overflow[kMaxScales], counter, hdrs[kMaxScales], recs[kMaxScales], wfrag[kMaxScales],
-        masks_bytes, chunks, ranks, diag, rows, row_list, partial, tickets, item_w, wmax, wexp, amax, total;
+        masks_bytes, chunks, ranks, diag, rows, row_list, partial, tickets, item_w, tile_w, wmax, wexp, amax, total;
     int tiles_l, tiles_w, n_tiles, rows_cap, views_pad;
 };
 inline WorkspaceLayout layout_of(int n_views, int L, int W, int n_scales)
@@ -1193,6 +1282,7 @@
     }
     w.counter = off; off += 256;
     w.tickets = off; off = align_up(off + (size_t)w.n_tiles * sizeof(unsigned), 256);
+    w.tile_w = off; off = align_up(off + (size_t)w.n_tiles * sizeof(unsigned), 256);
     w.masks_bytes = off;
     for (int s = 0; s < kMaxScales; ++s) {
         const bool on = s < n_scales;
@@ -1301,6 +1391,7 @@
     a.rows_cap = (unsigned)rows_cap_of(lay, workspace_bytes);
     a.row_list = reinterpret_cast<unsigned *>(ws + lay.row_list);
     a.item_w = reinterpret_cast<unsigned short *>(ws + lay.item_w);
+    a.tile_w = reinterpret_cast<unsigned *>(ws + lay.tile_w);
     a.views_pad = lay.views_pad;
     const hipError_t e = zero_fill(ws, lay.masks_bytes, s);
     if (e != hipSuccess) return (int)e;
@@ -1313,7 +1404,7 @@
                        size_t workspace_bytes, void *stream)
 {
     const int terms = flags & VFA_FLAG_TERMS_MASK;
-    if ((flags & ~VFA_FLAG_TERMS_MASK) || (terms != 0 && terms != 2 && terms != 3 && terms != 4)) return VFA_ERR_BAD_ARGUMENT;
+    if ((flags & ~(VFA_FLAG_TERMS_MASK | VFA_FLAG_OWN_ROWS)) || (terms != 0 && terms != 2 && terms != 3 && terms != 4)) return VFA_ERR_BAD_ARGUMENT;
     if (n_views < 0 || L < 0 || W < 0 || n_scales < 1 || n_scales > kMaxScales) return VFA_ERR_BAD_ARGUMENT;
     if (n_views > 32) return VFA_ERR_UNSUPPORTED;
     const WorkspaceLayout lay = layout_of(n_views, L, W, n_scales);
@@ -1326,7 +1417,10 @@
         const int q = k < n_scales ? k : 0;
         ca.live[k] = reinterpret_cast<const unsigned *>(ws + lay.live[q]);
         ca.overflow[k] = reinterpret_cast<const unsigned *>(ws + lay.overflow[q]);
-    }
+        ca.direct[k] = reinterpret_cast<const unsigned *>(ws + lay.direct[q]);
+    }
+    ca.tile_w = reinterpret_cast<const unsigned *>(ws + lay.tile_w);
+    ca.own_cost = (flags & VFA_FLAG_OWN_ROWS) ? kOwnRowCost : 0u;
     ca.n_scales = n_scales; ca.n_tiles = lay.n_tiles; ca.n_views = n_views; ca.views_pad = lay.views_pad;
     ca.item_w = reinterpret_cast<const unsigned short *>(ws + lay.item_w);
     ca.chunk_start = reinterpret_cast<int *>(ws + lay.chunks);
@@ -1345,8 +1439,8 @@
         sa.f16 = (terms == 0 || terms == 2) ? 1 : 0;
         ca.n_split_blocks = n_scales * kSplitBlocks;
     }
-    if (n_views <= 8) hipLaunchKernelGGL(tile_chunks_kernel<1>, dim3(1 + ca.n_split_blocks), dim3(1024), 0, s, ca);
-    else hipLaunchKernelGGL(tile_chunks_kernel<4>, dim3(1 + ca.n_split_blocks), dim3(1024), 0, s, ca);
+    if (n_views <= 8) hipLaunchKernelGGL(tile_chunks_kernel<1>, dim3(kCutBlocks + ca.n_split_blocks), dim3(1024), 0, s, ca);
+    else hipLaunchKernelGGL(tile_chunks_kernel<4>, dim3(kCutBlocks + ca.n_split_blocks), dim3(1024), 0, s, ca);
     return (int)hipGetLastError();
 }
 
@@ -1402,8 +1496,8 @@
     const int terms = flags & VFA_FLAG_TERMS_MASK, reserved_cus = (flags >> 8) & 0xff;
     const int debug = ((flags >> 16) & 0xfff) | ((flags & VFA_FLAG_DUMP_VOX) ? kDbgDumpVox : 0);
     if (debug && terms != 0 && terms != 2) return VFA_ERR_BAD_ARGUMENT;
-    if (flags & ~(VFA_FLAG_TERMS_MASK | 0xfffff00 | VFA_FLAG_ROWS_ONLY | VFA_FLAG_SKIP_ROWS | VFA_FLAG_DUMP_VOX)) return VFA_ERR_BAD_ARGUMENT;
-    if ((flags & VFA_FLAG_ROWS_ONLY) && (flags & VFA_FLAG_SKIP_ROWS)) return VFA_ERR_BAD_ARGUMENT;
+    if (flags & ~(VFA_FLAG_TERMS_MASK | 0xfffff00 | VFA_FLAG_ROWS_ONLY | VFA_FLAG_SKIP_ROWS | VFA_FLAG_DUMP_VOX | VFA_FLAG_OWN_ROWS)) return VFA_ERR_BAD_ARGUMENT;
+    if ((flags & VFA_FLAG_ROWS_ONLY) && (flags & (VFA_FLAG_SKIP_ROWS | VFA_FLAG_OWN_ROWS))) return VFA_ERR_BAD_ARGUMENT;
     if (n_views < 0 || L < 0 || W < 0 || n_scales < 1 || n_scales > kMaxScales || !feat_hw || !integrals ||
         (terms != 0 && terms != 2 && terms != 3 && terms != 4))
         return VFA_ERR_BAD_ARGUMENT;
@@ -1476,7 +1570,8 @@
     a.rows = reinterpret_cast<const float *>(ws + lay.rows);
     a.row_counter = reinterpret_cast<const unsigned *>(ws + lay.counter);
     a.rows_cap = rows_cap;
-    if (!(debug & 64) && !(flags & VFA_FLAG_SKIP_ROWS)) {
+    a.own_rows = (flags & VFA_FLAG_OWN_ROWS) ? 1 : 0;
+    if (!(debug & 64) && !(flags & (VFA_FLAG_SKIP_ROWS | VFA_FLAG_OWN_ROWS))) {
         RowsArgs ra;
         for (int k = 0; k < kMaxScales; ++k) {
             ra.integral[k] = a.sc[k].integral; ra.recs[k] = a.sc[k].recs;
diff --git a/vfa_amd/ops.py b/vfa_amd/ops.py
--- a/vfa_amd/ops.py
+++ b/vfa_amd/ops.py
@@ -723,7 +723,7 @@
 
 
 def frame_records(calibs, grid, z_layers, corner_off, conv_kind, image_wh, feat_hws, weights=None, crange=(-1, 0.95),
-                  workspace=None, row_slots=None, cuts=True, terms=0):
+                  workspace=None, row_slots=None, cuts=True, terms=0, own_rows=False):
     calibs, grid, z_layers, corner_off = _geometry(calibs, grid, z_layers, corner_off)
     n, (L, W) = calibs.shape[0], grid.shape[:2]
     if z_layers.numel() != 1:
@@ -744,15 +744,17 @@
                 _lib.ptr(workspace), workspace.numel(), _lib.current_stream_handle(), tag=(n, L, W, ns))
         return workspace
     _launch("vfa_frame_records_f32", _lib.ptr(calibs), _lib.ptr(grid), _lib.ptr(z_layers), _lib.ptr(corner_off), n, L, W,
-            int(conv_kind), float(image_wh[0]), float(image_wh[1]), float(crange[0]), float(crange[1]), ns, hw, wts, int(terms) & 0xf,
+            int(conv_kind), float(image_wh[0]), float(image_wh[1]), float(crange[0]), float(crange[1]), ns, hw, wts,
+            (int(terms) & 0xf) | (_lib.FLAG_OWN_ROWS if own_rows else 0),
             _lib.ptr(workspace), workspace.numel(), _lib.current_stream_handle(), tag=(n, L, W, ns))
     return workspace
 
 
-def frame_cuts(workspace, n_views, grid_lw, n_scales, weights=None, terms=0):
+def frame_cuts(workspace, n_views, grid_lw, n_scales, weights=None, terms=0, own_rows=False):
     _lib.require_device(workspace)
     wts = _weight_ptrs(weights, n_scales, (256, 256))
-    _launch("vfa_frame_cuts_f32", int(n_views), int(grid_lw[0]), int(grid_lw[1]), int(n_scales), wts, int(terms) & 0xf, _lib.ptr(workspace),
+    _launch("vfa_frame_cuts_f32", int(n_views), int(grid_lw[0]), int(grid_lw[1]), int(n_scales), wts,
+            (int(terms) & 0xf) | (_lib.FLAG_OWN_ROWS if own_rows else 0), _lib.ptr(workspace),
             workspace.numel(), _lib.current_stream_handle(), tag=(int(n_views), int(grid_lw[0]), int(grid_lw[1]), int(n_scales)))
     return workspace
 
@@ -760,7 +762,7 @@
 def pool_collapse(integrals, biases, workspace, grid_lw, out=None, accumulate=False, terms=0, reserved_cus=0, debug=0, stage="all",
                   absmax=None, dump_vox=False):
     _lib.require_device(*integrals, workspace, out)
-    stage_flag = {"all": 0, "rows": _lib.FLAG_ROWS_ONLY, "main": _lib.FLAG_SKIP_ROWS}[stage]
+    stage_flag = {"all": 0, "rows": _lib.FLAG_ROWS_ONLY, "main": _lib.FLAG_SKIP_ROWS, "own": _lib.FLAG_OWN_ROWS}[stage]
     ns = len(integrals)
     n = integrals[0].shape[0]
     L, W = grid_lw
diff --git a/vfa_amd/vfa_op.py b/vfa_amd/vfa_op.py
--- a/vfa_amd/vfa_op.py
+++ b/vfa_amd/vfa_op.py
@@ -91,6 +91,7 @@
 
 
 SIDE_STREAM = os.environ.get("VFA_AMD_SIDE_STREAM", "1") == "1"
+OWN_ROWS = os.environ.get("VFA_AMD_OWN_ROWS", "0") == "1"
 _side_streams = {}
 
 
@@ -145,6 +146,10 @@
             ops.frame_records(calibs, grid, z_layers, corner_off, conv_kind, (img_w, img_h), feat_hws, weights=weights,
                               crange=crange, workspace=ws, terms=_fused_terms())
             boxes_done = None
+        elif OWN_ROWS:
+            with torch.cuda.stream(side):
+                ops.frame_records(calibs, grid, z_layers, corner_off, conv_kind, (img_w, img_h), feat_hws, weights=weights,
+                                  crange=crange, workspace=ws, terms=_fused_terms(), own_rows=True)
         else:
             with torch.cuda.stream(side):
                 ops.frame_records(calibs, grid, z_layers, corner_off, conv_kind, (img_w, img_h), feat_hws, crange=crange,
@@ -155,6 +160,10 @@
         if integrals is None:
             integrals = ops.integral_images(features)
         biases = [m.collapse.bias for m in mods]
+        if side is not cur and OWN_ROWS:
+            cur.wait_stream(side)
+            return ops.pool_collapse(integrals, biases, ws, (length, width), out=out, accumulate=accumulate, terms=_fused_terms(),
+                                     reserved_cus=reserved_cus, stage="own")
         if boxes_done is None:
             return ops.pool_collapse(integrals, biases, ws, (length, width), out=out, accumulate=accumulate, terms=_fused_terms(),
                                      reserved_cus=reserved_cus)
```

Measured after the change: 1.533 billion voxels/s (median of 3 runs). No clear change (+0.0%).
